# wei-zeng98/piano-a2s

Hardware: AMD Instinct MI355X
Metric: training clips/sec (12 s, 5-bar) (higher is better)
Workload: dtype f32

## Files before the change

### include/a2s.h

```cpp
#ifndef A2S_H
#define A2S_H
#include <stddef.h>
#include <stdint.h>
#ifdef __cplusplus
extern "C" {
#endif

#define A2S_OK 0
#define A2S_ERR_ARG (-1)
#define A2S_ERR_HIP (-2)
#define A2S_ERR_WORKSPACE (-3)

const char* a2s_last_error(void);
int a2s_version(void);
long long a2s_launch_count(void);

int a2s_gemm_f32(void* stream, int M, int N, int K, float alpha, const float* A, long sAm, long sAk,
                 const float* B, long sBk, long sBn, float beta, float* C, long ldc, const float* bias, int act,
                 int batch, long bsA, long bsB, long bsC, int splitk, float* workspace, size_t workspace_bytes);
int a2s_gemm_f32_affine(void* stream, int M, int N, int K, float alpha, const float* A, long sAm, long sAk, const float* B, long sBk,
                        long sBn, float beta, float* C, long ldc, const float* bias, int act, int batch, long bsA, long bsB, long bsC,
                        int splitk, float* workspace, size_t workspace_bytes, const float* a_scale, const float* a_shift, int a_period,
                        const float* b_scale, const float* b_shift, int b_period);
int a2s_gemm_f32_bnstats(void* stream, int M, int N, int K, const float* A, long sAm, long sAk, const float* B, long sBk, long sBn, float* C, long ldc,
                         const float* y, const float* mean, const float* invstd, const float* scale, const float* shift, int period, float* partial);
int a2s_gemm_f32_affine_scaled(void* stream, int M, int N, int K, float alpha, const float* A, long sAm, long sAk, const float* B, long sBk,
                               long sBn, float beta, float* C, long ldc, const float* bias, int act, int batch, long bsA, long bsB, long bsC,
                               int splitk, float* workspace, size_t workspace_bytes, const float* a_scale, const float* a_shift, int a_period,
                               const float* b_scale, const float* b_shift, int b_period, const float* a_absmax, const float* b_absmax);
int a2s_gemm_f32_bnstats_scaled(void* stream, int M, int N, int K, const float* A, long sAm, long sAk, const float* B, long sBk, long sBn, float* C, long ldc,
                                const float* y, const float* mean, const float* invstd, const float* scale, const float* shift, int period, float* partial,
                                const float* a_absmax, const float* b_absmax);
int a2s_linear_dgrad_bnstats(void* stream, int M, int N, int K, const float* dz, long lda, const float* Wt, float* da, long ldc, const float* y,
                             const float* mean, const float* invstd, const float* scale, const float* shift, int period, float* partial,
                             const float* dz_absmax, const float* w_absmax, float* workspace, size_t workspace_bytes, float* da_absmax_out);
int a2s_linear_fwd(void* stream, int M, int N, int K, const float* y, long lda, const float* W, float* z, long ldc, const float* scale, const float* shift,
                   int period, const float* y_absmax, const float* w_absmax, float* workspace, size_t workspace_bytes);
int a2s_linear_fwd_eligible(int M, int N, int K, int period);
int a2s_linear_wgrad(void* stream, int M, int N, int K, const float* dz, long ldz, const float* y, long lda, float* G, long ldg, const float* scale,
                     const float* shift, int period, const float* dz_absmax, const float* y_absmax, float* workspace, size_t workspace_bytes);
size_t a2s_linear_wgrad_ws_bytes(int M, int K);
int a2s_linear_wgrad_eligible(int M, int N, int K, int period);
size_t a2s_linear_dgrad_ws_bytes(int N, int K);
int a2s_linear_dgrad_blocks(int M);
int a2s_linear_dgrad_eligible(int M, int N, int K, int period);
int a2s_absmax(void* stream, const float* x, long n, float* out);
int a2s_gemm_bnstats_blocks(int M, int period);
size_t a2s_gemm_workspace_bytes(int M, int N, int batch, int splitk);
int a2s_gemm_pick_splitk(int M, int N, int K, int batch);
void a2s_gemm_debug_tile(int cfg);
int a2s_debug_set(const char* key, int value);
int a2s_debug_get(const char* key);
int a2s_env_check(void);
int a2s_persist_abort_latch(void* device_word);

int a2s_conv3x3(void* stream, const float* x, const float* w, float* y, const float* in_scale, const float* in_shift,
                float* stat_partial, int B, int T, int F, int Cin, int Cout, int flip, float* workspace);
int a2s_conv3x3_ranged(void* stream, const float* x, const float* w, float* y, const float* in_scale, const float* in_shift, const float* in_absmax,
                       float* stat_partial, float* out_absmax, int B, int T, int F, int Cin, int Cout, float* workspace);
int a2s_conv3x3_stat_blocks(int B, int T, int F, int Cin);
int a2s_conv3x3_dgrad_bnstats(void* stream, const float* dy, const float* w, float* g, const float* yl, const float* yl_mean, const float* yl_invstd,
                              const float* yl_scale, const float* yl_shift, float* stat_partial, int B, int T, int F, int Cin, int Cout,
                              float* workspace);
int a2s_bn_bwd_from_partial(void* stream, const float* g, const float* x, const float* mean, const float* invstd, const float* scale, const float* shift,
                            float* dgamma, float* dbeta, float* dx , const float* partial, int nblocks, float* c12, long rows, int C, int F);
int a2s_conv3x3_dgrad_bnstats_scaled(void* stream, const float* dy, const float* w, float* g, const float* yl, const float* yl_mean, const float* yl_invstd,
                                     const float* yl_scale, const float* yl_shift, float* stat_partial, int B, int T, int F, int Cin, int Cout,
                                     float* workspace, const float* dy_absmax);
int a2s_conv3x3_dgrad_bnstats_ranged(void* stream, const float* dy, const float* w, float* g, const float* yl, const float* yl_mean, const float* yl_invstd,
                                     const float* yl_scale, const float* yl_shift, float* stat_partial, int B, int T, int F, int Cin, int Cout,
                                     float* workspace, const float* dy_absmax, float* g_absmax_out);
int a2s_bn_bwd_from_partial_amax(void* stream, const float* g, const float* x, const float* mean, const float* invstd, const float* scale, const float* shift,
                                 float* dgamma, float* dbeta, float* dx, const float* partial, int nblocks, float* c12, long rows, int C, int F,
                                 float* dx_absmax);
size_t a2s_conv3x3_workspace_floats(int Cin);
int a2s_bn_finalize(void* stream, const float* partial, int nblocks, int C, double count, const float* gamma,
                    const float* beta, float* running_mean, float* running_var, long long* num_batches_tracked,
                    float* mean, float* invstd, float* scale, float* shift, float eps, float momentum, int training);
int a2s_bn_relu_apply(void* stream, const float* x, float* y, const float* scale, const float* shift, long n, int C, int F);
int a2s_col_stats(void* stream, const float* x, float* partial, long rows, int C, int rows_per_block);
int a2s_bn1d_relu_dropout(void* stream, const float* x, float* y, const float* scale, const float* shift,
                          const uint8_t* keep_mask, float inv_keep, long n, int C);

int a2s_gru_gates_fwd(void* stream, const float* gi, long ldgi, const float* gh, long ldgh, const float* hprev, long ldhp,
                      float* hout, long ldho, float* hout2, long ldho2, float* save, int R, int H);
int a2s_gru_seq_fwd(void* stream, const float* gi_all, long gi_bstride, long gi_tstride, const float* w_hh,
                    const float* b_hh, float* out, long out_bstride, long out_tstride, float* hbuf, float* gh,
                    float* save, float* hn, int B, int T, int H, int reverse, float* workspace, size_t workspace_bytes);

int a2s_attn_step_fwd(void* stream, const float* keys, const float* enc, const float* q, long ldq, const float* v,
                      float* ctx, long ldctx, float* ctx2, long ldctx2, float* attw, int B, int T, int H,
                      const int* n_done, int n_rows_total, float* workspace);
int a2s_attn_step_fwd_rows(void* stream, const float* keys, const float* enc, const float* q, long ldq, const float* v, float* ctx,
                           long ldctx, float* ctx2, long ldctx2, float* attw, int R, int T, int H, float* workspace, int n_clips,
                           const int* clip_order, const int* clip_rank, const int* row_until, int n_active, int step);
size_t a2s_attn_workspace_floats(int B, int T, int H);
size_t a2s_attn_workspace_floats_fused(int n_clips, int T, int H, int groups);

int a2s_log_softmax_rows(void* stream, const float* x, long ldx, float* y, long ldy, int* argmax_out, int R, int V);
int a2s_embed_rows(void* stream, const float* table, const long long* ids64, const int* ids32, long id_stride,
                   int const_id, float* out, long ldo, int col0, int R, int E, const uint8_t* keep_mask, float inv_keep);

typedef struct a2s_note_dec_args {
    const float* attn_w; const float* attn_b; const float* attn_v;
    const float* w_ih; const float* w_hh; const float* b_ih; const float* b_hh;
    const float* out_w; const float* out_b; const float* emb;
    const float* keys; const float* enc;
    float* h; float* x; float* q; float* gates; float* attw; float* o;
    float* gh; float* gi; float* logits;
    float* probs; long probs_bstride;
    const long long* gt; long gt_bstride;
    const uint8_t* tf_flags;
    const uint8_t* drop; float inv_keep;
    int* argmax_out; long am_bstride;
    int* eos_seen; long long* lengths; int* n_done;
    int* steps_exec;
    float* attn_ws;
    float* gemm_ws; size_t gemm_ws_bytes;
    int* t_base;
    const int* clip_order;
    const int* clip_rank;
    const int* row_until;
    const int* n_active;
    int n_clips;
    const int* m_active;
// ... 22 lines not shown
    float* probs_scratch;
    int* ids_out; long long* lengths_out; float* score_out;
} a2s_beam_args;
int a2s_note_decoder_fwd_beam(void* stream, const a2s_note_dec_args* args, const a2s_beam_args* beam, int* steps_done);
int a2s_beam_step(void* stream, const a2s_beam_args* beam, const float* logits, long ldl, const float* emb, float* xnext, long ldx, float* h, int h_cols,
                  float* q, int q_cols, int* n_done, int* steps_exec, int B, int V, int E, int t, int max_steps, int eos_id);
int a2s_beam_backtrack(void* stream, const a2s_beam_args* beam, float* probs, long probs_bstride, const int* steps_exec, int B, int V, int max_steps, int eos_id);
int a2s_beam_launches(void);
typedef struct a2s_align_args {
    float* attw_step;
    int* peak; float* weight; float* centroid;
    long out_stride;
    const signed char* next_state; int n_states;
    int* row_state;
} a2s_align_args;
int a2s_attn_align_rows(void* stream, const float* attw, long ldw, int R, int T, int* peak_out, float* weight_out, float* centroid_out, long out_stride);
int a2s_note_decoder_fwd_align(void* stream, const a2s_note_dec_args* args, const a2s_align_args* align, int* steps_done);
int a2s_align_launches(void);

int a2s_render_notes(void* stream, const int* programs, int rows_per_clip, int n_samples, float* wave, long wave_bstride, int B);
int a2s_render_launches(void);
int a2s_note_decoder_fwd_pair(void* stream_upper, void* stream_lower, const a2s_note_dec_args* upper, const a2s_note_dec_args* lower,
                              const int* pair_order, const int* pair_rank, const int* pair_n_active, int* steps_done_upper, int* steps_done_lower);
size_t a2s_note_step_workspace_floats(int H, int E);
size_t a2s_note_decoder_persist_ws_bytes(int n_clips, int R, int steps);
size_t a2s_note_decoder_bwd_persist_ws_bytes(int n_clips);

int a2s_staff_emb_fwd(void* stream, const float* note_emb, const float* const* gru_w, const long long* ids64,
                      const int* ids32, long id_bstride, const long long* lengths, long len_stride, float* out,
                      long ldo, int col0, float* hsave, int R, int maxlen, int E, int S);


int a2s_log_softmax_bwd_rows(void* stream, const float* g, const float* y, long outer_stride, int inner, float* dx,
                             int R, int V, int n_outer, int time_major);
int a2s_gru_gates_bwd(void* stream, const float* dh_a, long lda, const float* dh_b, long ldb, const float* save,
                      const float* hprev, long ldhp, float* dgi, long ldgi, float* dgh, long ldgh, float* dgh2, long ldgh2,
                      float* dhprev, long lddp, int R, int H);
int a2s_attn_step_bwd(void* stream, const float* keys, const float* enc, const float* q, long ldq, const float* v,
                      const float* attw, const float* ctx, long ldctx, const float* dctx_a, long ldda, const float* dctx_b,
                      long lddb, float* dctx_out, long lddo, float* dq, long lddq, float* ds_out, int B, int T, int H, float* workspace);
int a2s_attn_step_bwd_rows(void* stream, const float* keys, const float* enc, const float* q, long ldq, const float* v, const float* attw,
                           const float* ctx, long ldctx, const float* dctx_a, long ldda, const float* dctx_b, long lddb, float* dctx_out,
                           long lddo, float* dq, long lddq, float* ds_out, int R, int T, int H, float* workspace, int n_clips,
                           const int* clip_order, const int* clip_rank, const int* row_until, int n_active, int step);
int a2s_attn_dk_accum(void* stream, const float* keys, const float* q_all, const float* ds_all, const float* v, float* dK,
                      float* dv_partial, int B, int T, int S, int H, const int* row_until, int groups);
int a2s_attn_dk_blocks(int B, int T);
int a2s_attn_denc_accum(void* stream, const float* attw_all, const float* dctx_all, float* dEnc, int B, int T, int S, int H2,
                        const int* row_until, int groups);
int a2s_col_sum(void* stream, const float* x, long ld, float* out, long rows, int C, float alpha, float beta, float* workspace, size_t workspace_floats);
int a2s_embed_scatter_add(void* stream, float* table_grad, const long long* ids64, const int* ids32, long id_stride,
                          int const_id, const float* g, long ldg, int col0, int R, int E, const uint8_t* keep_mask, float inv_keep);
int a2s_ew_act_bwd(void* stream, const float* g, const float* y, float* dx, long n, int act);

typedef struct a2s_note_dec_bwd_args {
    const float* attn_w; const float* attn_v; const float* w_ih; const float* w_hh;
    const float* keys; const float* enc;
    const float* h; const float* x; const float* q; const float* gates; const float* attw;
    const float* do_all;
    float* dgi_all; float* dgh_all; float* dq_all; float* ds_all; float* dctx_all; float* dx;
    float* dh;
    float* attn_ws;
    float* gemm_ws; size_t gemm_ws_bytes;
    const int* clip_order;
    const int* clip_rank;
    const int* row_until;
    const int* n_active;
    int n_clips;
    const int* m_active;
    const int* row_list;
    const int* n_rows_active;
    int R, T, H, E, steps;
    float* step_ws; size_t step_ws_floats;
    float* persist_ws; size_t persist_ws_bytes;
    const float* w_ih_full;
} a2s_note_dec_bwd_args;
int a2s_note_decoder_bwd(void* stream, const a2s_note_dec_bwd_args* args);
int a2s_note_decoder_bwd_pair(void* stream_upper, void* stream_lower, const a2s_note_dec_bwd_args* upper, const a2s_note_dec_bwd_args* lower,
                              const int* pair_order, const int* pair_rank, const int* pair_n_active);

int a2s_gru_seq_bwd(void* stream, const float* dout, long do_bstride, long do_tstride, const float* out, long out_bstride,
                    long out_tstride, const float* gates, const float* w_hh, const float* dhn, float* dgi_all, float* dgh_shift,
                    float* dgh_first, float* dhbuf, float* dgh_tmp, int B, int T, int H, int reverse, float* workspace, size_t workspace_bytes);
int a2s_staff_emb_bwd(void* stream, const float* note_emb, const float* const* gru_w, float* const* grads, float* note_emb_grad,
                      const long long* ids64, const int* ids32, long id_bstride, const long long* lengths, long len_stride,
                      const float* dout, long lddo, int col0, const float* hsave, int R, int maxlen, int E, int S);

int a2s_bn_bwd(void* stream, const float* g, const float* x, const float* mean, const float* invstd, const float* scale,
               const float* shift, const uint8_t* keep_mask, float inv_keep, float* dgamma, float* dbeta, float* dx,
               float* partial, float* c12, long rows, int C, int F);
int a2s_bn_bwd_amax(void* stream, const float* g, const float* x, const float* mean, const float* invstd, const float* scale,
                    const float* shift, const uint8_t* keep_mask, float inv_keep, float* dgamma, float* dbeta, float* dx,
                    float* partial, float* c12, long rows, int C, int F, float* dx_absmax);
size_t a2s_bn_bwd_partial_floats(long rows, int C, int F);
int a2s_bn_bwd_stats(void* stream, const float* g, const float* x, const float* mean, const float* invstd, const float* scale,
                     const float* shift, const uint8_t* keep_mask, float inv_keep, float* partial, float* sums, long rows, int C, int F);
int a2s_bn_bwd_apply(void* stream, const float* g, const float* x, const float* mean, const float* invstd, const float* scale,
                     const float* shift, const uint8_t* keep_mask, float inv_keep, const float* sums_local, const float* sums_global,
                     double count_global, float* dgamma, float* dbeta, float* dx, float* c12, long rows, int C, int F);
int a2s_bn_bwd_sums_from_partial(void* stream, const float* partial, int nblocks, int C, float* sums);
int a2s_bn_bwd_c12_from_sums(void* stream, const float* sums_local, const float* sums_global, double count_global, float* dgamma, float* dbeta,
                             float* c12, int C);
int a2s_conv3x3_wgrad(void* stream, const float* dy, const float* x, const float* in_scale, const float* in_shift, float* dW,
                      float* workspace, size_t workspace_bytes, int B, int T, int F, int Cin, int Cout);
int a2s_conv3x3_wgrad_scaled(void* stream, const float* dy, const float* x, const float* in_scale, const float* in_shift, float* dW,
                             float* workspace, size_t workspace_bytes, int B, int T, int F, int Cin, int Cout, const float* dy_absmax);
int a2s_conv3x3_wgrad_ranged(void* stream, const float* dy, const float* x, const float* in_scale, const float* in_shift, float* dW, float* workspace,
                             size_t workspace_bytes, int B, int T, int F, int Cin, int Cout, const float* dy_absmax, const float* act_absmax);
int a2s_act_bound(void* stream, const float* scale, const float* shift, const float* absmax, int C, float* out);
size_t a2s_conv3x3_wgrad_workspace_bytes(int Cin, int Cout);
int a2s_conv3x3_wgrad_bn(void* stream, const float* g, const float* y, const float* mean, const float* invstd, const float* scale, const float* shift,
                         const float* c12, float* dy_out, const float* x, const float* in_scale, const float* in_shift, float* dW, float* workspace,
                         size_t workspace_bytes, int B, int T, int F, int Cin, int Cout);
int a2s_conv3x3_wgrad_bn_ranged(void* stream, const float* g, const float* y, const float* mean, const float* invstd, const float* scale, const float* shift,
                                const float* c12, const float* g_absmax, int g_absmax_n, const float* y_absmax, float* dy_out, float* dy_absmax_out, const float* x,
                                const float* in_scale, const float* in_shift, float* dW, float* workspace, size_t workspace_bytes, int B, int T, int F,
                                int Cin, int Cout, const float* act_absmax);
int a2s_conv3x3_wgrad_bn_ranged_eligible(int F, int Cin, int Cout);

int a2s_nll_loss(void* stream, const float* logp, const long long* target, long rows, int V, long long ignore_index,
                 float* loss_out, float* dlogp, float gscale, double* partial, int nblocks);
int a2s_nll_grad(void* stream, float* dlogp, const long long* target, const float* loss_out, float gscale, long rows, int V,
                 long long ignore_index);
int a2s_clip_adadelta(void* stream, float* params, float* grads, float* square_avg, float* acc_delta, long n, const float* loss,
                      float max_norm, float lr, float rho, float eps, float* ctl, double* partial, int nblocks, int zero_grad);

int a2s_vqt_logmag(void* stream, const float* C, float* out, float* partial, int B, long rows, int bins, float top_db);
int a2s_vqt_logmag_octaves(void* stream, const float* C, float* out, float* partial, int B, long rows, int bins, int bins_per_octave, float top_db);
int a2s_vqt_decimate(void* stream, const float* ypad, long padded_len, const float* taps, int ntaps, float* out, long n_out, int B);

int a2s_edit_distance(void* stream, const int* ref, const long long* ref_off, const int* hyp, const long long* hyp_off, const int* order,
                      int n_pairs, int max_ref_len, int max_hyp_len, int* dist);
int a2s_edit_distance_max_len(void);

#ifdef __cplusplus
}
#endif
#endif
```

### piano_a2s_amd/csrc/a2s_api.hip

```cpp
#define A2S_SWITCHES_IMPL
#include "a2s_internal.h"

thread_local char a2s_err_msg[512] = {0};
long long a2s_launch_counter = 0;

#define ST ((hipStream_t)stream)

extern "C" {

const char* a2s_last_error(void) { return a2s_err_msg; }
int a2s_version(void) { return 1; }
long long a2s_launch_count(void) { return __atomic_load_n(&a2s_launch_counter, __ATOMIC_RELAXED); }

int a2s_gemm_f32(void* stream, int M, int N, int K, float alpha, const float* A, long sAm, long sAk, const float* B, long sBk,
                 long sBn, float beta, float* C, long ldc, const float* bias, int act, int batch, long bsA, long bsB, long bsC,
                 int splitk, float* workspace, size_t workspace_bytes) {
    return a2s_gemm_impl(ST, M, N, K, alpha, A, sAm, sAk, B, sBk, sBn, beta, C, ldc, bias, act, batch, bsA, bsB, bsC, splitk,
                         workspace, workspace_bytes);
}
int a2s_gemm_f32_affine(void* stream, int M, int N, int K, float alpha, const float* A, long sAm, long sAk, const float* B, long sBk,
                        long sBn, float beta, float* C, long ldc, const float* bias, int act, int batch, long bsA, long bsB, long bsC,
                        int splitk, float* workspace, size_t workspace_bytes, const float* a_scale, const float* a_shift, int a_period,
                        const float* b_scale, const float* b_shift, int b_period) {
    return a2s_gemm_affine_impl(ST, M, N, K, alpha, A, sAm, sAk, B, sBk, sBn, beta, C, ldc, bias, act, batch, bsA, bsB, bsC, splitk,
                                workspace, workspace_bytes, a_scale, a_shift, a_period, b_scale, b_shift, b_period,
                                nullptr, nullptr, nullptr, nullptr, nullptr, nullptr, 0, 0, nullptr, nullptr);
}
int a2s_gemm_f32_affine_scaled(void* stream, int M, int N, int K, float alpha, const float* A, long sAm, long sAk, const float* B, long sBk,
                               long sBn, float beta, float* C, long ldc, const float* bias, int act, int batch, long bsA, long bsB, long bsC,
                               int splitk, float* workspace, size_t workspace_bytes, const float* a_scale, const float* a_shift, int a_period,
                               const float* b_scale, const float* b_shift, int b_period, const float* a_absmax, const float* b_absmax) {
    return a2s_gemm_affine_impl(ST, M, N, K, alpha, A, sAm, sAk, B, sBk, sBn, beta, C, ldc, bias, act, batch, bsA, bsB, bsC, splitk,
                                workspace, workspace_bytes, a_scale, a_shift, a_period, b_scale, b_shift, b_period,
                                nullptr, nullptr, nullptr, nullptr, nullptr, nullptr, 0, 1, a_absmax, b_absmax);
}
int a2s_gemm_f32_bnstats_scaled(void* stream, int M, int N, int K, const float* A, long sAm, long sAk, const float* B, long sBk, long sBn, float* C, long ldc,
                                const float* y, const float* mean, const float* invstd, const float* scale, const float* shift, int period, float* partial,
                                const float* a_absmax, const float* b_absmax) {
    return a2s_gemm_affine_impl(ST, M, N, K, 1.f, A, sAm, sAk, B, sBk, sBn, 0.f, C, ldc, nullptr, 0, 1, 0, 0, 0, 1, nullptr, 0,
                                nullptr, nullptr, 0, nullptr, nullptr, 0, y, mean, invstd, scale, shift, partial, period, 1, a_absmax, b_absmax);
}
int a2s_absmax(void* stream, const float* x, long n, float* out) { return a2s_absmax_impl(ST, x, n, out); }
int a2s_linear_dgrad_bnstats(void* stream, int M, int N, int K, const float* dz, long lda, const float* Wt, float* da, long ldc, const float* y,
                             const float* mean, const float* invstd, const float* scale, const float* shift, int period, float* partial,
                             const float* dz_absmax, const float* w_absmax, float* workspace, size_t workspace_bytes, float* da_absmax_out) {
    return a2s_linear_dgrad_bnstats_impl(ST, M, N, K, dz, lda, Wt, 1, K, da, ldc, y, mean, invstd, scale, shift, period, partial, dz_absmax, w_absmax,
                                         workspace, workspace_bytes, da_absmax_out);
}
size_t a2s_linear_dgrad_ws_bytes(int N, int K) { return a2s_linear_dgrad_ws_bytes_impl(N, K); }
int a2s_linear_fwd(void* stream, int M, int N, int K, const float* y, long lda, const float* W, float* z, long ldc, const float* scale, const float* shift,
                   int period, const float* y_absmax, const float* w_absmax, float* workspace, size_t workspace_bytes) {
    return a2s_linear_fwd_impl(ST, M, N, K, y, lda, W, z, ldc, scale, shift, period, y_absmax, w_absmax, workspace, workspace_bytes);
}
int a2s_linear_wgrad(void* stream, int M, int N, int K, const float* dz, long ldz, const float* y, long lda, float* G, long ldg, const float* scale,
                     const float* shift, int period, const float* dz_absmax, const float* y_absmax, float* workspace, size_t workspace_bytes) {
    return a2s_linear_wgrad_impl(ST, M, N, K, dz, ldz, y, lda, G, ldg, scale, shift, period, dz_absmax, y_absmax, workspace, workspace_bytes);
}
size_t a2s_linear_wgrad_ws_bytes(int M, int K) { return a2s_linear_wgrad_ws_bytes_impl(M, K); }
int a2s_linear_wgrad_eligible(int M, int N, int K, int period) { return a2s_linear_wgrad_ok(M, N, K, 256, 4, 4, period, nullptr, nullptr, nullptr) ? 1 : 0; }
int a2s_linear_fwd_eligible(int M, int N, int K, int period) { return a2s_linear_fwd_ok(M, N, K, 4, 4, period, nullptr, nullptr, nullptr) ? 1 : 0; }
int a2s_linear_dgrad_blocks(int M) { return a2s_linear_dgrad_blocks_impl(M); }
int a2s_linear_dgrad_eligible(int M, int N, int K, int period) {
    return a2s_linear_dgrad_ok(M, N, K, 4, 1, K, 4, period, nullptr, nullptr, nullptr, nullptr) ? 1 : 0;
}
int a2s_gemm_f32_bnstats(void* stream, int M, int N, int K, const float* A, long sAm, long sAk, const float* B, long sBk, long sBn, float* C, long ldc,
                         const float* y, const float* mean, const float* invstd, const float* scale, const float* shift, int period, float* partial) {
    return a2s_gemm_affine_impl(ST, M, N, K, 1.f, A, sAm, sAk, B, sBk, sBn, 0.f, C, ldc, nullptr, 0, 1, 0, 0, 0, 1, nullptr, 0,
                                nullptr, nullptr, 0, nullptr, nullptr, 0, y, mean, invstd, scale, shift, partial, period, 0, nullptr, nullptr);
}
int a2s_gemm_bnstats_blocks(int M, int period) { return a2s_cdiv(M, 128) * a2s_gemm_bnstats_slots(period); }
size_t a2s_gemm_workspace_bytes(int M, int N, int batch, int splitk) { return a2s_gemm_workspace_bytes_impl(M, N, batch, splitk); }
int a2s_gemm_pick_splitk(int M, int N, int K, int batch) { return a2s_gemm_pick_splitk_impl(M, N, K, batch); }
void a2s_gemm_debug_tile(int cfg) { a2s_gemm_debug_tile_impl(cfg); }
size_t a2s_note_step_workspace_floats(int H, int E) { return a2s_note_step_workspace_floats_impl(H, E); }
int a2s_debug_set(const char* key, int value) {
    if (!key) return A2S_ERR_ARG;
    const int id = a2s_switch_find(key);
    if (id >= 0) { a2s_switch_store(id, value); return A2S_OK; }
    if (!strcmp(key, "attn_deferred_fast")) { a2s_attn_deferred_fast = value ? 1 : 0; return A2S_OK; }
    if (!strcmp(key, "gemm_tile")) { a2s_gemm_debug_tile_impl(value); return A2S_OK; }
    snprintf(a2s_err_msg, sizeof(a2s_err_msg), "a2s_debug_set: unknown key %s", key);
    return A2S_ERR_ARG;
}
int a2s_env_check(void) {
    if (const char* e = a2s_switch_env_error()) A2S_FAIL(A2S_ERR_ARG, "%s: expected a decimal number >= 0", e);
    return A2S_OK;
}

int a2s_persist_abort_latch(void* device_word) { a2s_persist_latch_set(device_word); return A2S_OK; }

int a2s_debug_get(const char* key) {
    if (!key) return -1;
    const int id = a2s_switch_find(key);
    if (id == A2S_SW_attn_pair_fused_rows) return a2s_attn_pair_fused_rows();
    if (id >= 0) return a2s_sw((a2s_switch)id);
    if (!strcmp(key, "attn_pair_launches")) return (int)a2s_attn_pair_launches();
    if (!strcmp(key, "attn_pair_bwd_launches")) return (int)a2s_attn_pair_bwd_launches();
    if (!strcmp(key, "attn_deferred_fast")) return a2s_attn_deferred_fast;
    if (!strcmp(key, "attn_dk_ahead_launches")) return (int)a2s_attn_dk_ahead_launches();
    if (!strcmp(key, "attn_denc_launches")) return (int)a2s_attn_denc_launches();
    if (!strcmp(key, "dec_mid_launches")) return a2s_dec_mid_launches();
    if (!strcmp(key, "dec_persist_launches")) return a2s_dec_persist_launches();
    if (!strcmp(key, "edit_distance_launches")) return (int)a2s_edit_distance_launches();
    if (!strcmp(key, "conv_rows16_c20_launches")) return (int)a2s_conv_rows16_c20_launches();
    if (!strcmp(key, "device_cus")) return a2s_device_geometry().cus;
    if (!strcmp(key, "device_xccs")) return a2s_device_geometry().xccs;
    return -1;
}

int a2s_conv3x3(void* stream, const float* x, const float* w, float* y, const float* in_scale, const float* in_shift,
                float* stat_partial, int B, int T, int F, int Cin, int Cout, int flip, float* workspace) {
    return a2s_conv3x3_impl(ST, x, w, y, in_scale, in_shift, stat_partial, B, T, F, Cin, Cout, flip, workspace, nullptr, nullptr, nullptr, nullptr, nullptr, nullptr,
                            nullptr, nullptr);
}
int a2s_conv3x3_ranged(void* stream, const float* x, const float* w, float* y, const float* in_scale, const float* in_shift, const float* in_absmax,
                       float* stat_partial, float* out_absmax, int B, int T, int F, int Cin, int Cout, float* workspace) {
    return a2s_conv3x3_impl(ST, x, w, y, in_scale, in_shift, stat_partial, B, T, F, Cin, Cout, 0, workspace, nullptr, nullptr, nullptr, nullptr, nullptr, nullptr,
                            in_absmax, out_absmax);
}
int a2s_conv3x3_dgrad_bnstats(void* stream, const float* dy, const float* w, float* g, const float* yl, const float* yl_mean, const float* yl_invstd,
                              const float* yl_scale, const float* yl_shift, float* stat_partial, int B, int T, int F, int Cin, int Cout,
                              float* workspace) {
    if (!yl) { snprintf(a2s_err_msg, sizeof(a2s_err_msg), "conv3x3_dgrad_bnstats: yl is required"); return A2S_ERR_ARG; }
    return a2s_conv3x3_impl(ST, dy, w, g, nullptr, nullptr, stat_partial, B, T, F, Cin, Cout, 1, workspace, yl, yl_mean, yl_invstd, yl_scale, yl_shift, nullptr, nullptr, nullptr);
}
int a2s_conv3x3_dgrad_bnstats_scaled(void* stream, const float* dy, const float* w, float* g, const float* yl, const float* yl_mean, const float* yl_invstd,
                                     const float* yl_scale, const float* yl_shift, float* stat_partial, int B, int T, int F, int Cin, int Cout,
                                     float* workspace, const float* dy_absmax) {
    if (!yl) { snprintf(a2s_err_msg, sizeof(a2s_err_msg), "conv3x3_dgrad_bnstats_scaled: yl is required"); return A2S_ERR_ARG; }
    return a2s_conv3x3_impl(ST, dy, w, g, nullptr, nullptr, stat_partial, B, T, F, Cin, Cout, 1, workspace, yl, yl_mean, yl_invstd, yl_scale, yl_shift, dy_absmax, nullptr, nullptr);
}
int a2s_conv3x3_dgrad_bnstats_ranged(void* stream, const float* dy, const float* w, float* g, const float* yl, const float* yl_mean, const float* yl_invstd,
                                     const float* yl_scale, const float* yl_shift, float* stat_partial, int B, int T, int F, int Cin, int Cout,
                                     float* workspace, const float* dy_absmax, float* g_absmax_out) {
    if (!yl) { snprintf(a2s_err_msg, sizeof(a2s_err_msg), "conv3x3_dgrad_bnstats_ranged: yl is required"); return A2S_ERR_ARG; }
    return a2s_conv3x3_impl(ST, dy, w, g, nullptr, nullptr, stat_partial, B, T, F, Cin, Cout, 1, workspace, yl, yl_mean, yl_invstd, yl_scale, yl_shift, dy_absmax, nullptr, g_absmax_out);
}
int a2s_bn_bwd_from_partial(void* stream, const float* g, const float* x, const float* mean, const float* invstd, const float* scale, const float* shift,
                            float* dgamma, float* dbeta, float* dx, const float* partial, int nblocks, float* c12, long rows, int C, int F) {
    return a2s_bn_bwd_from_partial_impl(ST, g, x, mean, invstd, scale, shift, dgamma, dbeta, dx, partial, nblocks, c12, rows, C, F, nullptr);
}
int a2s_bn_bwd_from_partial_amax(void* stream, const float* g, const float* x, const float* mean, const float* invstd, const float* scale, const float* shift,
                                 float* dgamma, float* dbeta, float* dx, const float* partial, int nblocks, float* c12, long rows, int C, int F,
                                 float* dx_absmax) {
    return a2s_bn_bwd_from_partial_impl(ST, g, x, mean, invstd, scale, shift, dgamma, dbeta, dx, partial, nblocks, c12, rows, C, F, dx_absmax);
}
size_t a2s_conv3x3_workspace_floats(int Cin) { return a2s_conv3x3_workspace_floats_impl(Cin); }
int a2s_conv3x3_stat_blocks(int B, int T, int F, int Cin) { return a2s_conv3x3_stat_blocks_impl(B, T, F, Cin); }
int a2s_bn_finalize(void* stream, const float* partial, int nblocks, int C, double count, const float* gamma, const float* beta,
                    float* running_mean, float* running_var, long long* nbt, float* mean, float* invstd, float* scale,
                    float* shift, float eps, float momentum, int training) {
    return a2s_bn_finalize_impl(ST, partial, nblocks, C, count, gamma, beta, running_mean, running_var, nbt, mean, invstd, scale,
                                shift, eps, momentum, training);
}
int a2s_bn_relu_apply(void* stream, const float* x, float* y, const float* scale, const float* shift, long n, int C, int F) {
    return a2s_bn_relu_apply_impl(ST, x, y, scale, shift, n, C, F);
}
int a2s_col_stats(void* stream, const float* x, float* partial, long rows, int C, int rows_per_block) {
    return a2s_col_stats_impl(ST, x, partial, rows, C, rows_per_block);
}
int a2s_bn1d_relu_dropout(void* stream, const float* x, float* y, const float* scale, const float* shift, const uint8_t* keep_mask,
                          float inv_keep, long n, int C) {
    return a2s_bn1d_relu_dropout_impl(ST, x, y, scale, shift, keep_mask, inv_keep, n, C);
}
int a2s_gru_gates_fwd(void* stream, const float* gi, long ldgi, const float* gh, long ldgh, const float* hprev, long ldhp,
                      float* hout, long ldho, float* hout2, long ldho2, float* save, int R, int H) {
    return a2s_gru_gates_fwd_impl(ST, gi, ldgi, gh, ldgh, hprev, ldhp, hout, ldho, hout2, ldho2, save, R, H);
}
int a2s_gru_seq_fwd(void* stream, const float* gi_all, long gi_bstride, long gi_tstride, const float* w_hh, const float* b_hh,
                    float* out, long out_bstride, long out_tstride, float* hbuf, float* gh, float* save, float* hn, int B, int T,
                    int H, int reverse, float* workspace, size_t workspace_bytes) {
    return a2s_gru_seq_fwd_impl(ST, gi_all, gi_bstride, gi_tstride, w_hh, b_hh, out, out_bstride, out_tstride, hbuf, gh, save, hn,
                                B, T, H, reverse, workspace, workspace_bytes);
}
int a2s_attn_step_fwd(void* stream, const float* keys, const float* enc, const float* q, long ldq, const float* v, float* ctx,
                      long ldctx, float* ctx2, long ldctx2, float* attw, int B, int T, int H, const int* n_done, int n_rows_total, float* workspace) {
    return a2s_attn_step_fwd_impl(ST, keys, enc, q, ldq, v, ctx, ldctx, ctx2, ldctx2, attw, B, T, H, n_done, n_rows_total, workspace, nullptr);
}
int a2s_attn_step_fwd_rows(void* stream, const float* keys, const float* enc, const float* q, long ldq, const float* v, float* ctx,
                           long ldctx, float* ctx2, long ldctx2, float* attw, int R, int T, int H, float* workspace, int n_clips,
                           const int* clip_order, const int* clip_rank, const int* row_until, int n_active, int step) {
// ... 39 lines not shown
    if (!beam) { snprintf(a2s_err_msg, sizeof(a2s_err_msg), "beam_backtrack: null args"); return A2S_ERR_ARG; }
    const a2s_beam_args& g = *beam;
    const BeamBackArgs a = {g.score, g.token_hist, g.parent_hist, g.probs_scratch, probs, probs_bstride, g.ids_out, (long)max_steps, g.lengths_out, g.score_out,
                            steps_exec, g.alpha, B, g.K, V, max_steps, eos_id, g.pad_id};
    return a2s_beam_backtrack_impl(ST, a);
}
int a2s_beam_launches(void) { return a2s_beam_launches_impl(); }
int a2s_attn_align_rows(void* stream, const float* attw, long ldw, int R, int T, int* peak_out, float* weight_out, float* centroid_out, long out_stride) {
    return a2s_attn_align_rows_impl(ST, attw, ldw, R, T, peak_out, weight_out, centroid_out, out_stride);
}
int a2s_note_decoder_fwd_align(void* stream, const a2s_note_dec_args* args, const a2s_align_args* align, int* steps_done) {
    if (!args || !align) { snprintf(a2s_err_msg, sizeof(a2s_err_msg), "note_decoder_fwd_align: null args"); return A2S_ERR_ARG; }
    return a2s_note_decoder_fwd_align_impl(ST, *args, *align, steps_done);
}
int a2s_align_launches(void) { return a2s_align_launches_impl(); }
int a2s_render_notes(void* stream, const int* programs, int rows_per_clip, int n_samples, float* wave, long wave_bstride, int B) {
    return a2s_render_notes_impl(ST, programs, rows_per_clip, n_samples, wave, wave_bstride, B);
}
int a2s_render_launches(void) { return a2s_render_launches_impl(); }
int a2s_note_decoder_fwd_pair(void* stream_upper, void* stream_lower, const a2s_note_dec_args* upper, const a2s_note_dec_args* lower,
                              const int* pair_order, const int* pair_rank, const int* pair_n_active, int* steps_done_upper, int* steps_done_lower) {
    if (!upper || !lower) { snprintf(a2s_err_msg, sizeof(a2s_err_msg), "note_decoder_fwd_pair: null args"); return A2S_ERR_ARG; }
    return a2s_note_decoder_fwd_pair_impl((hipStream_t)stream_upper, (hipStream_t)stream_lower, *upper, *lower, pair_order, pair_rank, pair_n_active,
                                          steps_done_upper, steps_done_lower);
}
int a2s_staff_emb_fwd(void* stream, const float* note_emb, const float* const* gru_w, const long long* ids64, const int* ids32,
                      long id_bstride, const long long* lengths, long len_stride, float* out, long ldo, int col0, float* hsave,
                      int R, int maxlen, int E, int S) {
    if (!gru_w) { snprintf(a2s_err_msg, sizeof(a2s_err_msg), "staff_emb_fwd: null weight table"); return A2S_ERR_ARG; }
    return a2s_staff_emb_fwd_impl(ST, note_emb, gru_w, ids64, ids32, id_bstride, lengths, len_stride, out, ldo, col0, hsave, R,
                                  maxlen, E, S);
}

int a2s_log_softmax_bwd_rows(void* stream, const float* g, const float* y, long outer_stride, int inner, float* dx, int R, int V,
                             int n_outer, int time_major) {
    return a2s_log_softmax_bwd_rows_impl(ST, g, y, outer_stride, inner, dx, R, V, n_outer, time_major);
}
int a2s_gru_gates_bwd(void* stream, const float* dh_a, long lda, const float* dh_b, long ldb, const float* save, const float* hprev,
                      long ldhp, float* dgi, long ldgi, float* dgh, long ldgh, float* dgh2, long ldgh2, float* dhprev, long lddp, int R, int H) {
    return a2s_gru_gates_bwd_impl(ST, dh_a, lda, dh_b, ldb, save, hprev, ldhp, dgi, ldgi, dgh, ldgh, dgh2, ldgh2, dhprev, lddp, R, H);
}
int a2s_attn_step_bwd(void* stream, const float* keys, const float* enc, const float* q, long ldq, const float* v, const float* attw,
                      const float* ctx, long ldctx, const float* dctx_a, long ldda, const float* dctx_b, long lddb, float* dctx_out,
                      long lddo, float* dq, long lddq, float* ds_out, int B, int T, int H, float* workspace) {
    return a2s_attn_step_bwd_impl(ST, keys, enc, q, ldq, v, attw, ctx, ldctx, dctx_a, ldda, dctx_b, lddb, dctx_out, lddo, dq, lddq, ds_out, B, T, H, workspace, nullptr);
}
int a2s_attn_step_bwd_rows(void* stream, const float* keys, const float* enc, const float* q, long ldq, const float* v, const float* attw,
                           const float* ctx, long ldctx, const float* dctx_a, long ldda, const float* dctx_b, long lddb, float* dctx_out,
                           long lddo, float* dq, long lddq, float* ds_out, int R, int T, int H, float* workspace, int n_clips,
                           const int* clip_order, const int* clip_rank, const int* row_until, int n_active, int step) {
    a2s_attn_rows rows = {clip_order, clip_rank, row_until, n_clips, n_active, step};
    return a2s_attn_step_bwd_impl(ST, keys, enc, q, ldq, v, attw, ctx, ldctx, dctx_a, ldda, dctx_b, lddb, dctx_out, lddo, dq, lddq, ds_out, R, T, H, workspace, &rows);
}
int a2s_attn_dk_accum(void* stream, const float* keys, const float* q_all, const float* ds_all, const float* v, float* dK,
                      float* dv_partial, int B, int T, int S, int H, const int* row_until, int groups) {
    return a2s_attn_dk_accum_impl(ST, keys, q_all, ds_all, v, dK, dv_partial, B, T, S, H, row_until, groups);
}
int a2s_attn_dk_blocks(int B, int T) { return B * ((T + 15) / 16); }
int a2s_attn_denc_accum(void* stream, const float* attw_all, const float* dctx_all, float* dEnc, int B, int T, int S, int H2,
                        const int* row_until, int groups) {
    return a2s_attn_denc_accum_impl(ST, attw_all, dctx_all, dEnc, B, T, S, H2, row_until, groups);
}
int a2s_col_sum(void* stream, const float* x, long ld, float* out, long rows, int C, float alpha, float beta, float* workspace, size_t workspace_floats) {
    return a2s_col_sum_impl(ST, x, ld, out, rows, C, alpha, beta, workspace, workspace_floats);
}
int a2s_embed_scatter_add(void* stream, float* table_grad, const long long* ids64, const int* ids32, long id_stride, int const_id,
                          const float* g, long ldg, int col0, int R, int E, const uint8_t* keep_mask, float inv_keep) {
    return a2s_embed_scatter_add_impl(ST, table_grad, ids64, ids32, id_stride, const_id, g, ldg, col0, R, E, keep_mask, inv_keep);
}
int a2s_ew_act_bwd(void* stream, const float* g, const float* y, float* dx, long n, int act) { return a2s_ew_act_bwd_impl(ST, g, y, dx, n, act); }
int a2s_note_decoder_bwd(void* stream, const a2s_note_dec_bwd_args* args) {
    if (!args) { snprintf(a2s_err_msg, sizeof(a2s_err_msg), "note_decoder_bwd: null args"); return A2S_ERR_ARG; }
    return a2s_note_decoder_bwd_impl(ST, *args);
}
int a2s_note_decoder_bwd_pair(void* stream_upper, void* stream_lower, const a2s_note_dec_bwd_args* upper, const a2s_note_dec_bwd_args* lower,
                              const int* pair_order, const int* pair_rank, const int* pair_n_active) {
    if (!upper || !lower) { snprintf(a2s_err_msg, sizeof(a2s_err_msg), "note_decoder_bwd_pair: null args"); return A2S_ERR_ARG; }
    return a2s_note_decoder_bwd_pair_impl((hipStream_t)stream_upper, (hipStream_t)stream_lower, *upper, *lower, pair_order, pair_rank, pair_n_active);
}
int a2s_gru_seq_bwd(void* stream, const float* dout, long do_bstride, long do_tstride, const float* out, long out_bstride, long out_tstride,
                    const float* gates, const float* w_hh, const float* dhn, float* dgi_all, float* dgh_shift, float* dgh_first,
                    float* dhbuf, float* dgh_tmp, int B, int T, int H, int reverse, float* workspace, size_t workspace_bytes) {
    return a2s_gru_seq_bwd_impl(ST, dout, do_bstride, do_tstride, out, out_bstride, out_tstride, gates, w_hh, dhn, dgi_all, dgh_shift,
                                dgh_first, dhbuf, dgh_tmp, B, T, H, reverse, workspace, workspace_bytes);
}
int a2s_staff_emb_bwd(void* stream, const float* note_emb, const float* const* gru_w, float* const* grads, float* note_emb_grad,
                      const long long* ids64, const int* ids32, long id_bstride, const long long* lengths, long len_stride,
                      const float* dout, long lddo, int col0, const float* hsave, int R, int maxlen, int E, int S) {
    if (!gru_w) { snprintf(a2s_err_msg, sizeof(a2s_err_msg), "staff_emb_bwd: null weight table"); return A2S_ERR_ARG; }
    return a2s_staff_emb_bwd_impl(ST, note_emb, gru_w, grads, note_emb_grad, ids64, ids32, id_bstride, lengths, len_stride, dout, lddo,
                                  col0, hsave, R, maxlen, E, S);
}

int a2s_bn_bwd(void* stream, const float* g, const float* x, const float* mean, const float* invstd, const float* scale, const float* shift,
               const uint8_t* keep_mask, float inv_keep, float* dgamma, float* dbeta, float* dx, float* partial, float* c12, long rows, int C, int F) {
    return a2s_bn_bwd_impl(ST, g, x, mean, invstd, scale, shift, keep_mask, inv_keep, dgamma, dbeta, dx, partial, c12, rows, C, F, nullptr);
}
int a2s_bn_bwd_amax(void* stream, const float* g, const float* x, const float* mean, const float* invstd, const float* scale, const float* shift,
                    const uint8_t* keep_mask, float inv_keep, float* dgamma, float* dbeta, float* dx, float* partial, float* c12, long rows, int C, int F,
                    float* dx_absmax) {
    return a2s_bn_bwd_impl(ST, g, x, mean, invstd, scale, shift, keep_mask, inv_keep, dgamma, dbeta, dx, partial, c12, rows, C, F, dx_absmax);
}
size_t a2s_bn_bwd_partial_floats(long rows, int C, int F) { return a2s_bn_bwd_partial_floats_impl(rows, C, F); }
int a2s_conv3x3_wgrad(void* stream, const float* dy, const float* x, const float* in_scale, const float* in_shift, float* dW, float* workspace,
                      size_t workspace_bytes, int B, int T, int F, int Cin, int Cout) {
    return a2s_conv3x3_wgrad_impl(ST, dy, x, in_scale, in_shift, dW, workspace, workspace_bytes, B, T, F, Cin, Cout, nullptr, nullptr, nullptr, nullptr,
                                  nullptr, nullptr, nullptr, nullptr, nullptr);
}
int a2s_conv3x3_wgrad_ranged(void* stream, const float* dy, const float* x, const float* in_scale, const float* in_shift, float* dW, float* workspace,
                             size_t workspace_bytes, int B, int T, int F, int Cin, int Cout, const float* dy_absmax, const float* act_absmax) {
    return a2s_conv3x3_wgrad_impl(ST, dy, x, in_scale, in_shift, dW, workspace, workspace_bytes, B, T, F, Cin, Cout, nullptr, nullptr, nullptr, nullptr,
                                  nullptr, nullptr, nullptr, dy_absmax, act_absmax);
}
int a2s_act_bound(void* stream, const float* scale, const float* shift, const float* absmax, int C, float* out) {
    return a2s_act_bound_impl(ST, scale, shift, absmax, C, out);
}
int a2s_conv3x3_wgrad_scaled(void* stream, const float* dy, const float* x, const float* in_scale, const float* in_shift, float* dW, float* workspace,
                             size_t workspace_bytes, int B, int T, int F, int Cin, int Cout, const float* dy_absmax) {
    return a2s_conv3x3_wgrad_impl(ST, dy, x, in_scale, in_shift, dW, workspace, workspace_bytes, B, T, F, Cin, Cout, nullptr, nullptr, nullptr, nullptr,
                                  nullptr, nullptr, nullptr, dy_absmax, nullptr);
}
int a2s_conv3x3_wgrad_bn(void* stream, const float* g, const float* y, const float* mean, const float* invstd, const float* scale, const float* shift,
                         const float* c12, float* dy_out, const float* x, const float* in_scale, const float* in_shift, float* dW, float* workspace,
                         size_t workspace_bytes, int B, int T, int F, int Cin, int Cout) {
    if (!y) { snprintf(a2s_err_msg, sizeof(a2s_err_msg), "conv3x3_wgrad_bn: y is required"); return A2S_ERR_ARG; }
    return a2s_conv3x3_wgrad_impl(ST, g, x, in_scale, in_shift, dW, workspace, workspace_bytes, B, T, F, Cin, Cout, y, mean, invstd, scale, shift, c12, dy_out, nullptr, nullptr);
}
size_t a2s_conv3x3_wgrad_workspace_bytes(int Cin, int Cout) { return a2s_conv3x3_wgrad_workspace_bytes_impl(Cin, Cout); }
int a2s_conv3x3_wgrad_bn_ranged_eligible(int F, int Cin, int Cout) { return (a2s_wgrad_rows_eligible(F, Cin, Cout) && !(Cin == 40 && Cout == 20)) ? 1 : 0; }
int a2s_conv3x3_wgrad_bn_ranged(void* stream, const float* g, const float* y, const float* mean, const float* invstd, const float* scale, const float* shift,
                                const float* c12, const float* g_absmax, int g_absmax_n, const float* y_absmax, float* dy_out, float* dy_absmax_out, const float* x,
                                const float* in_scale, const float* in_shift, float* dW, float* workspace, size_t workspace_bytes, int B, int T, int F,
                                int Cin, int Cout, const float* act_absmax) {
    if (!a2s_conv3x3_wgrad_bn_ranged_eligible(F, Cin, Cout)) { snprintf(a2s_err_msg, sizeof(a2s_err_msg), "conv3x3_wgrad_bn_ranged: shape not eligible"); return A2S_ERR_ARG; }
    return a2s_conv3x3_wgrad_rows_bn_impl(ST, g, y, mean, invstd, scale, shift, c12, g_absmax, g_absmax_n, y_absmax, dy_out, dy_absmax_out, x, in_scale, in_shift, dW,
                                          workspace, workspace_bytes, B, T, F, Cin, Cout, act_absmax);
}

int a2s_nll_grad(void* stream, float* dlogp, const long long* target, const float* loss_out, float gscale, long rows, int V, long long ignore_index) {
    return a2s_nll_grad_impl(ST, dlogp, target, loss_out, gscale, rows, V, ignore_index);
}
int a2s_nll_loss(void* stream, const float* logp, const long long* target, long rows, int V, long long ignore_index, float* loss_out,
                 float* dlogp, float gscale, double* partial, int nblocks) {
    return a2s_nll_loss_impl(ST, logp, target, rows, V, ignore_index, loss_out, dlogp, gscale, partial, nblocks);
}
int a2s_clip_adadelta(void* stream, float* params, float* grads, float* square_avg, float* acc_delta, long n, const float* loss, float max_norm,
                      float lr, float rho, float eps, float* ctl, double* partial, int nblocks, int zero_grad) {
    return a2s_clip_adadelta_impl(ST, params, grads, square_avg, acc_delta, n, loss, max_norm, lr, rho, eps, ctl, partial, nblocks, zero_grad);
}

int a2s_vqt_logmag(void* stream, const float* C, float* out, float* partial, int B, long rows, int bins, float top_db) {
    return a2s_vqt_logmag_impl(ST, C, out, partial, B, rows, bins, top_db);
}

int a2s_edit_distance(void* stream, const int* ref, const long long* ref_off, const int* hyp, const long long* hyp_off, const int* order,
                      int n_pairs, int max_ref_len, int max_hyp_len, int* dist) {
    return a2s_edit_distance_impl(ST, ref, ref_off, hyp, hyp_off, order, n_pairs, max_ref_len, max_hyp_len, dist);
}
int a2s_edit_distance_max_len(void) { return a2s_edit_distance_max_len_impl(); }

int a2s_bn_bwd_stats(void* stream, const float* g, const float* x, const float* mean, const float* invstd, const float* scale, const float* shift,
                     const uint8_t* keep_mask, float inv_keep, float* partial, float* sums, long rows, int C, int F) {
    return a2s_bn_bwd_stats_impl(ST, g, x, mean, invstd, scale, shift, keep_mask, inv_keep, partial, sums, rows, C, F);
}
int a2s_bn_bwd_apply(void* stream, const float* g, const float* x, const float* mean, const float* invstd, const float* scale, const float* shift,
                     const uint8_t* keep_mask, float inv_keep, const float* sums_local, const float* sums_global, double count_global,
                     float* dgamma, float* dbeta, float* dx, float* c12, long rows, int C, int F) {
// ... 19 lines not shown
```

### piano_a2s_amd/csrc/a2s_bwd.hip

```cpp
#include "a2s_internal.h"

__global__ __launch_bounds__(256) void log_softmax_bwd_rows(const float* __restrict__ g, const float* __restrict__ y,
                                                            long outer_stride, int inner, float* __restrict__ dx,
                                                            int R, int V, int n_outer, int time_major) {
    const int row = blockIdx.x * 4 + (threadIdx.x >> 6), lane = threadIdx.x & 63;
    if (row >= R) return;
    const int ob = row / inner, in = row % inner;
    const float* gr = g + (long)ob * outer_stride + (long)in * V;
    const float* yr = y + (long)ob * outer_stride + (long)in * V;
    float s = 0.f;
    for (int j = lane; j < V; j += 64) s += gr[j];
    s = wave_sum(s);
    const long orow = time_major ? ((long)in * n_outer + ob) : row;
    for (int j = lane; j < V; j += 64) dx[orow * V + j] = gr[j] - expf(yr[j]) * s;
}

int a2s_log_softmax_bwd_rows_impl(hipStream_t st, const float* g, const float* y, long outer_stride, int inner, float* dx,
                                  int R, int V, int n_outer, int time_major) {
    hipLaunchKernelGGL(log_softmax_bwd_rows, dim3(a2s_cdiv(R, 4)), dim3(256), 0, st, g, y, outer_stride, inner, dx, R, V, n_outer, time_major);
    A2S_CHECK_LAUNCH("log_softmax_bwd_rows");
    return A2S_OK;
}

__global__ void gru_gates_bwd(const float* __restrict__ dh_a, long lda, const float* __restrict__ dh_b, long ldb,
// ... 473 lines not shown
    for (int s = a.steps - 1; s >= 0 && !any_fused; --s) any_fused = note_bwd_step_fused(a, s);
    const bool mid = a2s_note_step_mid_bwd_ok(a);
    bool any_mid = false;
    if (mid) for (int s = a.steps - 1; s >= 0 && !any_mid; --s) any_mid = !note_bwd_step_fused(a, s);
    if (any_fused || any_mid) { int rc = a2s_note_step_fused_bwd_prepare(st, a); if (rc) return rc; }
    *mid_out = mid;
    return A2S_OK;
}
static int note_bwd_finish(hipStream_t st, const a2s_note_dec_bwd_args& a, int cur) {
    if (cur != 0) {
        const hipError_t e = hipMemcpyAsync(a.dh, a.dh + (long)a.R * 2 * a.H, sizeof(float) * a.R * 2 * a.H, hipMemcpyDeviceToDevice, st);
        if (e != hipSuccess) A2S_FAIL(A2S_ERR_HIP, "note_decoder_bwd copy: %s", hipGetErrorString(e));
    }
    return A2S_OK;
}

int a2s_note_decoder_bwd_impl(hipStream_t st, const a2s_note_dec_bwd_args& a) {
    if (a2s_note_decoder_bwd_persist_ok(a)) return a2s_note_decoder_bwd_persist(st, a);
    bool mid = false;
    int rc = note_bwd_prepare(st, a, &mid);
    if (rc) return rc;
    int cur = 0;
    for (int s = a.steps - 1; s >= 0; --s) {
        rc = note_bwd_step(st, a, s, cur, mid, 0, nullptr);
        if (rc) return rc;
    }
    return note_bwd_finish(st, a, cur);
}

int a2s_note_decoder_bwd_pair_impl(hipStream_t su, hipStream_t sl, const a2s_note_dec_bwd_args& au, const a2s_note_dec_bwd_args& al, const int* pair_order,
                                   const int* pair_rank, const int* pair_n_active) {
    const a2s_note_dec_bwd_args* as[2] = {&au, &al};
    hipStream_t sts[2] = {su, sl};
    const bool can_pair = a2s_sw(A2S_SW_attn_pair) && su != sl && pair_order && pair_rank && pair_n_active && au.n_active && al.n_active && au.n_clips > 0 &&
                          au.n_clips == al.n_clips && au.R == al.R && au.T == al.T && au.H == 256 && al.H == 256 && au.enc == al.enc && au.attn_ws && al.attn_ws &&
                          !a2s_note_decoder_bwd_persist_ok(au) && !a2s_note_decoder_bwd_persist_ok(al) && a2s_note_step_mid_bwd_ok(au) && a2s_note_step_mid_bwd_ok(al);
    if (!can_pair) {
        const int rc = a2s_note_decoder_bwd_impl(su, au);
        return rc ? rc : a2s_note_decoder_bwd_impl(sl, al);
    }
    static thread_local hipEvent_t ev[2] = {nullptr, nullptr};
    for (int k = 0; k < 2; ++k)
        if (!ev[k]) { const hipError_t e = hipEventCreateWithFlags(&ev[k], hipEventDisableTiming); if (e != hipSuccess) A2S_FAIL(A2S_ERR_HIP, "note_decoder_bwd_pair: hipEventCreate: %s", hipGetErrorString(e)); }
    bool mid[2] = {false, false};
    int cur[2] = {0, 0};
    const PairRowsLimit limit(a2s_attn_pair_fused_rows());
    for (int k = 0; k < 2; ++k) { const int rc = note_bwd_prepare(sts[k], *as[k], &mid[k]); if (rc) return rc; }
    const int nmax = au.steps > al.steps ? au.steps : al.steps;
    for (int s = nmax - 1; s >= 0; --s) {
        bool in[2], fused[2] = {false, false};
        for (int k = 0; k < 2; ++k) { in[k] = s < as[k]->steps; if (in[k]) fused[k] = note_bwd_step_fused(*as[k], s); }
        AttnPairBwdStep p = {pair_order, pair_rank, au.n_clips, pair_n_active[s], s, 1, au.T};
        const bool joint = in[0] && in[1] && mid[0] && mid[1] && !fused[0] && !fused[1] && p.n_active > 0 && au.n_active[s] > 0 && al.n_active[s] > 0;
        if (!joint) {
            for (int k = 0; k < 2; ++k)
                if (in[k]) { const int rc = note_bwd_step(sts[k], *as[k], s, cur[k], mid[k], 0, nullptr); if (rc) return rc; }
            continue;
        }
        for (int k = 0; k < 2; ++k) { const int rc = note_bwd_step(sts[k], *as[k], s, cur[k], mid[k], 1, nullptr); if (rc) return rc; }
        hipError_t e = hipEventRecord(ev[1], sl);
        if (e == hipSuccess) e = hipStreamWaitEvent(su, ev[1], 0);
        if (e != hipSuccess) A2S_FAIL(A2S_ERR_HIP, "note_decoder_bwd_pair: event: %s", hipGetErrorString(e));
        const int rc = attn_pair_bwd_sweep(su, au, al, s, p);
        if (rc) return rc;
        e = hipEventRecord(ev[0], su);
        if (e == hipSuccess) e = hipStreamWaitEvent(sl, ev[0], 0);
        if (e != hipSuccess) A2S_FAIL(A2S_ERR_HIP, "note_decoder_bwd_pair: event: %s", hipGetErrorString(e));
        for (int k = 0; k < 2; ++k) { const int rc2 = note_bwd_step(sts[k], *as[k], s, cur[k], mid[k], 2, &p); if (rc2) return rc2; }
    }
    for (int k = 0; k < 2; ++k) { const int rc = note_bwd_finish(sts[k], *as[k], cur[k]); if (rc) return rc; }
    return A2S_OK;
}


__global__ void transpose_f32(const float* __restrict__ in, float* __restrict__ out, int rows, int cols) {
    const int idx = blockIdx.x * blockDim.x + threadIdx.x;
    if (idx >= rows * cols) return;
    const int c = idx / rows, r = idx % rows;
    out[idx] = in[(long)r * cols + c];
}

int a2s_gru_seq_bwd_impl(hipStream_t st, const float* dout, long do_bstride, long do_tstride, const float* out, long out_bstride,
                         long out_tstride, const float* gates, const float* w_hh, const float* dhn, float* dgi_all, float* dgh_shift,
                         float* dgh_first, float* dhbuf, float* dgh_tmp, int B, int T, int H, int reverse, float* ws, size_t ws_bytes) {
    A2S_REQUIRE(dout && out && gates && w_hh && dgi_all && dgh_shift && dgh_first && dhbuf && dgh_tmp, "gru_seq_bwd: null tensor");
    hipError_t e;
    if (dhn) e = hipMemcpyAsync(dhbuf, dhn, sizeof(float) * B * H, hipMemcpyDeviceToDevice, st);
    else e = hipMemsetAsync(dhbuf, 0, sizeof(float) * B * H, st);
    if (e != hipSuccess) A2S_FAIL(A2S_ERR_HIP, "gru_seq_bwd init: %s", hipGetErrorString(e));
    e = hipMemsetAsync(dgh_shift, 0, sizeof(float) * (size_t)B * T * 3 * H, st);
    if (e != hipSuccess) A2S_FAIL(A2S_ERR_HIP, "gru_seq_bwd memset: %s", hipGetErrorString(e));
    const bool fused = a2s_sw(A2S_SW_gru_fused) && H % 32 == 0 && ws && ws_bytes >= sizeof(float) * 3 * H * H && ((uintptr_t)ws % 16 == 0);
    if (fused) {
        hipLaunchKernelGGL(transpose_f32, dim3(a2s_cdiv(3 * H * H, 256)), dim3(256), 0, st, w_hh, ws, 3 * H, H);
        A2S_CHECK_LAUNCH("transpose_f32");
    }
    if (fused && a2s_gru_seq_bwd_persist_ok(B, T, H, ws, ws_bytes, sizeof(float) * 3 * (size_t)H * H))
        return a2s_gru_seq_bwd_persist_impl(st, dout, do_bstride, do_tstride, out, out_bstride, out_tstride, gates, ws, dhn, dgi_all, dgh_shift, dgh_first, B, T, H,
                                            reverse, ws, sizeof(float) * 3 * (size_t)H * H, ws_bytes);
    if (fused && ws_bytes >= sizeof(float) * (3 * (size_t)H * H + 3 * (size_t)B * H) && (3 * H * H) % 4 == 0) {
        float* tmp[2] = {dgh_tmp, ws + 3 * (size_t)H * H};
        auto tix = [&](int s) { return reverse ? T - 1 - s : s; };
        int cur = 0, p = 0;
        {
            const int s = T - 1, t = tix(s), tp = reverse ? t + 1 : t - 1;
            float* dgh = (s == 0) ? dgh_first : tmp[p];
            int rc = a2s_gru_gates_bwd_impl(st, dhbuf, H, dout + (long)t * do_tstride, do_bstride, gates + (long)t * B * 4 * H,
                                            s == 0 ? nullptr : out + (long)tp * out_tstride, out_bstride,
                                            dgi_all + (long)t * 3 * H, (long)T * 3 * H, dgh, 3 * H,
                                            s == 0 ? nullptr : dgh_shift + (long)tp * 3 * H, (long)T * 3 * H, dhbuf + (long)B * H, H, B, H);
            if (rc) return rc;
            cur = 1;
        }
        for (int s = T - 1; s >= 1; --s) {
            const int sp = s - 1, t = tix(sp), tp = reverse ? t + 1 : t - 1;
            float* dgh_out = (sp == 0) ? dgh_first : tmp[p ^ 1];
            int rc = a2s_gru_bptt_step_impl(st, tmp[p], ws, dhbuf + (long)cur * B * H, dout + (long)t * do_tstride, do_bstride,
                                            gates + (long)t * B * 4 * H, sp == 0 ? nullptr : out + (long)tp * out_tstride, out_bstride,
                                            dgi_all + (long)t * 3 * H, (long)T * 3 * H, dgh_out,
                                            sp == 0 ? nullptr : dgh_shift + (long)tp * 3 * H, (long)T * 3 * H,
                                            dhbuf + (long)(cur ^ 1) * B * H, B, H);
            if (rc) return rc;
            cur ^= 1; p ^= 1;
        }
        return A2S_OK;
    }
    int cur = 0;
    for (int s = T - 1; s >= 0; --s) {
        const int t = reverse ? T - 1 - s : s;
        const int tp = reverse ? t + 1 : t - 1;
        float* dh_in = dhbuf + (long)cur * B * H;
        float* dh_out = dhbuf + (long)(cur ^ 1) * B * H;
        float* dgh = (s == 0) ? dgh_first : dgh_tmp;
        int rc = a2s_gru_gates_bwd_impl(st, dh_in, H, dout + (long)t * do_tstride, do_bstride, gates + (long)t * B * 4 * H,
                                        s == 0 ? nullptr : out + (long)tp * out_tstride, out_bstride,
                                        dgi_all + (long)t * 3 * H, (long)T * 3 * H, dgh, 3 * H,
                                        s == 0 ? nullptr : dgh_shift + (long)tp * 3 * H, (long)T * 3 * H, dh_out, H, B, H);
        if (rc) return rc;
        if (s > 0) {
            if (fused) rc = a2s_skinny_gemm_acc_impl(st, dgh, 3 * H, ws, 3 * H, dh_out, H, B, H, 3 * H);
            else rc = a2s_gemm_impl(st, B, H, 3 * H, 1.f, dgh, 3 * H, 1, w_hh, H, 1, 1.f, dh_out, H, nullptr, 0, 1, 0, 0, 0, 0, ws, ws_bytes);
            if (rc) return rc;
        }
        cur ^= 1;
    }
    return A2S_OK;
}

__global__ __launch_bounds__(128) void staff_emb_bwd(const float* __restrict__ note_emb, const float* __restrict__ w_ih_f,
                                                     const float* __restrict__ w_hh_f, const float* __restrict__ b_ih_f,
                                                     const float* __restrict__ b_hh_f, const float* __restrict__ w_ih_r,
                                                     const float* __restrict__ w_hh_r, const float* __restrict__ b_ih_r,
                                                     const float* __restrict__ b_hh_r, float* const* __restrict__ grads ,
                                                     float* __restrict__ note_emb_grad, const long long* __restrict__ ids64,
                                                     const int* __restrict__ ids32, long id_bstride, const long long* __restrict__ lengths,
                                                     long len_stride, const float* __restrict__ dout, long lddo, int col0,
                                                     const float* __restrict__ hsave, int maxlen, int E, int S) {
    extern __shared__ float sm[];
    const int b = blockIdx.x, dir = blockIdx.y, tid = threadIdx.x, nt = blockDim.x;
    const float* w_ih = dir ? w_ih_r : w_ih_f; const float* w_hh = dir ? w_hh_r : w_hh_f;
    const float* b_ih = dir ? b_ih_r : b_ih_f; const float* b_hh = dir ? b_hh_r : b_hh_f;
    float* Wi = sm;
    float* Wh = Wi + 3 * S * E;
    float* gWi = Wh + 3 * S * S;
    float* gWh = gWi + 3 * S * E;
    float* gbi = gWh + 3 * S * S;
    float* gbh = gbi + 3 * S;
    float* bi = gbh + 3 * S; float* bh = bi + 3 * S;
    float* xe = bh + 3 * S;
    float* hp = xe + E;
    float* g = hp + S;
    float* dgi = g + 6 * S;
    float* dgh = dgi + 3 * S;
    float* dh = dgh + 3 * S;
    for (int i = tid; i < 3 * S * E; i += nt) { Wi[i] = w_ih[i]; gWi[i] = 0.f; }
    for (int i = tid; i < 3 * S * S; i += nt) { Wh[i] = w_hh[i]; gWh[i] = 0.f; }
    for (int i = tid; i < 3 * S; i += nt) { bi[i] = b_ih[i]; bh[i] = b_hh[i]; gbi[i] = 0.f; gbh[i] = 0.f; }
    for (int i = tid; i < S; i += nt) dh[i] = dout[(long)b * lddo + col0 + dir * S + i];
    int len = (int)lengths[(long)b * len_stride];
    len = max(0, min(len, maxlen));
    int* lid = reinterpret_cast<int*>(dh + S);
    for (int i = tid; i < len; i += nt) {
// ... 815 lines not shown
```

### piano_a2s_amd/csrc/a2s_internal.h

```cpp
#pragma once
#include "a2s_common.h"
#include "../../include/a2s.h"
#include "a2s_switches.h"

static inline int a2s_attn_pair_fused_rows(void) {
    const int cap = a2s_sw(A2S_SW_dec_fused_max_rows), v = a2s_sw(A2S_SW_attn_pair_fused_rows);
    return v < cap ? v : cap;
}
static inline unsigned a2s_persist_dbg(void) {
    return (a2s_sw(A2S_SW_persist_force_agent) ? PERSIST_DBG_FORCE_AGENT : 0u) | (a2s_sw(A2S_SW_persist_inject_abort) ? PERSIST_DBG_INJECT_ABORT : 0u);
}

int a2s_absmax_impl(hipStream_t st, const float* x, long n, float* out);
size_t a2s_gemm_workspace_bytes_impl(int M, int N, int batch, int splitk);
int a2s_gemm_pick_splitk_impl(int M, int N, int K, int batch);
int a2s_gemm_bnstats_slots(int period);
void a2s_gemm_debug_tile_impl(int cfg);
int a2s_gemm_affine_impl(hipStream_t st, int M, int N, int K, float alpha, const float* A, long sAm, long sAk,
    const float* B, long sBk, long sBn, float beta, float* C, long ldc, const float* bias, int act,
    int batch, long bsA, long bsB, long bsC, int splitk, float* ws, size_t ws_bytes,
    const float* a_scale, const float* a_shift, int a_period, const float* b_scale, const float* b_shift, int b_period,
    const float* ep_y, const float* ep_mean, const float* ep_invstd, const float* ep_scale, const float* ep_shift,
    float* ep_partial, int ep_period, int two_term, const float* a_absmax, const float* b_absmax);
int a2s_gemm_impl(hipStream_t st, int M, int N, int K, float alpha, const float* A, long sAm, long sAk,
    const float* B, long sBk, long sBn, float beta, float* C, long ldc, const float* bias, int act,
    int batch, long bsA, long bsB, long bsC, int splitk, float* ws, size_t ws_bytes);

size_t a2s_linear_dgrad_ws_bytes_impl(int N, int K);
int a2s_linear_dgrad_blocks_impl(int M);
bool a2s_linear_dgrad_ok(int M, int N, int K, long lda, long sBk, long sBn, long ldc, int period, const void* A, const void* B, const void* C, const void* y);
int a2s_linear_dgrad_bnstats_impl(hipStream_t st, int M, int N, int K, const float* A, long lda, const float* Wt, long sBk, long sBn, float* C, long ldc,
    const float* ep_y, const float* mean, const float* invstd, const float* scale, const float* shift, int period,
    float* partial, const float* a_absmax, const float* b_absmax, float* ws, size_t ws_bytes, float* c_absmax_out);
bool a2s_linear_fwd_ok(int M, int N, int K, long lda, long ldc, int period, const void* A, const void* W, const void* C);
int a2s_linear_fwd_impl(hipStream_t st, int M, int N, int K, const float* A, long lda, const float* W, float* C, long ldc, const float* a_scale,
    const float* a_shift, int period, const float* a_absmax, const float* w_absmax, float* ws, size_t ws_bytes);
size_t a2s_linear_wgrad_ws_bytes_impl(int M, int K);
bool a2s_linear_wgrad_ok(int M, int N, int K, long ldz, long lda, long ldg, int period, const void* dz, const void* A, const void* G);
int a2s_linear_wgrad_impl(hipStream_t st, int M, int N, int K, const float* dz, long ldz, const float* A, long lda, float* G, long ldg, const float* a_scale,
    const float* a_shift, int period, const float* dz_absmax, const float* a_absmax, float* ws, size_t ws_bytes);

int a2s_act_bound_impl(hipStream_t st, const float* scale, const float* shift, const float* absmax, int C, float* out);
size_t a2s_conv3x3_workspace_floats_impl(int Cin);
int a2s_conv3x3_impl(hipStream_t st, const float* x, const float* w, float* y, const float* in_scale,
    const float* in_shift, float* stat_partial, int B, int T, int F, int Cin, int Cout, int flip, float* ws,
    const float* yl, const float* yl_mean, const float* yl_invstd, const float* yl_scale, const float* yl_shift,
    const float* x_absmax, const float* in_absmax, float* out_absmax);
int a2s_conv3x3_stat_blocks_impl(int B, int T, int F, int Cin);
int a2s_bn_finalize_impl(hipStream_t st, const float* partial, int nblocks, int C, double count, const float* gamma,
    const float* beta, float* running_mean, float* running_var, long long* nbt, float* mean,
    float* invstd, float* scale, float* shift, float eps, float momentum, int training);
int a2s_bn_relu_apply_impl(hipStream_t st, const float* x, float* y, const float* scale, const float* shift, long n, int C, int F);
int a2s_col_stats_impl(hipStream_t st, const float* x, float* partial, long rows, int C, int rows_per_block);
int a2s_bn1d_relu_dropout_impl(hipStream_t st, const float* x, float* y, const float* scale, const float* shift,
    const uint8_t* mask, float inv_keep, long n, int C);
size_t a2s_conv3x3_wgrad_workspace_bytes_impl(int Cin, int Cout);
int a2s_conv3x3_wgrad_impl(hipStream_t st, const float* dy, const float* x, const float* in_scale, const float* in_shift, float* dW,
    float* ws, size_t ws_bytes, int B, int T, int F, int Cin, int Cout, const float* bn_y, const float* bn_mean,
    const float* bn_invstd, const float* bn_scale, const float* bn_shift, const float* bn_c12, float* dy_out,
    const float* dy_absmax, const float* act_absmax);
int a2s_bn_bwd_impl(hipStream_t st, const float* g, const float* x, const float* mean, const float* invstd, const float* scale,
    const float* shift, const uint8_t* mask, float inv_keep, float* dgamma, float* dbeta, float* dx, float* partial,
    float* c12, long rows, int C, int F, float* dx_absmax);
int a2s_bn_bwd_from_partial_impl(hipStream_t st, const float* g, const float* x, const float* mean, const float* invstd, const float* scale,
    const float* shift, float* dgamma, float* dbeta, float* dx, const float* partial, int nblocks, float* c12,
    long rows, int C, int F, float* dx_absmax);
int a2s_bn_bwd_stats_impl(hipStream_t st, const float* g, const float* x, const float* mean, const float* invstd, const float* scale,
    const float* shift, const uint8_t* mask, float inv_keep, float* partial, float* sums, long rows, int C, int F);
int a2s_bn_bwd_apply_impl(hipStream_t st, const float* g, const float* x, const float* mean, const float* invstd, const float* scale,
    const float* shift, const uint8_t* mask, float inv_keep, const float* sums_local, const float* sums_global,
    double count_global, float* dgamma, float* dbeta, float* dx, float* c12, long rows, int C, int F);
int a2s_bn_bwd_sums_from_partial_impl(hipStream_t st, const float* partial, int nblocks, int C, float* sums);
int a2s_bn_bwd_c12_from_sums_impl(hipStream_t st, const float* sums_local, const float* sums_global, double count_global, float* dgamma, float* dbeta,
    float* c12, int C);
size_t a2s_bn_bwd_partial_floats_impl(long rows, int C, int F);

int a2s_channel_absmax_impl(hipStream_t st, const float* x, long rows, int C, int F, float* out);
bool a2s_conv_rows_eligible(int F, int Cin);
int a2s_conv_rows_blocks(int B, int T, int F);
size_t a2s_conv_rows_workspace_floats(int Cin);
long a2s_conv_rows16_c20_launches(void);
int a2s_conv3x3_rows_impl(hipStream_t st, const float* x, const float* w, float* y, const float* in_scale, const float* in_shift,
    const float* in_absmax, float* stat_partial, float* out_absmax, int B, int T, int F, int Cin, int Cout, int flip,
    float* ws, const float* yl, const float* yl_mean, const float* yl_invstd, const float* yl_scale, const float* yl_shift,
    const float* x_absmax);

bool a2s_wgrad_rows_eligible(int F, int Cin, int Cout);
int a2s_conv3x3_wgrad_rows_bn_impl(hipStream_t st, const float* g, const float* y, const float* mean, const float* invstd, const float* scale,
    const float* shift, const float* c12, const float* g_absmax, int g_absmax_n, const float* y_absmax, float* dz_out,
    float* dz_absmax_out, const float* x, const float* in_scale, const float* in_shift, float* dW, float* ws, size_t ws_bytes,
    int B, int T, int F, int Cin, int Cout, const float* act_absmax);
int a2s_conv3x3_wgrad_rows_impl(hipStream_t st, const float* dy, const float* x, const float* in_scale, const float* in_shift, float* dW, float* ws,
    size_t ws_bytes, int B, int T, int F, int Cin, int Cout, const float* dy_absmax, const float* act_absmax);

struct StepFinArgs {
    const float* logits; long ldl;
    float* probs; long probs_bstride;
    const long long* gt; long gt_bstride;
    const float* emb;
    float* xnext; long ldx;
    const uint8_t* drop; float inv_keep;
    int* argmax_out; long am_bstride;
    int* eos_seen; long long* lengths; int* n_done; int* steps_exec;
    const int* t_base;
    const int* row_until;
    int n_clips;
    int R, V, E, t, teacher_force, eos_id, max_t;
};
struct a2s_grammar_ref { const signed char* next; int n_states; int* row_state; };
int a2s_gru_gates_fwd_impl(hipStream_t st, const float* gi, long ldgi, const float* gh, long ldgh, const float* hprev,
    long ldhp, float* hout, long ldho, float* hout2, long ldho2, float* save, int R, int H);
int a2s_gru_bptt_step_impl(hipStream_t st, const float* dgh, const float* w_hh_t, const float* dhz_in, const float* dout, long ld_dout,
    const float* save, const float* hprev, long ld_hprev, float* dgi, long ld_dgi, float* dgh_out, float* dgh2,
    long ld_dgh2, float* dhz_out, int R, int H);
int a2s_skinny_gemm_acc_impl(hipStream_t st, const float* A, long lda, const float* Bt, long ldb, float* Cm, long ldc, int R, int N, int K);
int a2s_gru_seq_fwd_impl(hipStream_t st, const float* gi_all, long gi_bstride, long gi_tstride, const float* w_hh,
    const float* b_hh, float* out, long out_bstride, long out_tstride, float* hbuf, float* gh,
    float* save, float* hn, int B, int T, int H, int reverse, float* ws, size_t ws_bytes);
int a2s_attn_step_fwd_impl(hipStream_t st, const float* Kmat, const float* enc, const float* q, long ldq, const float* v,
    float* ctx, long ldctx, float* ctx2, long ldctx2, float* attw, int B, int T, int H,
    const int* n_done, int n_rows_total, float* ws, const a2s_attn_rows* rows = nullptr, a2s_attn_deferred* defer = nullptr);
int a2s_log_softmax_rows_impl(hipStream_t st, const float* x, long ldx, float* y, long ldy, int* argmax_out, int R, int V);
int a2s_embed_rows_impl(hipStream_t st, const float* table, const long long* ids64, const int* ids32, long id_stride,
    int const_id, float* out, long ldo, int col0, int R, int E, const uint8_t* drop, float inv_keep);
int a2s_note_decoder_fwd_impl(hipStream_t st, const a2s_note_dec_args& a, int* steps_done);
int a2s_note_decoder_fwd_grammar_impl(hipStream_t st, const a2s_note_dec_args& a, const a2s_grammar_ref& g, int* steps_done);
int a2s_note_decoder_fwd_pair_impl(hipStream_t su, hipStream_t sl, const a2s_note_dec_args& au, const a2s_note_dec_args& al, const int* pair_order,
    const int* pair_rank, const int* pair_n_active, int* done_u, int* done_l);
int a2s_staff_emb_fwd_impl(hipStream_t st, const float* note_emb, const float* const* w ,
    const long long* ids64, const int* ids32, long id_bstride, const long long* lengths,
    long len_stride, float* out, long ldo, int col0, float* hsave, int R, int maxlen, int E, int S);
size_t a2s_attn_workspace_floats_impl(int B, int T, int H, int groups);
size_t a2s_attn_bulk_lds(size_t shm, int n_active, int backward);
long a2s_attn_pair_launches(void);

int a2s_log_softmax_bwd_rows_impl(hipStream_t st, const float* g, const float* y, long outer_stride, int inner, float* dx,
    int R, int V, int n_outer, int time_major);
int a2s_gru_gates_bwd_impl(hipStream_t st, const float* dh_a, long lda, const float* dh_b, long ldb, const float* save,
    const float* hprev, long ldhp, float* dgi, long ldgi, float* dgh, long ldgh, float* dgh2, long ldgh2,
    float* dhprev, long lddp, int R, int H);
int a2s_attn_step_bwd_impl(hipStream_t st, const float* Kmat, const float* enc, const float* q, long ldq, const float* v,
    const float* attw, const float* ctx, long ldctx, const float* dctx_a, long ldda, const float* dctx_b,
    long lddb, float* dctx_out, long lddo, float* dq, long lddq, float* ds_out, int B, int T, int H, float* ws,
    const a2s_attn_rows* rows = nullptr);
int a2s_attn_dk_accum_impl(hipStream_t st, const float* Kmat, const float* q_all, const float* ds_all, const float* v,
    float* dK, float* dv_partial, int B, int T, int S, int H, const int* row_until, int groups);
int a2s_attn_denc_accum_impl(hipStream_t st, const float* attw_all, const float* dctx_all, float* dEnc, int B, int T, int S, int H2,
    const int* row_until, int groups);
long a2s_attn_dk_ahead_launches(void);
long a2s_attn_denc_launches(void);
int a2s_col_sum_impl(hipStream_t st, const float* x, long ld, float* out, long rows, int C, float alpha, float beta, float* ws, size_t ws_floats);
int a2s_embed_scatter_add_impl(hipStream_t st, float* table_grad, const long long* ids64, const int* ids32, long id_stride,
    int const_id, const float* g, long ldg, int col0, int R, int E, const uint8_t* drop, float inv_keep);
int a2s_ew_act_bwd_impl(hipStream_t st, const float* g, const float* y, float* dx, long n, int act);
int a2s_note_decoder_bwd_impl(hipStream_t st, const a2s_note_dec_bwd_args& a);
int a2s_note_decoder_bwd_pair_impl(hipStream_t su, hipStream_t sl, const a2s_note_dec_bwd_args& au, const a2s_note_dec_bwd_args& al, const int* pair_order,
    const int* pair_rank, const int* pair_n_active);
int a2s_gru_seq_bwd_impl(hipStream_t st, const float* dout, long do_bstride, long do_tstride, const float* out, long out_bstride,
    long out_tstride, const float* gates, const float* w_hh, const float* dhn, float* dgi_all, float* dgh_shift,
    float* dgh_first, float* dhbuf, float* dgh_tmp, int B, int T, int H, int reverse, float* ws, size_t ws_bytes);
int a2s_staff_emb_bwd_impl(hipStream_t st, const float* note_emb, const float* const* w, float* const* grads_dev, float* note_emb_grad,
    const long long* ids64, const int* ids32, long id_bstride, const long long* lengths, long len_stride,
    const float* dout, long lddo, int col0, const float* hsave, int R, int maxlen, int E, int S);
long a2s_attn_pair_bwd_launches(void);

size_t a2s_note_step_fused_head_floats(void);
size_t a2s_note_step_workspace_floats_impl(int H, int E);
int a2s_dec_mid_launches(void);
bool a2s_dec_step_fusable(int R, int H, int E, int V, const void* const* ptrs, int nptrs, const float* ws, size_t ws_floats, bool greedy = false);
int a2s_note_step_fused_fwd(hipStream_t st, const a2s_note_dec_args& a, int si, int so, int sv, int sv_next, int t, const int* t_base, int tf, bool last,
    int nrows, const int* rowmap, const a2s_attn_deferred* defer = nullptr);
int a2s_note_step_fused_bwd_prepare(hipStream_t st, const a2s_note_dec_bwd_args& a);
int a2s_note_step_fused_bwd(hipStream_t st, const a2s_note_dec_bwd_args& a, int s, const float* dh_in, float* dh_out, const a2s_attn_rows* rows,
    int nrows, const int* rowmap);
bool a2s_note_step_mid_ok(int H, int E, const void* const* ptrs, int nptrs);
int a2s_note_step_mid_gru(hipStream_t st, const a2s_note_dec_args& a, int si, int so, int sv, int sv_next, int nrows, const int* rowmap);
bool a2s_note_step_mid_bwd_ok(const a2s_note_dec_bwd_args& a);
int a2s_note_step_mid_bwd(hipStream_t st, const a2s_note_dec_bwd_args& a, int s, float* dh_out, int nrows, const int* rowmap);
int a2s_note_step_mid_bwd_query(hipStream_t st, const a2s_note_dec_bwd_args& a, int s, float* dh_out, int nrows, const int* rowmap);

bool a2s_grammar_ref_ok(const a2s_grammar_ref& g, int R, int V);
int a2s_grammar_argmax_rows_impl(hipStream_t st, const float* x, long ldx, float* y, long ldy, const signed char* next, int n_states, int* row_state,
    int* choice_out, int R, int V);
int a2s_grammar_step_finalize_impl(hipStream_t st, const StepFinArgs& a, const a2s_grammar_ref& g);
int a2s_grammar_launches_impl(void);

int a2s_attn_align_rows_impl(hipStream_t st, const float* attw, long ldw, int R, int T, int* peak_out, float* weight_out, float* centroid_out,
    long out_stride, const int* n_done = nullptr, int n_rows_total = 0);
int a2s_align_launches_impl(void);
int a2s_note_decoder_fwd_align_impl(hipStream_t st, const a2s_note_dec_args& a, const a2s_align_args& g, int* steps_done);

int a2s_render_notes_impl(hipStream_t st, const int* programs, int rows_per_clip, int n_samples, float* wave, long wave_bstride, int B);
int a2s_render_launches_impl(void);

struct BeamStepArgs {
    const float* logits; long ldl;
    const float* emb;
    float* xnext; long ldx;
    float* h; int h_cols;
    float* q; int q_cols;
    const signed char* next; int n_states; int* row_state;
    float* score; int* finished; int* done_count;
    int* token_hist; int* parent_hist; float* score_hist;
    float* probs_scratch;
    int* n_done; int* steps_exec;
    int B, K, V, E, t, max_t, eos_id, pad_id;
};
struct BeamBackArgs {
    const float* score; const int* token_hist; const int* parent_hist; const float* probs_scratch;
    float* probs; long probs_bstride;
    int* ids_out; long ids_bstride; long long* lengths_out; float* score_out;
    const int* steps_exec;
    float alpha;
    int B, K, V, max_t, eos_id, pad_id;
};
bool a2s_beam_args_ok(const a2s_beam_args& g, int R, int n_clips, int V);
int a2s_beam_init_impl(hipStream_t st, const a2s_beam_args& g, int* n_done, int B, int steps);
int a2s_beam_step_finalize_impl(hipStream_t st, const BeamStepArgs& a);
int a2s_beam_backtrack_impl(hipStream_t st, const BeamBackArgs& a);
int a2s_beam_launches_impl(void);
int a2s_note_decoder_fwd_beam_impl(hipStream_t st, const a2s_note_dec_args& a, const a2s_beam_args& g, int* steps_done);

unsigned* a2s_persist_latch_ptr(void);
void a2s_persist_latch_set(void* p);
a2s_device_geom a2s_device_geometry(void);
bool a2s_gru_seq_fwd_persist_ok(const float* w_hh, const float* gi, int B, int T, int H, float* ws, size_t ws_bytes);
int a2s_gru_seq_fwd_persist_impl(hipStream_t st, const float* gi_all, long gi_bstride, long gi_tstride, const float* w_hh, const float* b_hh, float* out,
    long out_bstride, long out_tstride, float* save, float* hn, int B, int T, int H, int reverse, float* ws, size_t ws_bytes);
bool a2s_gru_seq_bwd_persist_ok(int B, int T, int H, float* ws, size_t ws_bytes, size_t ws_used);
int a2s_gru_seq_bwd_persist_impl(hipStream_t st, const float* dout, long do_bstride, long do_tstride, const float* out, long out_bstride, long out_tstride,
    const float* gates, const float* w_hh_t, const float* dhn, float* dgi_all, float* dgh_shift, float* dgh_first, int B, int T,
    int H, int reverse, float* ws, size_t ws_off, size_t ws_bytes);

int a2s_dec_persist_launches(void);
bool a2s_note_decoder_fwd_persist_ok(const a2s_note_dec_args& a);
int a2s_note_decoder_fwd_persist(hipStream_t st, const a2s_note_dec_args& a, int* steps_done);
bool a2s_note_decoder_bwd_persist_ok(const a2s_note_dec_bwd_args& a);
int a2s_note_decoder_bwd_persist(hipStream_t st, const a2s_note_dec_bwd_args& a);

int a2s_nll_loss_impl(hipStream_t st, const float* logp, const long long* target, long rows, int V, long long ignore_index,
    float* loss_out , float* dlogp , float gscale, double* partial, int nblocks);
int a2s_nll_grad_impl(hipStream_t st, float* dlogp, const long long* target, const float* loss_out, float gscale, long rows, int V, long long ignore_index);
int a2s_clip_adadelta_impl(hipStream_t st, float* params, float* grads, float* square_avg, float* acc_delta, long n, const float* loss,
    float max_norm, float lr, float rho, float eps, float* ctl , double* partial, int nblocks, int zero_grad);

int a2s_edit_distance_max_len_impl(void);
long a2s_edit_distance_launches(void);
int a2s_edit_distance_impl(hipStream_t st, const int* ref, const long long* ref_off, const int* hyp, const long long* hyp_off, const int* order,
    int n_pairs, int max_ref_len, int max_hyp_len, int* dist);

int a2s_vqt_logmag_impl(hipStream_t st, const float* C, float* out, float* partial, int B, long rows, int bins, float top_db);
int a2s_vqt_decimate_impl(hipStream_t st, const float* ypad, long plen, const float* taps, int ntaps, float* out, long n_out, int B);
int a2s_vqt_logmag_octaves_impl(hipStream_t st, const float* C, float* out, float* partial, int B, long rows, int bins, int bpo, float top_db);
```

### piano_a2s_amd/csrc/a2s_linear.hip

```cpp
#include "a2s_internal.h"

#define LIN_BM 128
#define LIN_K 256
#define LIN_RS 288
#define LIN_NTH 512
#define LIN_LDS (2 * 2 * LIN_BM * LIN_RS)

typedef unsigned lu32x4 __attribute__((ext_vector_type(4)));

struct LinDgradArgs {
    const float* A; long lda;
    const unsigned char* planes;
    float* C; long ldc;
    const float* ep_y;
    const float* mean; const float* invstd; const float* scale; const float* shift;
    float* partial;
    const float* a_absmax; const float* b_absmax;
    int M, N, period, channels;
    float* c_absmax_out;
};

__global__ __launch_bounds__(256) void lin_pack_planes_k(const float* __restrict__ W, long ld, int N, int K, const float* __restrict__ absmax,
                                                         unsigned char* __restrict__ out) {
    const long id = (long)blockIdx.x * 256 + threadIdx.x;
// ... 262 lines not shown
    load_b(0, bf[0]);
    auto load_af = [&](const unsigned char* st, int h, int qt, lu32x4 (&af)[2][2]) {
#pragma unroll
        for (int sp = 0; sp < 2; ++sp)
#pragma unroll
            for (int q = 0; q < 2; ++q) af[sp][q] = *reinterpret_cast<const lu32x4*>(st + (sp * LIN_BM + (qt * 2 + q) * 16 + lr) * LF_RS + h * 64 + lk * 16);
    };
    auto multiply = [&](int qt, const lu32x4 (&af)[2][2], const lu32x4 (&b)[4][2]) {
#define LR_PRODUCT(SA, SB)                                                                                                        \
        _Pragma("unroll") for (int nt = 0; nt < 4; ++nt)                                                                          \
            _Pragma("unroll") for (int q = 0; q < 2; ++q)                                                                         \
                acc[qt * 2 + q][nt] = __builtin_amdgcn_mfma_f32_16x16x32_f16(__builtin_bit_cast(f16x8, b[nt][SB]),                \
                                                                             __builtin_bit_cast(f16x8, af[SA][q]), acc[qt * 2 + q][nt], 0, 0, 0);
        LR_PRODUCT(1, 0) LR_PRODUCT(0, 1) LR_PRODUCT(0, 0)
#undef LR_PRODUCT
    };
#pragma unroll 1
    for (int blk = 0; blk < nblk; ++blk) {
        __syncthreads();
        const unsigned char* st = lds + (blk % LF_NS) * LF_STAGE;
        lu32x4 fa[2][2], fb[2][2];
        load_af(st, 0, 0, fa);
        load_b(2 * blk + 1, bf[1]);
        __builtin_amdgcn_sched_barrier(0);
        load_af(st, 0, 1, fb); multiply(0, fa, bf[0]);
        __builtin_amdgcn_sched_barrier(0);
        load_af(st, 0, 2, fa); multiply(1, fb, bf[0]);
        __builtin_amdgcn_sched_barrier(0);
        load_af(st, 0, 3, fb); multiply(2, fa, bf[0]);
        __builtin_amdgcn_sched_barrier(0);
        load_af(st, 1, 0, fa); multiply(3, fb, bf[0]);
        __builtin_amdgcn_sched_barrier(0);
        load_b(2 * blk + 2, bf[0]);
        load_af(st, 1, 1, fb); multiply(0, fa, bf[1]);
        __builtin_amdgcn_sched_barrier(0);
        load_af(st, 1, 2, fa); multiply(1, fb, bf[1]);
        __builtin_amdgcn_sched_barrier(0);
        load_af(st, 1, 3, fb); multiply(2, fa, bf[1]);
        __builtin_amdgcn_sched_barrier(0);
        multiply(3, fb, bf[1]);
        __builtin_amdgcn_sched_barrier(0);
    }
#pragma unroll
    for (int mt = 0; mt < 8; ++mt) {
        const int m = m0 + mt * 16 + lr;
        if (m >= a.M) continue;
#pragma unroll
        for (int nt = 0; nt < 4; ++nt) {
            f32x4 v = acc[mt][nt];
#pragma unroll
            for (int r = 0; r < 4; ++r) v[r] *= unscale;
            *reinterpret_cast<f32x4*>(a.C + (long)m * a.ldc + wave * 64 + nt * 16 + lk * 4) = v;
        }
    }
}

bool a2s_linear_fwd_ok(int M, int N, int K, long lda, long ldc, int period, const void* A, const void* W, const void* C) {
    return N == 256 && M >= 1 && K >= 128 && K % 64 == 0 && (period == 0 || (period % 32 == 0 && K % period == 0)) && lda % 4 == 0 && ldc % 4 == 0 &&
           (((uintptr_t)A | (uintptr_t)W | (uintptr_t)C) % 16 == 0);
}

int a2s_linear_fwd_impl(hipStream_t st, int M, int N, int K, const float* A, long lda, const float* W, float* C, long ldc, const float* a_scale,
                        const float* a_shift, int period, const float* a_absmax, const float* w_absmax, float* ws, size_t ws_bytes) {
    A2S_REQUIRE(A && W && C && w_absmax && ws && ((a_scale == nullptr) == (a_shift == nullptr)), "linear_fwd: null argument");
    A2S_REQUIRE(a2s_linear_fwd_ok(M, N, K, lda, ldc, a_scale ? period : 0, A, W, C),
                "linear_fwd: needs N = 256, K %% 64 == 0, period %% 32 == 0 and 16-byte aligned rows");
    A2S_REQUIRE(((uintptr_t)ws % 16 == 0) && ws_bytes >= (size_t)N * K * 4, "linear_fwd: workspace too small (%zu bytes needed)", (size_t)N * K * 4);
    unsigned char* planes = reinterpret_cast<unsigned char*>(ws);
    hipLaunchKernelGGL(lin_pack_planes_k, dim3((unsigned)(((long)N * (K / 8) + 255) / 256)), dim3(256), 0, st, W, (long)K, N, K, w_absmax, planes);
    A2S_CHECK_LAUNCH("lin_pack_planes_k");
    LinFwdArgs a{A, lda, planes, C, ldc, a_scale, a_shift, a_absmax, w_absmax, M, K, a_scale ? period : K};
    hipLaunchKernelGGL(lin_fwd_roles, dim3((M + LIN_BM - 1) / LIN_BM), dim3(LIN_NTH), 0, st, a);
    A2S_CHECK_LAUNCH("lin_fwd");
    return A2S_OK;
}

struct LinWgradArgs {
    const float* A; long lda;
    const unsigned char* planes;
    float* partial;
    const float* a_scale; const float* a_shift;
    const float* a_absmax; const float* d_absmax;
    int M, K, period, nblk, blk_per_split;
};

__global__ __launch_bounds__(256) void lin_pack_dz_planes(const float* __restrict__ dz, long ld, int M, int nsteps, const float* __restrict__ absmax,
                                                          unsigned char* __restrict__ out) {
    const long id = (long)blockIdx.x * 256 + threadIdx.x;
    const int n = (int)(id & 255), lk = (int)((id >> 8) & 3), s = (int)(id >> 10);
    if (s >= nsteps) return;
    float ps = ldexpf(1.f, pow2_scale_exp(*absmax, 12));
    if ((s >> 3) & 1) ps = -ps;
    float x[8];
#pragma unroll
    for (int j = 0; j < 8; ++j) {
        const int m = s * 32 + lk * 8 + j;
        x[j] = m < M ? __builtin_amdgcn_fmed3f(dz[(long)m * ld + n] * ps, -65000.f, 65000.f) : 0.f;
    }
    lu32x4 hi, lo;
#pragma unroll
    for (int i = 0; i < 4; ++i) { unsigned h, l; split2_pair_f16(x[2 * i], x[2 * i + 1], h, l); hi[i] = h; lo[i] = l; }
    unsigned char* o = out + ((((long)s * 16 + (n >> 4)) * 2) * 64 + (lk * 16 + (n & 15))) * 16;
    *reinterpret_cast<lu32x4*>(o) = hi;
    *reinterpret_cast<lu32x4*>(o + 64 * 16) = lo;
}

__global__ __launch_bounds__(LIN_NTH) void lin_wgrad_roles(LinWgradArgs a) {
    __shared__ __attribute__((aligned(16))) unsigned char lds[LF_NS * LF_STAGE];
    const int tid = threadIdx.x, lane = tid & 63, lr = lane & 15, lk = lane >> 4;
    const int wave = __builtin_amdgcn_readfirstlane(tid >> 6);
    const int k0 = blockIdx.x * LIN_BM;
    const int b_lo = blockIdx.y * a.blk_per_split, b_hi = min(a.nblk, b_lo + a.blk_per_split);
    const int ka = a.a_absmax ? pow2_scale_exp(*a.a_absmax, 12) : 0, kd = pow2_scale_exp(*a.d_absmax, 12);
    const float psa = ldexpf(1.f, ka), unscale = ldexpf(1.f, -(ka + kd));
    const bool affine = a.a_scale != nullptr;
    if (wave >= 4) {
        const int st_ = tid - 256;
        const int rq = st_ & 15, cq0 = st_ >> 4;
        float sc[2], sh[2];
#pragma unroll
        for (int u = 0; u < 2; ++u) {
            const int ch = affine ? (k0 + 4 * (cq0 + 16 * u)) / a.period : 0;
            sc[u] = affine ? a.a_scale[ch] * psa : psa; sh[u] = affine ? a.a_shift[ch] * psa : 0.f;
        }
        const float floor_ = affine ? 0.f : -INFINITY;
        f32x4 ar[2][8];
        auto issue_a = [&](int blk, f32x4 (&r)[8]) {
#pragma unroll
            for (int u = 0; u < 2; ++u)
#pragma unroll
                for (int j = 0; j < 4; ++j) {
                    const int m = blk * 64 + 4 * rq + j;
                    r[4 * u + j] = (f32x4){0.f, 0.f, 0.f, 0.f};
                    if (m < a.M && blk < b_hi) r[4 * u + j] = __builtin_nontemporal_load(reinterpret_cast<const f32x4*>(a.A + (long)m * a.lda + k0 + 4 * (cq0 + 16 * u)));
                }
        };
        auto commit_a = [&](int blk, const f32x4 (&r)[8]) {
            if (blk >= b_hi) return;
            unsigned char* st = lds + (blk % LF_NS) * LF_STAGE;
#pragma unroll
            for (int u = 0; u < 2; ++u)
#pragma unroll
                for (int c = 0; c < 4; ++c) {
                    float x[4];
#pragma unroll
                    for (int j = 0; j < 4; ++j) x[j] = __builtin_amdgcn_fmed3f(fmaxf(fmaf(r[4 * u + j][c], sc[u], sh[u]), floor_), -65000.f, 65000.f);
                    uint2 hi, lo;
                    split2_pair_f16(x[0], x[1], hi.x, lo.x);
                    split2_pair_f16(x[2], x[3], hi.y, lo.y);
                    *reinterpret_cast<uint2*>(st + (0 * LIN_BM + 4 * (cq0 + 16 * u) + c) * LF_RS + rq * 8) = hi;
                    *reinterpret_cast<uint2*>(st + (1 * LIN_BM + 4 * (cq0 + 16 * u) + c) * LF_RS + rq * 8) = lo;
                }
        };
        if (b_lo < b_hi) {
            issue_a(b_lo, ar[0]);
            commit_a(b_lo, ar[0]);
            issue_a(b_lo + 1, ar[1]); issue_a(b_lo + 2, ar[0]);
        }
#pragma unroll 1
        for (int b = b_lo; b < b_hi; b += 2) {
            __syncthreads();
            commit_a(b + 1, ar[1]); issue_a(b + 3, ar[1]);
            if (b + 1 < b_hi) {
                __syncthreads();
                commit_a(b + 2, ar[0]); issue_a(b + 4, ar[0]);
            }
        }
        return;
    }
    lu32x4 df[2][4][2];
    auto load_d = [&](int step, lu32x4 (&dst)[4][2]) {
        if (step >= 2 * b_hi) return;
#pragma unroll
        for (int nt = 0; nt < 4; ++nt)
#pragma unroll
            for (int sp = 0; sp < 2; ++sp)
                dst[nt][sp] = *reinterpret_cast<const lu32x4*>(a.planes + ((((long)step) * 16 + wave * 4 + nt) * 2 + sp) * 1024 + (unsigned)lane * 16u);
    };
    f32x4 acc[8][4];
#pragma unroll
    for (int kt = 0; kt < 8; ++kt)
#pragma unroll
        for (int nt = 0; nt < 4; ++nt) acc[kt][nt] = (f32x4){0.f, 0.f, 0.f, 0.f};
    bool neg = false;
    auto flip = [&]() {
#pragma unroll
        for (int kt = 0; kt < 8; ++kt)
#pragma unroll
            for (int nt = 0; nt < 4; ++nt)
#pragma unroll
                for (int r = 0; r < 4; ++r) acc[kt][nt][r] = -acc[kt][nt][r];
    };
    auto load_bf = [&](const unsigned char* st, int h, int qt, lu32x4 (&f)[2][2]) {
#pragma unroll
        for (int sp = 0; sp < 2; ++sp)
#pragma unroll
            for (int q = 0; q < 2; ++q) f[sp][q] = *reinterpret_cast<const lu32x4*>(st + (sp * LIN_BM + (qt * 2 + q) * 16 + lr) * LF_RS + h * 64 + lk * 16);
    };
    auto multiply = [&](int qt, const lu32x4 (&f)[2][2], const lu32x4 (&d)[4][2]) {
#define LW_PRODUCT(SX, SD)                                                                                                        \
        _Pragma("unroll") for (int nt = 0; nt < 4; ++nt)                                                                          \
            _Pragma("unroll") for (int q = 0; q < 2; ++q)                                                                         \
                acc[qt * 2 + q][nt] = __builtin_amdgcn_mfma_f32_16x16x32_f16(__builtin_bit_cast(f16x8, f[SX][q]),                 \
                                                                             __builtin_bit_cast(f16x8, d[nt][SD]), acc[qt * 2 + q][nt], 0, 0, 0);
        LW_PRODUCT(1, 0) LW_PRODUCT(0, 1) LW_PRODUCT(0, 0)
#undef LW_PRODUCT
    };
    load_d(2 * b_lo, df[0]);
#pragma unroll 1
    for (int blk = b_lo; blk < b_hi; ++blk) {
        const bool want = ((2 * blk) >> 3) & 1;
        if (want != neg) { flip(); neg = want; }
        __syncthreads();
        const unsigned char* st = lds + (blk % LF_NS) * LF_STAGE;
        lu32x4 fa[2][2], fb[2][2];
        load_bf(st, 0, 0, fa);
        load_d(2 * blk + 1, df[1]);
        __builtin_amdgcn_sched_barrier(0);
        load_bf(st, 0, 1, fb); multiply(0, fa, df[0]);
        __builtin_amdgcn_sched_barrier(0);
        load_bf(st, 0, 2, fa); multiply(1, fb, df[0]);
        __builtin_amdgcn_sched_barrier(0);
        load_bf(st, 0, 3, fb); multiply(2, fa, df[0]);
        __builtin_amdgcn_sched_barrier(0);
        load_bf(st, 1, 0, fa); multiply(3, fb, df[0]);
        __builtin_amdgcn_sched_barrier(0);
        load_d(2 * blk + 2, df[0]);
        load_bf(st, 1, 1, fb); multiply(0, fa, df[1]);
        __builtin_amdgcn_sched_barrier(0);
        load_bf(st, 1, 2, fa); multiply(1, fb, df[1]);
        __builtin_amdgcn_sched_barrier(0);
        load_bf(st, 1, 3, fb); multiply(2, fa, df[1]);
        __builtin_amdgcn_sched_barrier(0);
        multiply(3, fb, df[1]);
        __builtin_amdgcn_sched_barrier(0);
    }
    if (neg) flip();
    float* slab = a.partial + (long)blockIdx.y * 256 * a.K;
#pragma unroll
    for (int kt = 0; kt < 8; ++kt)
#pragma unroll
        for (int nt = 0; nt < 4; ++nt) {
            f32x4 v = acc[kt][nt];
#pragma unroll
            for (int r = 0; r < 4; ++r) v[r] *= unscale;
            *reinterpret_cast<f32x4*>(slab + (long)(wave * 64 + nt * 16 + lr) * a.K + k0 + kt * 16 + lk * 4) = v;
        }
}

__global__ __launch_bounds__(256) void lin_wgrad_reduce(const float* __restrict__ partial, int splits, long n, float* __restrict__ G, long ldg, int K) {
    const long i = ((long)blockIdx.x * 256 + threadIdx.x) * 4;
    if (i >= n) return;
    f32x4 s = *reinterpret_cast<const f32x4*>(partial + i);
    for (int p = 1; p < splits; ++p) {
        const f32x4 v = *reinterpret_cast<const f32x4*>(partial + (long)p * n + i);
#pragma unroll
        for (int r = 0; r < 4; ++r) s[r] += v[r];
    }
    float* g = G + (i / K) * ldg + (i % K);
    const f32x4 o = *reinterpret_cast<const f32x4*>(g);
#pragma unroll
    for (int r = 0; r < 4; ++r) s[r] += o[r];
    *reinterpret_cast<f32x4*>(g) = s;
}

static int lin_wgrad_splits(int M, int K) {
    const int ncol = K / LIN_BM, nblk = (M + 63) / 64;
    int s = (768 + ncol - 1) / ncol;
    if (s > 16) s = 16;
    if (s > nblk) s = nblk;
    return s < 1 ? 1 : s;
}
size_t a2s_linear_wgrad_ws_bytes_impl(int M, int K) {
    if (M < 1 || K < LIN_BM || K % LIN_BM) return 0;
    const size_t nsteps = 2 * (size_t)((M + 63) / 64);
    return nsteps * 16 * 2 * 1024 + (size_t)lin_wgrad_splits(M, K) * 256 * K * sizeof(float);
}
bool a2s_linear_wgrad_ok(int M, int N, int K, long ldz, long lda, long ldg, int period, const void* dz, const void* A, const void* G) {
    return N == 256 && M >= 64 && K >= LIN_BM && K % LIN_BM == 0 && (period == 0 || (period % 4 == 0 && K % period == 0)) && lda % 4 == 0 && ldg % 4 == 0 && ldz >= 256 &&
           (((uintptr_t)dz | (uintptr_t)A | (uintptr_t)G) % 16 == 0);
}
int a2s_linear_wgrad_impl(hipStream_t st, int M, int N, int K, const float* dz, long ldz, const float* A, long lda, float* G, long ldg, const float* a_scale,
                          const float* a_shift, int period, const float* dz_absmax, const float* a_absmax, float* ws, size_t ws_bytes) {
    A2S_REQUIRE(dz && A && G && dz_absmax && ws && ((a_scale == nullptr) == (a_shift == nullptr)), "linear_wgrad: null argument");
    A2S_REQUIRE(a2s_linear_wgrad_ok(M, N, K, ldz, lda, ldg, a_scale ? period : 0, dz, A, G), "linear_wgrad: needs N = 256, K %% 128 == 0, period %% 4 == 0, 16-byte aligned rows");
    A2S_REQUIRE(((uintptr_t)ws % 16 == 0) && ws_bytes >= a2s_linear_wgrad_ws_bytes_impl(M, K), "linear_wgrad: workspace too small (%zu bytes needed)",
                a2s_linear_wgrad_ws_bytes_impl(M, K));
    const int nblk = (M + 63) / 64, nsteps = 2 * nblk, splits = lin_wgrad_splits(M, K);
    unsigned char* planes = reinterpret_cast<unsigned char*>(ws);
    float* partial = reinterpret_cast<float*>(planes + (size_t)nsteps * 16 * 2 * 1024);
    hipLaunchKernelGGL(lin_pack_dz_planes, dim3((unsigned)(((long)nsteps * 1024 + 255) / 256)), dim3(256), 0, st, dz, ldz, M, nsteps, dz_absmax, planes);
    A2S_CHECK_LAUNCH("lin_pack_dz_planes");
    LinWgradArgs a{A, lda, planes, partial, a_scale, a_shift, a_absmax, dz_absmax, M, K, a_scale ? period : K, nblk, (nblk + splits - 1) / splits};
    hipLaunchKernelGGL(lin_wgrad_roles, dim3(K / LIN_BM, splits), dim3(LIN_NTH), 0, st, a);
    A2S_CHECK_LAUNCH("lin_wgrad");
    const long n = 256L * K;
    hipLaunchKernelGGL(lin_wgrad_reduce, dim3((unsigned)((n / 4 + 255) / 256)), dim3(256), 0, st, partial, splits, n, G, ldg, K);
    A2S_CHECK_LAUNCH("lin_wgrad_reduce");
    return A2S_OK;
}
```

### piano_a2s_amd/csrc/a2s_persist.hip

```cpp
#include "a2s_internal.h"

typedef unsigned long long u64;
typedef __attribute__((address_space(1))) u64 gu64;
typedef __attribute__((address_space(1))) unsigned gu32;
#define RLX_AGENT __ATOMIC_RELAXED, __HIP_MEMORY_SCOPE_AGENT
#define SPIN_LIMIT (1u << 21)

__device__ __forceinline__ u64 granule_load(const u64* g) {
    return __hip_atomic_load((gu64*)(const_cast<u64*>(g)), RLX_AGENT);
}
__device__ __forceinline__ bool aborted(unsigned* flag) {
    return __hip_atomic_load((gu32*)(flag), RLX_AGENT) != 0;
}
__device__ __forceinline__ void raise_abort(unsigned* flag, unsigned code) {
    __hip_atomic_store((gu32*)(flag), code, RLX_AGENT);
}

typedef unsigned u32x4_t __attribute__((ext_vector_type(4)));
__device__ __forceinline__ void granule_put(u64* g, unsigned tag, float v, bool same_xcd) {
    const u64 x = ((u64)tag << 32) | (u64)__float_as_uint(v);
    if (same_xcd) __hip_atomic_store((gu64*)(g), x, __ATOMIC_RELAXED, __HIP_MEMORY_SCOPE_WORKGROUP);
    else __hip_atomic_store((gu64*)(g), x, RLX_AGENT);
}
__device__ __forceinline__ long granule_index(int r, int k) { return ((long)((k >> 4) * 64 + ((k & 15) >> 2) * 16 + r) << 2) + (k & 3); }
// ... 124 lines not shown
            }
            __syncthreads();
            if (wave == 0) {
#pragma unroll
                for (int g = 0; g < 3; ++g)
#pragma unroll
                    for (int w = 0; w < 3; ++w) {
                        const f32x4 o = part[(w * 3 + g) * 64 + lane];
#pragma unroll
                        for (int r = 0; r < 4; ++r) acc[g][r] += o[r];
                    }
            }
            __syncthreads();
        }
        if (wave == 0) {
            u64* gout = a.hx + (long)(s & 1) * par + by * TILE;
#pragma unroll
            for (int r = 0; r < 4; ++r) {
                const int row = row0 + lk * 4 + r;
                const float ghn = acc[2][r] + bn;
                const float rg = fast_sigmoid(gir[r] + acc[0][r] + br);
                const float zg = fast_sigmoid(giz[r] + acc[1][r] + bz);
                const float ng = fast_tanh(gin[r] + rg * ghn);
                const float hnew = (1.f - zg) * ng + zg * hp[r];
                hp[r] = hnew;
                if (s + 1 < a.T) granule_put(gout + granule_index(lk * 4 + r, j), (unsigned)(s + 1), hnew, same_xcd);
                if (row < R) {
                    a.out[(long)row * a.out_bstride + (long)t * a.out_tstride + j] = hnew;
                    if (a.save) {
                        float* sv = a.save + ((long)t * R + row) * 4 * H;
                        sv[j] = rg; sv[H + j] = zg; sv[2 * H + j] = ng; sv[3 * H + j] = ghn;
                    }
                }
            }
        }
    }
    if (wave == 0) {
        const bool bad = dead || aborted(a.abort_flag);
#pragma unroll
        for (int r = 0; r < 4; ++r) {
            const int row = row0 + lk * 4 + r;
            if (row < R) a.hn[(long)row * H + j] = bad ? __builtin_nanf("") : hp[r];
        }
        if (bad && lane == 0 && a.latch) atomicOr(a.latch, 1u);
    }
}

struct GruPersistBwd {
    const float* dout; long do_bstride, do_tstride;
    const float* out; long out_bstride, out_tstride;
    const float* gates;
    const float* w_hh_t;
    const float* dhn;
    float* dgi_all; float* dgh_shift; float* dgh_first;
    u64* gx;
    unsigned* abort_flag;
    unsigned* xcc;
    int B, T, reverse, nrb;
    unsigned* latch; unsigned dbg;
};

template <int H>
__global__ __launch_bounds__(256, 2) void gru_seq_bwd_persist(GruPersistBwd a) {
    constexpr int KS = 3 * H / 64;
    __shared__ f32x4 part[3 * 64];
    int bx, by;
    persist_block(H / 16, a.nrb, bx, by);
    const int j0 = bx * 16, row0 = by * 16;
    const int tid = threadIdx.x, lane = tid & 63, wave = tid >> 6;
    const int li = lane & 15, lk = lane >> 4;
    const int j = j0 + li, R = a.B, T = a.T;
    if ((a.dbg & PERSIST_DBG_INJECT_ABORT) && blockIdx.x == 0 && tid == 0) raise_abort(a.abort_flag, 99u);
    const bool same_xcd = wave == 0 && row_block_on_one_xcd(a.xcc + by * 16, bx, H / 16, lane, a.abort_flag) && !(a.dbg & PERSIST_DBG_FORCE_AGENT);
    if (tid == 0 && same_xcd) atomicAdd(a.abort_flag + 1, 1u);
    f32x4 bw[KS];
#pragma unroll
    for (int c = 0; c < KS; ++c) bw[c] = *reinterpret_cast<const f32x4*>(a.w_hh_t + (long)(j0 + li) * 3 * H + 16 * (wave + 4 * c) + 4 * lk);
    constexpr long TILE = 16L * 3 * H;
    const long par = (long)a.nrb * TILE;
    float carry[4];
#pragma unroll
    for (int r = 0; r < 4; ++r) carry[r] = (wave == 0 && a.dhn) ? a.dhn[(long)min(row0 + lk * 4 + r, R - 1) * H + j] : 0.f;
    bool dead = false;
    for (int s = T - 1; s >= 0; --s) {
        const int t = a.reverse ? T - 1 - s : s;
        const int tp = a.reverse ? t + 1 : t - 1;
        float dov[4], rg[4], zg[4], ng[4], ghn[4], hp[4];
        if (wave == 0) {
#pragma unroll
            for (int r = 0; r < 4; ++r) {
                const int row = min(row0 + lk * 4 + r, R - 1);
                dov[r] = a.dout[(long)row * a.do_bstride + (long)t * a.do_tstride + j];
                const float* sv = a.gates + ((long)t * R + row) * 4 * H;
                rg[r] = sv[j]; zg[r] = sv[H + j]; ng[r] = sv[2 * H + j]; ghn[r] = sv[3 * H + j];
                hp[r] = s > 0 ? a.out[(long)row * a.out_bstride + (long)tp * a.out_tstride + j] : 0.f;
            }
        }
        f32x4 acc = {0.f, 0.f, 0.f, 0.f};
        if (s < T - 1) {
            const __amdgpu_buffer_rsrc_t rs = tile_rsrc(a.gx + (long)((s + 1) & 1) * par + by * TILE, (unsigned)(TILE * 8));
            const unsigned tag = (unsigned)(T - 1 - s);
            if (!dead && !wait_tile<KS>(rs, wave, lane, tag, a.abort_flag, 2u)) dead = true;
            f32x4 acc2 = {0.f, 0.f, 0.f, 0.f};
            constexpr int NG = KS / 3;
#define A2S_BPTT_GROUP(G)                                                                                                   \
            if (!dead) {                                                                                                    \
                float av[NG][4];                                                                                            \
                if (!gather_tile<G * NG, NG>(rs, wave, lane, tag, av, a.abort_flag, 2u)) dead = true;                       \
                else {                                                                                                      \
                    _Pragma("unroll") for (int c = 0; c < NG; ++c) {                                                        \
                        acc = __builtin_amdgcn_mfma_f32_16x16x4f32(av[c][0], bw[G * NG + c][0], acc, 0, 0, 0);              \
                        acc2 = __builtin_amdgcn_mfma_f32_16x16x4f32(av[c][1], bw[G * NG + c][1], acc2, 0, 0, 0);            \
                        acc = __builtin_amdgcn_mfma_f32_16x16x4f32(av[c][2], bw[G * NG + c][2], acc, 0, 0, 0);              \
                        acc2 = __builtin_amdgcn_mfma_f32_16x16x4f32(av[c][3], bw[G * NG + c][3], acc2, 0, 0, 0);            \
                    }                                                                                                       \
                }                                                                                                           \
            }
            A2S_BPTT_GROUP(0)
            A2S_BPTT_GROUP(1)
            A2S_BPTT_GROUP(2)
#undef A2S_BPTT_GROUP
#pragma unroll
            for (int r = 0; r < 4; ++r) acc[r] += acc2[r];
            if (wave > 0) part[(wave - 1) * 64 + lane] = acc;
            __syncthreads();
            if (wave == 0) {
#pragma unroll
                for (int r = 0; r < 4; ++r) acc[r] += part[lane][r] + part[64 + lane][r] + part[128 + lane][r];
            }
            __syncthreads();
        }
        if (wave == 0) {
            u64* gout = a.gx + (long)(s & 1) * par + by * TILE;
            const unsigned tag = (unsigned)(T - s);
#pragma unroll
            for (int r = 0; r < 4; ++r) {
                const int row = row0 + lk * 4 + r;
                const float dh = carry[r] + acc[r] + dov[r];
                const float dn = dh * (1.f - zg[r]) * (1.f - ng[r] * ng[r]);
                const float dz = dh * (hp[r] - ng[r]) * zg[r] * (1.f - zg[r]);
                const float dr = dn * ghn[r] * rg[r] * (1.f - rg[r]);
                const float dnr = dn * rg[r];
                carry[r] = dh * zg[r];
                if (s > 0) {
                    const int rr = lk * 4 + r;
                    granule_put(gout + granule_index(rr, j), tag, dr, same_xcd);
                    granule_put(gout + granule_index(rr, H + j), tag, dz, same_xcd);
                    granule_put(gout + granule_index(rr, 2 * H + j), tag, dnr, same_xcd);
                }
                if (row < R) {
                    float* gi = a.dgi_all + ((long)row * T + t) * 3 * H;
                    gi[j] = dr; gi[H + j] = dz; gi[2 * H + j] = dn;
                    if (s > 0) { float* g2 = a.dgh_shift + ((long)row * T + tp) * 3 * H; g2[j] = dr; g2[H + j] = dz; g2[2 * H + j] = dnr; }
                    else { float* g1 = a.dgh_first + (long)row * 3 * H; g1[j] = dr; g1[H + j] = dz; g1[2 * H + j] = dnr; }
                }
            }
        }
    }
    if (wave == 0 && (dead || aborted(a.abort_flag))) {
#pragma unroll
        for (int r = 0; r < 4; ++r) {
            const int row = row0 + lk * 4 + r;
            if (row < R) a.dgh_first[(long)row * 3 * H + j] = __builtin_nanf("");
        }
        if (lane == 0 && a.latch) atomicOr(a.latch, 2u);
    }
}

static size_t a2s_gru_persist_ws_bytes(int B, int H, int bwd) {
    if (H != 256 || B < 1) return 0;
    const size_t rb = (size_t)(B + 15) / 16;
    return 256 + ((rb * 16 * sizeof(unsigned) + 255) & ~(size_t)255) + sizeof(u64) * 2 * rb * 16 * (size_t)(bwd ? 3 * H : H);
}
static unsigned* g_abort_latch = nullptr;
unsigned* a2s_persist_latch_ptr(void) { return g_abort_latch; }
void a2s_persist_latch_set(void* p) { g_abort_latch = reinterpret_cast<unsigned*>(p); }
a2s_device_geom a2s_device_geometry(void) {
    static a2s_device_geom cache[16];
    static bool have[16];
    int dev = 0;
    if (hipGetDevice(&dev) != hipSuccess || dev < 0 || dev >= 16) return a2s_device_geom{0, 0};
    if (!have[dev]) {
        int cus = 0, xccs = 0;
        if (hipDeviceGetAttribute(&cus, hipDeviceAttributeMultiprocessorCount, dev) != hipSuccess) cus = 0;
        if (hipDeviceGetAttribute(&xccs, hipDeviceAttributeNumberOfXccs, dev) != hipSuccess) xccs = 0;
        (void)hipGetLastError();
        cache[dev] = a2s_device_geom{cus, xccs};
        have[dev] = true;
    }
    return cache[dev];
}
template <typename K>
static int persist_blocks_per_cu(K kernel) {
    int n = 0;
    if (hipOccupancyMaxActiveBlocksPerMultiprocessor(&n, kernel, 256, 0) != hipSuccess) { (void)hipGetLastError(); n = 0; }
    return n;
}
static bool persist_fits(int B, int H, bool bwd) {
    static int occ[2] = {-1, -1};
    if (occ[bwd] < 0) occ[bwd] = bwd ? persist_blocks_per_cu(gru_seq_bwd_persist<256>) : persist_blocks_per_cu(gru_seq_fwd_persist<256>);
    const a2s_device_geom g = a2s_device_geometry();
    return (a2s_sw(A2S_SW_gru_persist_alone) ? 1L : 2L) * (H / 16) * ((B + 15) / 16) <= (long)g.cus * occ[bwd];
}

bool a2s_gru_seq_fwd_persist_ok(const float* w_hh, const float* gi, int B, int T, int H, float* ws, size_t ws_bytes) {
    return a2s_sw(A2S_SW_gru_persist) && H == 256 && T >= 2 && persist_fits(B, H, false) && ws && ((uintptr_t)ws % 256 == 0) && ws_bytes >= a2s_gru_persist_ws_bytes(B, H, 0) &&
           ((uintptr_t)w_hh % 16 == 0) && gi;
}
int a2s_gru_seq_fwd_persist_impl(hipStream_t st, const float* gi_all, long gi_bstride, long gi_tstride, const float* w_hh, const float* b_hh, float* out,
                                 long out_bstride, long out_tstride, float* save, float* hn, int B, int T, int H, int reverse, float* ws, size_t ws_bytes) {
    const size_t need = a2s_gru_persist_ws_bytes(B, H, 0);
    A2S_REQUIRE(need && ws_bytes >= need, "gru_seq_fwd_persist: workspace too small");
    hipError_t e = hipMemsetAsync(ws, 0, need, st);
    if (e != hipSuccess) A2S_FAIL(A2S_ERR_HIP, "gru_seq_fwd_persist memset: %s", hipGetErrorString(e));
    const int nrb = a2s_cdiv(B, 16);
    char* base = reinterpret_cast<char*>(ws);
    const size_t xcc_bytes = ((size_t)nrb * 16 * sizeof(unsigned) + 255) & ~(size_t)255;
    GruPersistFwd a{gi_all, gi_bstride, gi_tstride, w_hh, b_hh, out, out_bstride, out_tstride, save, hn,
                    reinterpret_cast<u64*>(base + 256 + xcc_bytes), reinterpret_cast<unsigned*>(base), reinterpret_cast<unsigned*>(base + 256), B, T, reverse, nrb,
                    g_abort_latch, a2s_persist_dbg()};
    hipLaunchKernelGGL(gru_seq_fwd_persist<256>, dim3((H / 16) * nrb), dim3(256), 0, st, a);
    A2S_CHECK_LAUNCH("gru_seq_fwd_persist");
    return A2S_OK;
}

bool a2s_gru_seq_bwd_persist_ok(int B, int T, int H, float* ws, size_t ws_bytes, size_t ws_used) {
    return a2s_sw(A2S_SW_gru_persist) && H == 256 && T >= 2 && persist_fits(B, H, true) && ws && ((uintptr_t)ws % 256 == 0) && ws_used % 256 == 0 &&
           ws_bytes >= ws_used + a2s_gru_persist_ws_bytes(B, H, 1);
}
int a2s_gru_seq_bwd_persist_impl(hipStream_t st, const float* dout, long do_bstride, long do_tstride, const float* out, long out_bstride, long out_tstride,
                                 const float* gates, const float* w_hh_t, const float* dhn, float* dgi_all, float* dgh_shift, float* dgh_first, int B, int T,
                                 int H, int reverse, float* ws, size_t ws_off, size_t ws_bytes) {
    const size_t need = a2s_gru_persist_ws_bytes(B, H, 1);
    A2S_REQUIRE(need && ws_bytes >= ws_off + need, "gru_seq_bwd_persist: workspace too small");
    char* base = reinterpret_cast<char*>(ws) + ws_off;
    hipError_t e = hipMemsetAsync(base, 0, need, st);
    if (e != hipSuccess) A2S_FAIL(A2S_ERR_HIP, "gru_seq_bwd_persist memset: %s", hipGetErrorString(e));
    const int nrb = a2s_cdiv(B, 16);
    const size_t xcc_bytes = ((size_t)nrb * 16 * sizeof(unsigned) + 255) & ~(size_t)255;
    GruPersistBwd a{dout, do_bstride, do_tstride, out, out_bstride, out_tstride, gates, w_hh_t, dhn, dgi_all, dgh_shift, dgh_first,
                    reinterpret_cast<u64*>(base + 256 + xcc_bytes), reinterpret_cast<unsigned*>(base), reinterpret_cast<unsigned*>(base + 256), B, T, reverse, nrb,
                    g_abort_latch, a2s_persist_dbg()};
    hipLaunchKernelGGL(gru_seq_bwd_persist<256>, dim3((H / 16) * nrb), dim3(256), 0, st, a);
    A2S_CHECK_LAUNCH("gru_seq_bwd_persist");
    return A2S_OK;
}
```

### piano_a2s_amd/engine_bwd.py

```python
import ctypes as C
import os
import threading

import torch

from . import hip
from .spec import SOS, VOCAB_SIZE

NULL = C.c_void_p(0)


def _os_env(name, default):
    return os.environ.get(name, default)


def _ptr(t, off=0):
    return C.c_void_p(t.data_ptr() + 4 * off)


_COLSUM_WS = {}


def _colsum(x, ld, out, rows, ncol, x_off=0, out_off=0, beta=1.0):
    ws = None
# ... 344 lines not shown
            ldxb = tokw + H2
            dgi, dgh = torch.empty((Bg, 3 * H2), device=dev), torch.empty((Bg, 3 * H2), device=dev)
            dhp = torch.empty((Bg, H2), device=dev)
            hip.check(L.a2s_gru_gates_bwd(hip.stream(), hip._p(d_hnew), C.c_long(H2), NULL, C.c_long(0), hip._p(b["gates"]), hip._p(b["hprev"]), C.c_long(H2),
                                          hip._p(dgi), C.c_long(3 * H2), hip._p(dgh), C.c_long(3 * H2), NULL, C.c_long(0), hip._p(dhp), C.c_long(H2), Bg, H2),
                      "gates bwd bar")
            d_xbar = torch.empty((Bg, ldxb), device=dev)
            _linear_bwd(b["xbar"], S["decoder.gru.weight_ih_l0"], dgi, Gg, "decoder.gru.weight_ih_l0", "decoder.gru.bias_ih_l0", dx=d_xbar)
            _linear_bwd(b["hprev"], S["decoder.gru.weight_hh_l0"], dgh, Gg, "decoder.gru.weight_hh_l0", "decoder.gru.bias_hh_l0", dx=dhp, dx_beta=1.0)
            dq, ds = torch.empty((Bg, H), device=dev), torch.empty((1, Bg, T), device=dev)
            dctx = torch.empty((1, Bg, H2), device=dev)
            from .engine import bar_attn_workspace
            bar_ws = bar_attn_workspace(dev, gidx, Bg, T, H)
            if bar_ws is not None:
                ctx_c, dctx_c = b["xbar"][:, tokw:].contiguous(), d_xbar[:, tokw:].contiguous()
                hip.check(L.a2s_attn_step_bwd(hip.stream(), hip._p(keys_g["decoder"]), hip._p(enc_g), hip._p(b["qb"]), C.c_long(H), hip._p(S["decoder.attn.v.weight"]),
                                              hip._p(b["attw"]), hip._p(ctx_c), C.c_long(H2), hip._p(dctx_c), C.c_long(H2), _ptr(d_headin, H2),
                                              C.c_long(4 * H), hip._p(dctx), C.c_long(H2), hip._p(dq), C.c_long(H), hip._p(ds), Bg, T, H, hip._p(bar_ws)), "attn bwd bar")
            else:
                hip.check(L.a2s_attn_step_bwd(hip.stream(), hip._p(keys_g["decoder"]), hip._p(enc_g), hip._p(b["qb"]), C.c_long(H), hip._p(S["decoder.attn.v.weight"]),
                                              hip._p(b["attw"]), _ptr(b["xbar"], tokw), C.c_long(ldxb), _ptr(d_xbar, tokw), C.c_long(ldxb), _ptr(d_headin, H2),
                                              C.c_long(4 * H), hip._p(dctx), C.c_long(H2), hip._p(dq), C.c_long(H), hip._p(ds), Bg, T, H, NULL), "attn bwd bar")
            Wa = S["decoder.attn.attn.weight"]
            hip.gemm(dq, H, 1, Wa, 4 * H, 1, dhp, H2, Bg, H2, H, beta=1.0)
            hip.gemm(dq, 1, H, b["hprev"], H2, 1, Gg["decoder.attn.attn.weight"], 4 * H, H, H2, Bg, beta=1.0)
            _colsum(dq, H, Gg["decoder.attn.attn.bias"], Bg, H)
            bar_attn.append((b["qb"].view(1, Bg, H), ds, b["attw"].view(1, Bg, T), dctx))
            d_hid_carry = dhp
            d_token = d_xbar[:, :tokw].contiguous()
            if b["keep"] is not None:
                d_token = d_token * b["keep"] / 0.9
            d_token_next = d_token
        qs, dss, aws, dcs = [torch.cat(t, 0) for t in zip(*bar_attn)]
        _attn_deferred(eng, S, Gg, "decoder.attn", keys_g["decoder"], enc_g, qs, dss, aws, dcs, dK_g["decoder"], dEnc_g, Bg, T, H, len(bar_attn))
        d_sos = d_token_next.clone()
        d_sos[:, :2 * Sz] += d_sos[:, 2 * Sz:4 * Sz]
        _staff_token_bwd(eng, S, Gg, gs["sos_rec"][0], d_sos)
        for table, cid, col, width in (("decoder.time_sig_emb.weight", cfg["num_time_sig"], 4 * Sz, te), ("decoder.key_emb.weight", cfg["num_keys"], 4 * Sz + te, ke)):
            hip.check(L.a2s_embed_scatter_add(hip.stream(), hip._p(Gg[table]), NULL, NULL, C.c_long(0), cid, hip._p(d_token_next), C.c_long(tokw), col, Bg, width,
                                              NULL, hip.f32(1.0)), "scatter sos ts/key")
        d_hidden[b0:b1].copy_(d_hid_carry)
        for ev in deferred_done:
            torch.cuda.current_stream().wait_event(ev)
        return None


    def finish(self, grad_ready=None):
        eng, S, G, dev = self.eng, self.S, self.G, self.dev
        B, T, F = self.B, self.T, self.F
        names, offs, total, flat = self.names, self.offs, self.total, self.flat
        dEnc, dK = self.dEnc, self.dK
        sv = eng.saved
        assert sv["training"], "backward needs a forward run with training=True (batch statistics / saved activations)"
        L = hip.lib()
        H = eng.cfg["hidden_size"]
        H2 = 2 * H
        enc = sv["enc_out"]
        G["__staff_emb_ptrs__"] = self.group_ptrs[0]
        late_join = None
        if self.late:
            dec_lo = next(off for k, off in zip(names, offs) if k.startswith("decoder."))
            assert all(k.startswith("decoder.") for k, off in zip(names, offs) if off >= dec_lo), "the decoder's parameters must be the tail of the flat layout"
            wg = _weight_grad_stream(dev)
            wg.wait_stream(torch.cuda.current_stream())
            with torch.cuda.stream(wg):
                for fn, ev, tensors in self.late:
                    wg.wait_event(ev)
                    for t in tensors:
                        if t is not None:
                            t.record_stream(wg)
                    fn()
            late_join = dec_lo
            self.late = []
        else:
            for gf in self.group_flat[1:]:
                flat.add_(gf)
        d_hid_carry = self.d_hidden
        if self.concurrent:
            dEnc.add_(self.dEnc_staff[0]).add_(self.dEnc_staff[1])
        enc2d = enc.view(B * T, H2)
        enc_amax = hip.absmax(enc) if self.two_term else None
        for p, dKp in dK.items():
            Wn = p + ".attn.attn.weight"
            sk = L.a2s_gemm_pick_splitk(H, H2, B * T, 1)
            dk_amax = hip.absmax(dKp) if self.two_term else None
            hip.gemm(dKp, 1, H, enc2d, H2, 1, G[Wn], 4 * H, H, H2, B * T, beta=1.0, splitk=sk, c_off=H2,
                     two_term=(dk_amax, enc_amax) if self.two_term else None)
            hip.gemm(dKp, H, 1, S[Wn], 4 * H, 1, dEnc, H2, B * T, H2, H, beta=1.0, b_off=H2,
                     two_term=(dk_amax, hip.absmax(S[Wn])) if self.two_term else None)
        if late_join is not None:
            wg = _weight_grad_stream(dev)
            wg.wait_stream(torch.cuda.current_stream())
            with torch.cuda.stream(wg):
                for gf in self.group_flat[1:]:
                    flat[late_join:].add_(gf[late_join:])
                if Backward.check_fold:
                    for gi, gf in enumerate(self.group_flat[1:], 1):
                        assert not bool(gf[:late_join].any()), f"clip group {gi}: non-decoder gradients in the group buffer would be lost by the late fold"
        defer = True
        d_conv = _encoder_bwd(eng, S, G, sv["enc"], dEnc, d_hid_carry, B, T, wait_weight_grads=not defer)
        n_conv = next(off for k, off in zip(names, offs) if not k.startswith("convstack."))
        if grad_ready is not None:
            if defer:
                with torch.cuda.stream(_weight_grad_stream(dev)):
                    grad_ready(self.flat_full, n_conv, total + 1)
            else:
                grad_ready(self.flat_full, n_conv, total + 1)
        if getattr(eng, "conv_unperm", None) is not None:
            d_conv = d_conv.reshape(B, T, -1).index_select(0, eng.conv_unperm)
        _convstack_bwd(eng, S, G, sv["conv"], d_conv, B, T, F)
        if defer:
            torch.cuda.current_stream().wait_stream(_weight_grad_stream(dev))
        if grad_ready is not None:
            grad_ready(flat, 0, n_conv)
        G[None] = flat
        G["__loss_gate__"] = self.flat_full[total:]
        eng._keep_alive = self.keep_alive
        return G




def backward(eng, S, grad_outputs, grad_ready=None, loss_total=None):
    from .engine import group_views, run_clip_groups
    sv = eng.saved
    assert sv["training"], "backward needs a forward run with training=True (batch statistics / saved activations)"
    dev = sv["enc_out"].device
    clip_groups = sv.get("clip_groups") or [(0, sv["shape"][0])]
    ctx = Backward(eng, S, sv["shape"], dev, clip_groups, sv.get("concurrent"), sv.get("bar_major"))
    dts, dkey, dup, dlo = [g.contiguous() for g in grad_outputs]

    def group(gidx):
        b0, b1 = clip_groups[gidx]
        if ctx.bar_major:
            dup_g, dlo_g = group_views(dup, clip_groups, gidx), group_views(dlo, clip_groups, gidx)
        else:
            dup_g, dlo_g = dup[b0:b1], dlo[b0:b1]
        ctx.decoder_group(gidx, sv["groups"][gidx], dts[b0:b1], dkey[b0:b1], dup_g, dlo_g)

    run_clip_groups(dev, [lambda gi=gi: group(gi) for gi in range(len(clip_groups))])
    if loss_total is not None:
        ctx.flat_full[ctx.total:].copy_(loss_total.reshape(1))
    return ctx.finish(grad_ready)


_WG_STREAMS = {}
_DEFERRED_STREAMS = {}


def _deferred_streams(dev, group=0):
    idx = torch.device(dev).index if torch.device(dev).index is not None else torch.cuda.current_device()
    key = (idx, group)
    if key not in _DEFERRED_STREAMS:
        _DEFERRED_STREAMS[key] = (torch.cuda.Stream(device=idx), torch.cuda.Stream(device=idx))
    return _DEFERRED_STREAMS[key]



def _weight_grad_stream(dev):
    from .engine import group_stream
    return group_stream(dev, 1)


def _encoder_bwd(eng, S, G, es, dEnc, d_hidden, B, T, wait_weight_grads=True):
    L = hip.lib()
    H = eng.cfg["hidden_size"]
    dev = dEnc.device
    W = S["encoder.fc.weight"]
    dpre = torch.empty_like(d_hidden)
    hip.check(L.a2s_ew_act_bwd(hip.stream(), hip._p(d_hidden), hip._p(es["hidden"]), hip._p(dpre), C.c_long(dpre.numel()), 2), "tanh bwd")
    dhn = []
    for l in (0, 1):
        for half, hfin in enumerate((es["finals"][2 * l], es["finals"][2 * l + 1])):
            d = torch.empty((B, H), device=dev)
            hip.gemm(dpre, 2 * H, 1, W, 2 * H, 1, d, H, B, H, H, a_off=l * H, b_off=half * H)
            hip.gemm(dpre, 1, 2 * H, hfin, H, 1, G["encoder.fc.weight"], 2 * H, H, H, B, beta=1.0, a_off=l * H, c_off=half * H)
            dhn.append(d)
        _colsum(dpre, 2 * H, G["encoder.fc.bias"], B, H, x_off=l * H)
    gws = [hip.gemm_workspace(B, dev), hip.gemm_workspace(B, dev)]
    two_term = True
    in_amax = hip.absmax(es["layers"][0]["in"]) if two_term else None
    dout = dEnc
    for layer in (1, 0):
        ls = es["layers"][layer]
        inp = ls["in"]
        I = inp.shape[1]
        out = ls["out"]
        dX = torch.empty((B * T, I), device=dev)
        from .engine import encoder_streams, fork_on_streams
        streams = encoder_streams(dev, B)

        def direction(d, sfx):
            dgi = torch.empty((B, T, 3 * H), device=dev)
            dghs = torch.empty((B, T, 3 * H), device=dev)
            dgh_first, dhbuf, dgh_tmp = torch.empty((B, 3 * H), device=dev), torch.empty((2, B, H), device=dev), torch.empty((B, 3 * H), device=dev)
            hip.check(L.a2s_gru_seq_bwd(hip.stream(), _ptr(dout, d * H), C.c_long(T * 2 * H), C.c_long(2 * H), _ptr(out, d * H), C.c_long(T * 2 * H),
                                        C.c_long(2 * H), hip._p(ls["dirs"][d]["gates"]), hip._p(S[f"encoder.gru.weight_hh_{sfx}"]), hip._p(dhn[2 * layer + d]),
                                        hip._p(dgi), hip._p(dghs), hip._p(dgh_first), hip._p(dhbuf), hip._p(dgh_tmp), B, T, H, d, hip._p(gws[d]),
                                        C.c_size_t(gws[d].numel() * 4)), "a2s_gru_seq_bwd")
            return (dgi, dghs, dgh_first, dhbuf, dgh_tmp)

        res = fork_on_streams(dev, streams, [lambda d=d, sfx=sfx: direction(d, sfx) for d, sfx in enumerate((f"l{layer}", f"l{layer}_reverse"))])()
        dgi_amax = []
        for d, sfx in enumerate((f"l{layer}", f"l{layer}_reverse")):
            dgi2 = res[d][0].view(B * T, 3 * H)
            Wih = S[f"encoder.gru.weight_ih_{sfx}"]
            tt = (hip.absmax(dgi2), hip.absmax(Wih)) if two_term else None
            dgi_amax.append(tt[0] if tt else None)
            if L.a2s_debug_get(b"gemm_bf16x3") > 0:
                hip.gemm(dgi2, 3 * H, 1, Wih.t().contiguous(), 1, 3 * H, dX, I, B * T, I, 3 * H, beta=0.0 if d == 0 else 1.0, two_term=tt)
            else:
                hip.gemm(dgi2, 3 * H, 1, Wih, I, 1, dX, I, B * T, I, 3 * H, beta=0.0 if d == 0 else 1.0, two_term=tt)
        wg = _weight_grad_stream(dev)
        ev = torch.cuda.Event()
        ev.record()
        wg.wait_event(ev)
        for d, sfx in enumerate((f"l{layer}", f"l{layer}_reverse")):
            dgi, dghs, dgh_first = res[d][:3]
            for t in (dgi, dghs, dgh_first, dgi_amax[d], in_amax):
                if t is not None:
                    t.record_stream(wg)
            with torch.cuda.stream(wg):
                dgi2, dghs2 = dgi.view(B * T, 3 * H), dghs.view(B * T, 3 * H)
                _linear_bwd(inp, S[f"encoder.gru.weight_ih_{sfx}"], dgi2, G, f"encoder.gru.weight_ih_{sfx}", f"encoder.gru.bias_ih_{sfx}",
                            dy_amax=dgi_amax[d], x_bound=(in_amax if layer == 0 else hip.one(dev)) if two_term else None)
                sk = L.a2s_gemm_pick_splitk(3 * H, H, B * T, 1)
                hip.gemm(dghs2, 1, 3 * H, out, 2 * H, 1, G[f"encoder.gru.weight_hh_{sfx}"], H, 3 * H, H, B * T, beta=1.0, splitk=sk, b_off=d * H,
                         two_term=(hip.absmax(dghs2), hip.one(dev)) if two_term else None)
                _colsum(dghs2, 3 * H, G[f"encoder.gru.bias_hh_{sfx}"], B * T, 3 * H)
                _colsum(dgh_first, 3 * H, G[f"encoder.gru.bias_hh_{sfx}"], B, 3 * H)
        dout = dX.view(B, T, I)
    if wait_weight_grads:
        torch.cuda.current_stream().wait_stream(_weight_grad_stream(dev))
    return dout


_FUSE_BN_APPLY = False
_FUSE_BN_APPLY_L1 = True
_DGRAD_BNSTATS = True
_SYNC_FUSED = True
_LIN_WGRAD_AT = "before"
_FUSE_BN_ROWS = os.environ.get("A2S_FUSE_BN_ROWS", "1") != "0"


def _linear_dgrad_generic(L, dev, rows, F, Cf, dz, Wout, da, y4, bn4, dz_amax, w_amax):
    nblk = L.a2s_gemm_bnstats_blocks(rows, F)
    part = torch.empty((nblk, 40, 2), dtype=torch.float32, device=dev)
    if L.a2s_debug_get(b"gemm_bf16x3") > 0:
        Wt = Wout.t().contiguous()
        wb, s_bk, s_bn = Wt, 1, Cf
    else:
        wb, s_bk, s_bn = Wout, 40 * F, 1
    hip.check(L.a2s_gemm_f32_bnstats_scaled(hip.stream(), rows, 40 * F, Cf, hip._p(dz), C.c_long(Cf), C.c_long(1), hip._p(wb), C.c_long(s_bk), C.c_long(s_bn),
                                            hip._p(da), C.c_long(40 * F), hip._p(y4), hip._p(bn4[0]), hip._p(bn4[1]), hip._p(bn4[2]), hip._p(bn4[3]), F,
                                            hip._p(part), hip._p(dz_amax), hip._p(w_amax)), "a2s_gemm_f32_bnstats_scaled")
    return part, nblk


def _convstack_bwd(eng, S, G, cs, d_out, B, T, F):
    L = hip.lib()
    dev = d_out.device
    Cf = eng.cfg["conv_feature_size"]
    rows = B * T

    def bn_bwd(g, x, bn, name, mask, n_rows, C_, F_, stats_only=False, partial=None, amax=None):
        mean, invstd, scale, shift = bn
        if partial is not None and eng.sync_bn and stats_only:
            import torch.distributed as dist
            local = torch.empty(2 * C_, dtype=torch.float32, device=dev)
            hip.check(L.a2s_bn_bwd_sums_from_partial(hip.stream(), hip._p(partial[0]), partial[1], C_, hip._p(local)), "a2s_bn_bwd_sums_from_partial")
            glob = local.clone()
            dist.all_reduce(glob)
            c12 = torch.empty(2 * C_, dtype=torch.float32, device=dev)
            hip.check(L.a2s_bn_bwd_c12_from_sums(hip.stream(), hip._p(local), hip._p(glob), C.c_double(eng.bn_counts[name]), hip._p(G[name + ".weight"]),
                                                 hip._p(G[name + ".bias"]), hip._p(c12), C_), "a2s_bn_bwd_c12_from_sums")
            return c12
        if partial is not None and not eng.sync_bn:
            c12 = torch.empty(2 * C_, dtype=torch.float32, device=dev)
            hip.check(L.a2s_bn_bwd_from_partial_amax(hip.stream(), hip._p(g), hip._p(x), hip._p(mean), hip._p(invstd), hip._p(scale), hip._p(shift),
                                                     hip._p(G[name + ".weight"]), hip._p(G[name + ".bias"]), NULL if stats_only else hip._p(g),
                                                     hip._p(partial[0]), partial[1], hip._p(c12), C.c_long(n_rows), C_, F_, hip._p(amax)),
                      "a2s_bn_bwd_from_partial")
            return c12 if stats_only else g
        part = torch.empty(L.a2s_bn_bwd_partial_floats(C.c_long(n_rows), C_, F_), dtype=torch.float32, device=dev)
        c12 = torch.empty(2 * C_, dtype=torch.float32, device=dev)
        if eng.sync_bn:
            import torch.distributed as dist
            local = torch.empty(2 * C_, dtype=torch.float32, device=dev)
            hip.check(L.a2s_bn_bwd_stats(hip.stream(), hip._p(g), hip._p(x), hip._p(mean), hip._p(invstd), hip._p(scale), hip._p(shift), hip._p(mask),
                                         hip.f32(1.0 / 0.8), hip._p(part), hip._p(local), C.c_long(n_rows), C_, F_), "a2s_bn_bwd_stats")
            glob = local.clone()
            dist.all_reduce(glob)
            hip.check(L.a2s_bn_bwd_apply(hip.stream(), hip._p(g), hip._p(x), hip._p(mean), hip._p(invstd), hip._p(scale), hip._p(shift), hip._p(mask),
                                         hip.f32(1.0 / 0.8), hip._p(local), hip._p(glob), C.c_double(eng.bn_counts[name]), hip._p(G[name + ".weight"]),
                                         hip._p(G[name + ".bias"]), hip._p(g), hip._p(c12), C.c_long(n_rows), C_, F_), "a2s_bn_bwd_apply")
            return g
        hip.check(L.a2s_bn_bwd_amax(hip.stream(), hip._p(g), hip._p(x), hip._p(mean), hip._p(invstd), hip._p(scale), hip._p(shift), hip._p(mask), hip.f32(1.0 / 0.8),
                                    hip._p(G[name + ".weight"]), hip._p(G[name + ".bias"]), NULL if stats_only else hip._p(g), hip._p(part), hip._p(c12),
                                    C.c_long(n_rows), C_, F_, hip._p(amax)), "a2s_bn_bwd")
        return c12 if stats_only else g

    g = d_out.reshape(rows, Cf).contiguous()
    dz_amax = torch.zeros(1, dtype=torch.float32, device=dev)
    dz = bn_bwd(g, cs["z"], cs["out_bn"], "convstack.out_bn", cs["drop"], rows, Cf, 1, amax=dz_amax)
    if eng.sync_bn:
        hip.absmax(dz, dz_amax)
    w_amax = cs.get("w_out_amax")
    a4 = cs["a4"]
    g_partial = None
    g_amax = None
    Wout = S["convstack.out.weight"]
    if a4 is None:
# ... 99 lines not shown
```

### piano_a2s_amd/hip.py

```python
import ctypes as C
import os

import torch

from .build import LIB

LIB = os.environ.get("A2S_LIB", LIB)

_lib = None


class A2SError(RuntimeError):
    pass


class NoteDecArgs(C.Structure):
    _fields_ = [(n, C.c_void_p) for n in (
        "attn_w", "attn_b", "attn_v", "w_ih", "w_hh", "b_ih", "b_hh", "out_w", "out_b", "emb", "keys", "enc",
        "h", "x", "q", "gates", "attw", "o", "gh", "gi", "logits")] + [
        ("probs", C.c_void_p), ("probs_bstride", C.c_long),
        ("gt", C.c_void_p), ("gt_bstride", C.c_long),
        ("tf_flags", C.c_void_p),
        ("drop", C.c_void_p), ("inv_keep", C.c_float),
        ("argmax_out", C.c_void_p), ("am_bstride", C.c_long),
        ("eos_seen", C.c_void_p), ("lengths", C.c_void_p), ("n_done", C.c_void_p), ("steps_exec", C.c_void_p), ("attn_ws", C.c_void_p),
        ("gemm_ws", C.c_void_p), ("gemm_ws_bytes", C.c_size_t), ("t_base", C.c_void_p), ("clip_order", C.c_void_p), ("clip_rank", C.c_void_p),
        ("row_until", C.c_void_p), ("n_active", C.c_void_p), ("n_clips", C.c_int), ("m_active", C.c_void_p),
        ("row_list", C.c_void_p), ("n_rows_active", C.c_void_p),
        ("R", C.c_int), ("T", C.c_int), ("H", C.c_int), ("E", C.c_int), ("V", C.c_int),
        ("steps", C.c_int), ("poll", C.c_int), ("eos_id", C.c_int), ("use_graph", C.c_int),
        ("step_ws", C.c_void_p), ("step_ws_floats", C.c_size_t),
        ("tf_flags_dev", C.c_void_p), ("persist_ws", C.c_void_p), ("persist_ws_bytes", C.c_size_t)]


class BeamArgs(C.Structure):
    _fields_ = [("K", C.c_int), ("alpha", C.c_float), ("next_state", C.c_void_p), ("n_states", C.c_int), ("pad_id", C.c_int)] + [
        (n, C.c_void_p) for n in ("row_state", "score", "finished", "done_count", "token_hist", "parent_hist", "score_hist", "probs_scratch",
                                  "ids_out", "lengths_out", "score_out")]


class AlignArgs(C.Structure):
    _fields_ = [("attw_step", C.c_void_p), ("peak", C.c_void_p), ("weight", C.c_void_p), ("centroid", C.c_void_p), ("out_stride", C.c_long),
                ("next_state", C.c_void_p), ("n_states", C.c_int), ("row_state", C.c_void_p)]


class NoteDecBwdArgs(C.Structure):
    _fields_ = [(n, C.c_void_p) for n in (
        "attn_w", "attn_v", "w_ih", "w_hh", "keys", "enc", "h", "x", "q", "gates", "attw", "do_all",
        "dgi_all", "dgh_all", "dq_all", "ds_all", "dctx_all", "dx", "dh", "attn_ws", "gemm_ws")] + [
        ("gemm_ws_bytes", C.c_size_t), ("clip_order", C.c_void_p), ("clip_rank", C.c_void_p), ("row_until", C.c_void_p),
        ("n_active", C.c_void_p), ("n_clips", C.c_int), ("m_active", C.c_void_p), ("row_list", C.c_void_p), ("n_rows_active", C.c_void_p),
        ("R", C.c_int), ("T", C.c_int), ("H", C.c_int), ("E", C.c_int), ("steps", C.c_int),
        ("step_ws", C.c_void_p), ("step_ws_floats", C.c_size_t), ("persist_ws", C.c_void_p), ("persist_ws_bytes", C.c_size_t), ("w_ih_full", C.c_void_p)]


def lib():
    global _lib
    if _lib is None:
        if not os.path.exists(LIB):
            raise A2SError(f"HIP extension not built: {LIB} is missing (run `python __graft_entry__.py build`). "
                           "There is no CPU fallback for the transcription hot path.")
        arith = os.environ.get("A2S_ARITH", "f16x2")
        if arith not in ("f16x2", "bf16x3", "f32"):
            raise A2SError(f"A2S_ARITH={arith!r}: expected f16x2, bf16x3 or f32")
        L = C.CDLL(LIB)
        L.a2s_last_error.restype = C.c_char_p
        L.a2s_launch_count.restype = C.c_longlong
        for fn in ("a2s_note_step_workspace_floats", "a2s_note_decoder_persist_ws_bytes", "a2s_note_decoder_bwd_persist_ws_bytes", "a2s_linear_dgrad_ws_bytes", "a2s_linear_wgrad_ws_bytes", "a2s_gemm_workspace_bytes", "a2s_bn_bwd_partial_floats", "a2s_conv3x3_wgrad_workspace_bytes", "a2s_attn_workspace_floats", "a2s_attn_workspace_floats_fused",
                   "a2s_conv3x3_workspace_floats"):
            getattr(L, fn).restype = C.c_size_t
        if hasattr(L, "a2s_env_check") and L.a2s_env_check() != 0:
            raise A2SError(L.a2s_last_error().decode())
        if hasattr(L, "a2s_edit_distance"):
            L.a2s_edit_distance.argtypes = [C.c_void_p] * 6 + [C.c_int] * 3 + [C.c_void_p]
        if hasattr(L, "a2s_attn_denc_accum"):
            L.a2s_attn_denc_accum.argtypes = [C.c_void_p] * 4 + [C.c_int] * 4 + [C.c_void_p, C.c_int]
        if arith != "f16x2":
            for key in (b"conv_f16x2", b"wgrad_f16x2", b"gemm_f16x2"):
                L.a2s_debug_set(key, 0)
        if arith == "f32":
            for key in (b"conv_bf16x3", b"gemm_bf16x3", b"wgrad_bf16x3"):
                L.a2s_debug_set(key, 0)
        _lib = L
    return _lib


LINEAR_KERNELS = os.environ.get("A2S_LINEAR_KERNELS", "1") != "0"

_ABORT_LATCH = {}
PERSIST_ABORTS = 0


def abort_latch(device):
    idx = torch.device(device).index if torch.device(device).index is not None else torch.cuda.current_device()
    t = _ABORT_LATCH.get(idx)
    if t is None:
        t = _ABORT_LATCH[idx] = torch.zeros(1, dtype=torch.int32, device=torch.device("cuda", idx))
        _ABORT_LATCH["registered"] = None
    if _ABORT_LATCH.get("registered") != idx:
        check(lib().a2s_persist_abort_latch(C.c_void_p(t.data_ptr())), "a2s_persist_abort_latch")
        _ABORT_LATCH["registered"] = idx
    return t


_LATCH_READS = {}


def post_persist_abort_read(device):
    idx = torch.device(device).index if torch.device(device).index is not None else torch.cuda.current_device()
    e = _LATCH_READS.get(idx)
    if e is None:
        e = _LATCH_READS[idx] = [torch.zeros(1, dtype=torch.int32).pin_memory(), None]
    if e[1] is not None:
        e[1].synchronize()
        _consume_latch_read(e, device, False)
    e[0].copy_(abort_latch(device), non_blocking=True)
    ev = torch.cuda.Event()
    ev.record()
    e[1] = ev


def poll_persist_abort(device, raise_error=False):
    idx = torch.device(device).index if torch.device(device).index is not None else torch.cuda.current_device()
    e = _LATCH_READS.get(idx)
    if e is None:
        return check_persist_abort(device, raise_error)
    if e[1] is None or not e[1].query():
        return 0
    return _consume_latch_read(e, device, raise_error)


def _consume_latch_read(e, device, raise_error):
    e[1] = None
    bits = int(e[0][0])
    if not bits:
        return 0
    return _persist_abort_seen(bits, abort_latch(device), raise_error)


def check_persist_abort(device, raise_error=False):
    t = abort_latch(device)
    bits = int(t.item())
    if not bits:
        return 0
    return _persist_abort_seen(bits, t, raise_error)


def _persist_abort_seen(bits, t, raise_error):
    global PERSIST_ABORTS
    t.zero_()
    PERSIST_ABORTS += 1
    L = lib()
    L.a2s_debug_set(b"gru_persist", 0)
    L.a2s_debug_set(b"dec_persist", 0)
    os.environ["A2S_DEC_PERSIST"] = "0"
    os.environ["A2S_GRU_PERSIST"] = "0"
    msg = (f"a persistent kernel gave up a bounded wait (latch bits {bits:#x}: 1/2 encoder fwd/bwd, 4/8 note decoder fwd/bwd); its outputs were "
           "poisoned with NaN and the persistent paths are switched off for the rest of this process (launch-per-step kernels from now on)")
    if raise_error:
# ... 205 lines not shown
         bias=bias, act=act, beta=beta, a_affine=x_affine, two_term=two_term)
    return out


def conv3x3_forward(x, w, y, scale, shift, partial, cws, in_absmax=None, out_absmax=None):
    B, T, Cin, F = x.shape
    check(lib().a2s_conv3x3_ranged(stream(), _p(x), _p(w), _p(y), _p(scale), _p(shift), _p(in_absmax), _p(partial), _p(out_absmax),
                                   B, T, F, Cin, y.shape[2], _p(cws)), "a2s_conv3x3_ranged")


def conv3x3_dgrad_for_test(dy, w, yl):
    L = lib()
    B, T, Cout, F = dy.shape
    Cin = w.shape[1]
    dev = dy.device
    dx = torch.full((B, T, Cin, F), float("nan"), device=dev)
    amax = absmax(dy)
    part = torch.zeros(L.a2s_conv3x3_stat_blocks(B, T, F, Cout), Cin, 2, device=dev)
    cws = conv_workspace(Cout, dev)
    zeros, ones = torch.zeros(Cin, device=dev), torch.ones(Cin, device=dev)
    check(L.a2s_conv3x3_dgrad_bnstats_scaled(stream(), _p(dy), _p(w), _p(dx), _p(yl), _p(zeros), _p(ones), _p(ones), _p(zeros), _p(part),
                                             B, T, F, Cout, Cin, _p(cws), _p(amax)), "a2s_conv3x3_dgrad_bnstats_scaled")
    torch.cuda.synchronize()
    return dx


def act_bound(scale, shift, x_absmax):
    out = torch.empty(1, dtype=torch.float32, device=scale.device)
    check(lib().a2s_act_bound(stream(), _p(scale), _p(shift), _p(x_absmax), scale.numel(), _p(out)), "a2s_act_bound")
    return out


def conv3x3_wgrad(dy, x, scale, shift, dW, ws, dy_absmax, act_absmax):
    B, T, Cout, F = dy.shape
    Cin = x.shape[2]
    check(lib().a2s_conv3x3_wgrad_ranged(stream(), _p(dy), _p(x), _p(scale), _p(shift), _p(dW), _p(ws), C.c_size_t(ws.numel() * 4), B, T, F, Cin, Cout,
                                          _p(dy_absmax), _p(act_absmax)), "a2s_conv3x3_wgrad_ranged")


def conv3x3_wgrad_for_test(dy, x, scale, shift):
    L = lib()
    B, T, Cout, F = dy.shape
    Cin = x.shape[2]
    dev = dy.device
    dW = torch.zeros(Cout, Cin, 3, 3, device=dev)
    ws = torch.empty(L.a2s_conv3x3_wgrad_workspace_bytes(Cin, Cout) // 4, device=dev)
    bound = act_bound(scale, shift, x.abs().amax(dim=(0, 1, 3)).contiguous())
    conv3x3_wgrad(dy, x, scale, shift, dW, ws, absmax(dy), bound)
    torch.cuda.synchronize()
    return dW


def linear_forward(x2d, weight, x_affine, x_bound, w_absmax, out=None):
    M, K = x2d.shape
    N = weight.shape[0]
    L = lib()
    period = x_affine[2]
    if (LINEAR_KERNELS and x2d.is_contiguous() and weight.is_contiguous() and x_bound is not None
            and L.a2s_linear_fwd_eligible(M, N, K, period)):
        if out is None:
            out = torch.empty((M, N), dtype=torch.float32, device=x2d.device)
        nb = L.a2s_linear_dgrad_ws_bytes(N, K)
        ws = torch.empty(nb // 4, dtype=torch.float32, device=x2d.device)
        check(L.a2s_linear_fwd(stream(), M, N, K, _p(x2d), C.c_long(K), _p(weight), _p(out), C.c_long(N), _p(x_affine[0]), _p(x_affine[1]), period,
                               _p(x_bound), _p(w_absmax), _p(ws), C.c_size_t(nb)), "a2s_linear_fwd")
        return out
    return linear(x2d, weight, out=out, x_affine=x_affine, two_term=(x_bound, w_absmax))


def linear_wgrad(dz, x2d, x_affine, dz_absmax, x_bound, G):
    M, K = x2d.shape
    N = dz.shape[1]
    L = lib()
    if (not LINEAR_KERNELS or not (x2d.is_contiguous() and dz.is_contiguous() and G.is_contiguous()) or dz_absmax is None
            or x_bound is None or not L.a2s_linear_wgrad_eligible(M, N, K, x_affine[2])):
        return False
    nb = L.a2s_linear_wgrad_ws_bytes(M, K)
    ws = torch.empty(nb // 4, dtype=torch.float32, device=x2d.device)
    check(L.a2s_linear_wgrad(stream(), M, N, K, _p(dz), C.c_long(N), _p(x2d), C.c_long(K), _p(G), C.c_long(K), _p(x_affine[0]), _p(x_affine[1]), x_affine[2],
                             _p(dz_absmax), _p(x_bound), _p(ws), C.c_size_t(nb)), "a2s_linear_wgrad")
    return True


def linear_forward_for_test(x, w, aff):
    period = aff[2]
    xmax = x.view(x.shape[0], -1, period).abs().amax(dim=(0, 2)).contiguous()
    return linear_forward(x, w, aff, act_bound(aff[0], aff[1], xmax), absmax(w))
```

Before: 626.6.

## Add tall-K wgrad path with fused bias for encoder GRU weight gradients

Adds a tall-K weight-gradient kernel path, reusing the linear wgrad roles kernel with plane-split batching. It fuses the bias column-sum into the A-operand commit and supports a transposed reduce. The GRU sequence backward can now emit absmax ranges of dgi and dghs directly, so separate absmax launches are skipped. This replaces the generic linear_bwd, split-K gemm and colsum calls for weight_ih and weight_hh gradients, at the cost of a new workspace and eligibility checks.

```diff
diff --git a/include/a2s.h b/include/a2s.h
--- a/include/a2s.h
+++ b/include/a2s.h
@@ -41,6 +41,10 @@
                      const float* shift, int period, const float* dz_absmax, const float* y_absmax, float* workspace, size_t workspace_bytes);
 size_t a2s_linear_wgrad_ws_bytes(int M, int K);
 int a2s_linear_wgrad_eligible(int M, int N, int K, int period);
+int a2s_tallk_wgrad(void* stream, int M, int Np, int K, const float* P, long ldp, const float* A, long lda, float* G, long ldg, int transposed, float* bias,
+                    const float* p_absmax, const float* a_absmax, float* workspace, size_t workspace_bytes);
+size_t a2s_tallk_wgrad_ws_bytes(int M, int Np, int K);
+int a2s_tallk_wgrad_eligible(int M, int Np, int K, long ldp, long lda, long ldg, int transposed);
 size_t a2s_linear_dgrad_ws_bytes(int N, int K);
 int a2s_linear_dgrad_blocks(int M);
 int a2s_linear_dgrad_eligible(int M, int N, int K, int period);
@@ -229,6 +233,10 @@
 int a2s_gru_seq_bwd(void* stream, const float* dout, long do_bstride, long do_tstride, const float* out, long out_bstride,
                     long out_tstride, const float* gates, const float* w_hh, const float* dhn, float* dgi_all, float* dgh_shift,
                     float* dgh_first, float* dhbuf, float* dgh_tmp, int B, int T, int H, int reverse, float* workspace, size_t workspace_bytes);
+int a2s_gru_seq_bwd_ranged(void* stream, const float* dout, long do_bstride, long do_tstride, const float* out, long out_bstride,
+                           long out_tstride, const float* gates, const float* w_hh, const float* dhn, float* dgi_all, float* dgh_shift,
+                           float* dgh_first, float* dhbuf, float* dgh_tmp, int B, int T, int H, int reverse, float* workspace, size_t workspace_bytes,
+                           float* ranges_out, int* ranges_valid);
 int a2s_staff_emb_bwd(void* stream, const float* note_emb, const float* const* gru_w, float* const* grads, float* note_emb_grad,
                       const long long* ids64, const int* ids32, long id_bstride, const long long* lengths, long len_stride,
                       const float* dout, long lddo, int col0, const float* hsave, int R, int maxlen, int E, int S);
diff --git a/piano_a2s_amd/csrc/a2s_api.hip b/piano_a2s_amd/csrc/a2s_api.hip
--- a/piano_a2s_amd/csrc/a2s_api.hip
+++ b/piano_a2s_amd/csrc/a2s_api.hip
@@ -58,6 +58,14 @@
 }
 size_t a2s_linear_wgrad_ws_bytes(int M, int K) { return a2s_linear_wgrad_ws_bytes_impl(M, K); }
 int a2s_linear_wgrad_eligible(int M, int N, int K, int period) { return a2s_linear_wgrad_ok(M, N, K, 256, 4, 4, period, nullptr, nullptr, nullptr) ? 1 : 0; }
+int a2s_tallk_wgrad(void* stream, int M, int Np, int K, const float* P, long ldp, const float* A, long lda, float* G, long ldg, int transposed, float* bias,
+                    const float* p_absmax, const float* a_absmax, float* workspace, size_t workspace_bytes) {
+    return a2s_tallk_wgrad_impl(ST, M, Np, K, P, ldp, A, lda, G, ldg, transposed, bias, p_absmax, a_absmax, workspace, workspace_bytes);
+}
+size_t a2s_tallk_wgrad_ws_bytes(int M, int Np, int K) { return a2s_tallk_wgrad_ws_bytes_impl(M, Np, K); }
+int a2s_tallk_wgrad_eligible(int M, int Np, int K, long ldp, long lda, long ldg, int transposed) {
+    return a2s_tallk_wgrad_ok(M, Np, K, ldp, lda, ldg, transposed, nullptr, nullptr, nullptr, nullptr) ? 1 : 0;
+}
 int a2s_linear_fwd_eligible(int M, int N, int K, int period) { return a2s_linear_fwd_ok(M, N, K, 4, 4, period, nullptr, nullptr, nullptr) ? 1 : 0; }
 int a2s_linear_dgrad_blocks(int M) { return a2s_linear_dgrad_blocks_impl(M); }
 int a2s_linear_dgrad_eligible(int M, int N, int K, int period) {
@@ -78,6 +86,8 @@
     const int id = a2s_switch_find(key);
     if (id >= 0) { a2s_switch_store(id, value); return A2S_OK; }
     if (!strcmp(key, "attn_deferred_fast")) { a2s_attn_deferred_fast = value ? 1 : 0; return A2S_OK; }
+    if (!strcmp(key, "tallk_wgrad")) { a2s_tallk_wgrad_on = value ? 1 : 0; return A2S_OK; }
+    if (!strcmp(key, "tallk_wgrad_max_splits")) { a2s_tallk_wgrad_max_splits = value > 0 ? value : 0; return A2S_OK; }
     if (!strcmp(key, "gemm_tile")) { a2s_gemm_debug_tile_impl(value); return A2S_OK; }
     snprintf(a2s_err_msg, sizeof(a2s_err_msg), "a2s_debug_set: unknown key %s", key);
     return A2S_ERR_ARG;
@@ -97,6 +107,9 @@
     if (!strcmp(key, "attn_pair_launches")) return (int)a2s_attn_pair_launches();
     if (!strcmp(key, "attn_pair_bwd_launches")) return (int)a2s_attn_pair_bwd_launches();
     if (!strcmp(key, "attn_deferred_fast")) return a2s_attn_deferred_fast;
+    if (!strcmp(key, "tallk_wgrad")) return a2s_tallk_wgrad_on;
+    if (!strcmp(key, "tallk_wgrad_max_splits")) return a2s_tallk_wgrad_max_splits;
+    if (!strcmp(key, "tallk_wgrad_launches")) return (int)a2s_tallk_wgrad_launches();
     if (!strcmp(key, "attn_dk_ahead_launches")) return (int)a2s_attn_dk_ahead_launches();
     if (!strcmp(key, "attn_denc_launches")) return (int)a2s_attn_denc_launches();
     if (!strcmp(key, "dec_mid_launches")) return a2s_dec_mid_launches();
@@ -302,7 +315,15 @@
                     const float* gates, const float* w_hh, const float* dhn, float* dgi_all, float* dgh_shift, float* dgh_first,
                     float* dhbuf, float* dgh_tmp, int B, int T, int H, int reverse, float* workspace, size_t workspace_bytes) {
     return a2s_gru_seq_bwd_impl(ST, dout, do_bstride, do_tstride, out, out_bstride, out_tstride, gates, w_hh, dhn, dgi_all, dgh_shift,
-                                dgh_first, dhbuf, dgh_tmp, B, T, H, reverse, workspace, workspace_bytes);
+                                dgh_first, dhbuf, dgh_tmp, B, T, H, reverse, workspace, workspace_bytes, nullptr, nullptr);
+}
+int a2s_gru_seq_bwd_ranged(void* stream, const float* dout, long do_bstride, long do_tstride, const float* out, long out_bstride, long out_tstride,
+                           const float* gates, const float* w_hh, const float* dhn, float* dgi_all, float* dgh_shift, float* dgh_first,
+                           float* dhbuf, float* dgh_tmp, int B, int T, int H, int reverse, float* workspace, size_t workspace_bytes,
+                           float* ranges_out, int* ranges_valid) {
+    if (!ranges_out || !ranges_valid) { snprintf(a2s_err_msg, sizeof(a2s_err_msg), "gru_seq_bwd_ranged: null ranges_out / ranges_valid"); return A2S_ERR_ARG; }
+    return a2s_gru_seq_bwd_impl(ST, dout, do_bstride, do_tstride, out, out_bstride, out_tstride, gates, w_hh, dhn, dgi_all, dgh_shift,
+                                dgh_first, dhbuf, dgh_tmp, B, T, H, reverse, workspace, workspace_bytes, ranges_out, ranges_valid);
 }
 int a2s_staff_emb_bwd(void* stream, const float* note_emb, const float* const* gru_w, float* const* grads, float* note_emb_grad,
                       const long long* ids64, const int* ids32, long id_bstride, const long long* lengths, long len_stride,
diff --git a/piano_a2s_amd/csrc/a2s_bwd.hip b/piano_a2s_amd/csrc/a2s_bwd.hip
--- a/piano_a2s_amd/csrc/a2s_bwd.hip
+++ b/piano_a2s_amd/csrc/a2s_bwd.hip
@@ -579,8 +579,10 @@
 
 int a2s_gru_seq_bwd_impl(hipStream_t st, const float* dout, long do_bstride, long do_tstride, const float* out, long out_bstride,
                          long out_tstride, const float* gates, const float* w_hh, const float* dhn, float* dgi_all, float* dgh_shift,
-                         float* dgh_first, float* dhbuf, float* dgh_tmp, int B, int T, int H, int reverse, float* ws, size_t ws_bytes) {
+                         float* dgh_first, float* dhbuf, float* dgh_tmp, int B, int T, int H, int reverse, float* ws, size_t ws_bytes,
+                         float* ranges_out, int* ranges_valid) {
     A2S_REQUIRE(dout && out && gates && w_hh && dgi_all && dgh_shift && dgh_first && dhbuf && dgh_tmp, "gru_seq_bwd: null tensor");
+    if (ranges_valid) *ranges_valid = 0;
     hipError_t e;
     if (dhn) e = hipMemcpyAsync(dhbuf, dhn, sizeof(float) * B * H, hipMemcpyDeviceToDevice, st);
     else e = hipMemsetAsync(dhbuf, 0, sizeof(float) * B * H, st);
@@ -592,9 +594,12 @@
         hipLaunchKernelGGL(transpose_f32, dim3(a2s_cdiv(3 * H * H, 256)), dim3(256), 0, st, w_hh, ws, 3 * H, H);
         A2S_CHECK_LAUNCH("transpose_f32");
     }
-    if (fused && a2s_gru_seq_bwd_persist_ok(B, T, H, ws, ws_bytes, sizeof(float) * 3 * (size_t)H * H))
-        return a2s_gru_seq_bwd_persist_impl(st, dout, do_bstride, do_tstride, out, out_bstride, out_tstride, gates, ws, dhn, dgi_all, dgh_shift, dgh_first, B, T, H,
-                                            reverse, ws, sizeof(float) * 3 * (size_t)H * H, ws_bytes);
+    if (fused && a2s_gru_seq_bwd_persist_ok(B, T, H, ws, ws_bytes, sizeof(float) * 3 * (size_t)H * H)) {
+        const int rc = a2s_gru_seq_bwd_persist_impl(st, dout, do_bstride, do_tstride, out, out_bstride, out_tstride, gates, ws, dhn, dgi_all, dgh_shift, dgh_first,
+                                                    B, T, H, reverse, ws, sizeof(float) * 3 * (size_t)H * H, ws_bytes, ranges_out);
+        if (rc == A2S_OK && ranges_out && ranges_valid) *ranges_valid = 1;
+        return rc;
+    }
     if (fused && ws_bytes >= sizeof(float) * (3 * (size_t)H * H + 3 * (size_t)B * H) && (3 * H * H) % 4 == 0) {
         float* tmp[2] = {dgh_tmp, ws + 3 * (size_t)H * H};
         auto tix = [&](int s) { return reverse ? T - 1 - s : s; };
diff --git a/piano_a2s_amd/csrc/a2s_internal.h b/piano_a2s_amd/csrc/a2s_internal.h
--- a/piano_a2s_amd/csrc/a2s_internal.h
+++ b/piano_a2s_amd/csrc/a2s_internal.h
@@ -39,6 +39,13 @@
 bool a2s_linear_wgrad_ok(int M, int N, int K, long ldz, long lda, long ldg, int period, const void* dz, const void* A, const void* G);
 int a2s_linear_wgrad_impl(hipStream_t st, int M, int N, int K, const float* dz, long ldz, const float* A, long lda, float* G, long ldg, const float* a_scale,
     const float* a_shift, int period, const float* dz_absmax, const float* a_absmax, float* ws, size_t ws_bytes);
+extern int a2s_tallk_wgrad_on;
+extern int a2s_tallk_wgrad_max_splits;
+long a2s_tallk_wgrad_launches(void);
+size_t a2s_tallk_wgrad_ws_bytes_impl(int M, int Np, int K);
+bool a2s_tallk_wgrad_ok(int M, int Np, int K, long ldp, long lda, long ldg, int transposed, const void* P, const void* A, const void* G, const void* bias);
+int a2s_tallk_wgrad_impl(hipStream_t st, int M, int Np, int K, const float* P, long ldp, const float* A, long lda, float* G, long ldg, int transposed,
+    float* bias, const float* p_absmax, const float* a_absmax, float* ws, size_t ws_bytes);
 
 int a2s_act_bound_impl(hipStream_t st, const float* scale, const float* shift, const float* absmax, int C, float* out);
 size_t a2s_conv3x3_workspace_floats_impl(int Cin);
@@ -158,7 +165,8 @@
     const int* pair_rank, const int* pair_n_active);
 int a2s_gru_seq_bwd_impl(hipStream_t st, const float* dout, long do_bstride, long do_tstride, const float* out, long out_bstride,
     long out_tstride, const float* gates, const float* w_hh, const float* dhn, float* dgi_all, float* dgh_shift,
-    float* dgh_first, float* dhbuf, float* dgh_tmp, int B, int T, int H, int reverse, float* ws, size_t ws_bytes);
+    float* dgh_first, float* dhbuf, float* dgh_tmp, int B, int T, int H, int reverse, float* ws, size_t ws_bytes,
+    float* ranges_out, int* ranges_valid);
 int a2s_staff_emb_bwd_impl(hipStream_t st, const float* note_emb, const float* const* w, float* const* grads_dev, float* note_emb_grad,
     const long long* ids64, const int* ids32, long id_bstride, const long long* lengths, long len_stride,
     const float* dout, long lddo, int col0, const float* hsave, int R, int maxlen, int E, int S);
@@ -230,7 +238,7 @@
 bool a2s_gru_seq_bwd_persist_ok(int B, int T, int H, float* ws, size_t ws_bytes, size_t ws_used);
 int a2s_gru_seq_bwd_persist_impl(hipStream_t st, const float* dout, long do_bstride, long do_tstride, const float* out, long out_bstride, long out_tstride,
     const float* gates, const float* w_hh_t, const float* dhn, float* dgi_all, float* dgh_shift, float* dgh_first, int B, int T,
-    int H, int reverse, float* ws, size_t ws_off, size_t ws_bytes);
+    int H, int reverse, float* ws, size_t ws_off, size_t ws_bytes, float* ranges_out);
 
 int a2s_dec_persist_launches(void);
 bool a2s_note_decoder_fwd_persist_ok(const a2s_note_dec_args& a);
diff --git a/piano_a2s_amd/csrc/a2s_linear.hip b/piano_a2s_amd/csrc/a2s_linear.hip
--- a/piano_a2s_amd/csrc/a2s_linear.hip
+++ b/piano_a2s_amd/csrc/a2s_linear.hip
@@ -368,6 +368,8 @@
     const float* a_scale; const float* a_shift;
     const float* a_absmax; const float* d_absmax;
     int M, K, period, nblk, blk_per_split;
+    long plane_stride; int np;
+    float* bias_partial;
 };
 
 __global__ __launch_bounds__(256) void lin_pack_dz_planes(const float* __restrict__ dz, long ld, int M, int nsteps, const float* __restrict__ absmax,
@@ -375,6 +377,8 @@
     const long id = (long)blockIdx.x * 256 + threadIdx.x;
     const int n = (int)(id & 255), lk = (int)((id >> 8) & 3), s = (int)(id >> 10);
     if (s >= nsteps) return;
+    dz += blockIdx.y * 256;
+    out += (size_t)blockIdx.y * nsteps * (16 * 2 * 1024);
     float ps = ldexpf(1.f, pow2_scale_exp(*absmax, 12));
     if ((s >> 3) & 1) ps = -ps;
     float x[8];
@@ -391,6 +395,7 @@
     *reinterpret_cast<lu32x4*>(o + 64 * 16) = lo;
 }
 
+template <bool BIAS>
 __global__ __launch_bounds__(LIN_NTH) void lin_wgrad_roles(LinWgradArgs a) {
     __shared__ __attribute__((aligned(16))) unsigned char lds[LF_NS * LF_STAGE];
     const int tid = threadIdx.x, lane = tid & 63, lr = lane & 15, lk = lane >> 4;
@@ -411,6 +416,7 @@
         }
         const float floor_ = affine ? 0.f : -INFINITY;
         f32x4 ar[2][8];
+        f32x4 bs[2] = {(f32x4){0.f, 0.f, 0.f, 0.f}, (f32x4){0.f, 0.f, 0.f, 0.f}};
         auto issue_a = [&](int blk, f32x4 (&r)[8]) {
 #pragma unroll
             for (int u = 0; u < 2; ++u)
@@ -424,6 +430,14 @@
         auto commit_a = [&](int blk, const f32x4 (&r)[8]) {
             if (blk >= b_hi) return;
             unsigned char* st = lds + (blk % LF_NS) * LF_STAGE;
+            if (BIAS) {
+#pragma unroll
+                for (int u = 0; u < 2; ++u)
+#pragma unroll
+                    for (int j = 0; j < 4; ++j)
+#pragma unroll
+                        for (int c = 0; c < 4; ++c) bs[u][c] += r[4 * u + j][c];
+            }
 #pragma unroll
             for (int u = 0; u < 2; ++u)
 #pragma unroll
@@ -452,16 +466,27 @@
                 commit_a(b + 2, ar[0]); issue_a(b + 4, ar[0]);
             }
         }
+        if (BIAS && blockIdx.z == 0) {
+#pragma unroll
+            for (int u = 0; u < 2; ++u) {
+#pragma unroll
+                for (int c = 0; c < 4; ++c)
+#pragma unroll
+                    for (int o = 1; o < 16; o <<= 1) bs[u][c] += __shfl_xor(bs[u][c], o, 64);
+                if (rq == 0) *reinterpret_cast<f32x4*>(a.bias_partial + (long)blockIdx.y * a.K + k0 + 4 * (cq0 + 16 * u)) = bs[u];
+            }
+        }
         return;
     }
     lu32x4 df[2][4][2];
+    const unsigned char* planes = a.planes + blockIdx.z * a.plane_stride;
     auto load_d = [&](int step, lu32x4 (&dst)[4][2]) {
         if (step >= 2 * b_hi) return;
 #pragma unroll
         for (int nt = 0; nt < 4; ++nt)
 #pragma unroll
             for (int sp = 0; sp < 2; ++sp)
-                dst[nt][sp] = *reinterpret_cast<const lu32x4*>(a.planes + ((((long)step) * 16 + wave * 4 + nt) * 2 + sp) * 1024 + (unsigned)lane * 16u);
+                dst[nt][sp] = *reinterpret_cast<const lu32x4*>(planes + ((((long)step) * 16 + wave * 4 + nt) * 2 + sp) * 1024 + (unsigned)lane * 16u);
     };
     f32x4 acc[8][4];
 #pragma unroll
@@ -522,7 +547,7 @@
         __builtin_amdgcn_sched_barrier(0);
     }
     if (neg) flip();
-    float* slab = a.partial + (long)blockIdx.y * 256 * a.K;
+    float* slab = a.partial + ((long)blockIdx.y * a.np + blockIdx.z * 256) * a.K;
 #pragma unroll
     for (int kt = 0; kt < 8; ++kt)
 #pragma unroll
@@ -534,14 +559,34 @@
         }
 }
 
-__global__ __launch_bounds__(256) void lin_wgrad_reduce(const float* __restrict__ partial, int splits, long n, float* __restrict__ G, long ldg, int K) {
+template <bool TR>
+__global__ __launch_bounds__(256) void lin_wgrad_reduce(const float* __restrict__ partial, int splits, long n, float* __restrict__ G, long ldg, int K,
+                                                        const float* __restrict__ bias_partial, float* __restrict__ bias) {
     const long i = ((long)blockIdx.x * 256 + threadIdx.x) * 4;
-    if (i >= n) return;
+    if (i >= n) {
+        const long k = i - n;
+        if (!bias_partial || k >= K) return;
+        f32x4 s = *reinterpret_cast<const f32x4*>(bias_partial + k);
+        for (int p = 1; p < splits; ++p) {
+            const f32x4 v = *reinterpret_cast<const f32x4*>(bias_partial + (long)p * K + k);
+#pragma unroll
+            for (int r = 0; r < 4; ++r) s[r] += v[r];
+        }
+#pragma unroll
+        for (int r = 0; r < 4; ++r) bias[k + r] += s[r];
+        return;
+    }
     f32x4 s = *reinterpret_cast<const f32x4*>(partial + i);
     for (int p = 1; p < splits; ++p) {
         const f32x4 v = *reinterpret_cast<const f32x4*>(partial + (long)p * n + i);
 #pragma unroll
         for (int r = 0; r < 4; ++r) s[r] += v[r];
+    }
+    if (TR) {
+        float* g = G + (i % K) * ldg + (i / K);
+#pragma unroll
+        for (int r = 0; r < 4; ++r) g[r * ldg] += s[r];
+        return;
     }
     float* g = G + (i / K) * ldg + (i % K);
     const f32x4 o = *reinterpret_cast<const f32x4*>(g);
@@ -577,11 +622,65 @@
     float* partial = reinterpret_cast<float*>(planes + (size_t)nsteps * 16 * 2 * 1024);
     hipLaunchKernelGGL(lin_pack_dz_planes, dim3((unsigned)(((long)nsteps * 1024 + 255) / 256)), dim3(256), 0, st, dz, ldz, M, nsteps, dz_absmax, planes);
     A2S_CHECK_LAUNCH("lin_pack_dz_planes");
-    LinWgradArgs a{A, lda, planes, partial, a_scale, a_shift, a_absmax, dz_absmax, M, K, a_scale ? period : K, nblk, (nblk + splits - 1) / splits};
-    hipLaunchKernelGGL(lin_wgrad_roles, dim3(K / LIN_BM, splits), dim3(LIN_NTH), 0, st, a);
+    LinWgradArgs a{A, lda, planes, partial, a_scale, a_shift, a_absmax, dz_absmax, M, K, a_scale ? period : K, nblk, (nblk + splits - 1) / splits, 0, 256, nullptr};
+    hipLaunchKernelGGL(lin_wgrad_roles<false>, dim3(K / LIN_BM, splits), dim3(LIN_NTH), 0, st, a);
     A2S_CHECK_LAUNCH("lin_wgrad");
     const long n = 256L * K;
-    hipLaunchKernelGGL(lin_wgrad_reduce, dim3((unsigned)((n / 4 + 255) / 256)), dim3(256), 0, st, partial, splits, n, G, ldg, K);
+    hipLaunchKernelGGL(lin_wgrad_reduce<false>, dim3((unsigned)((n / 4 + 255) / 256)), dim3(256), 0, st, partial, splits, n, G, ldg, K, nullptr, nullptr);
     A2S_CHECK_LAUNCH("lin_wgrad_reduce");
     return A2S_OK;
 }
+
+#define TALLK_SLAB_BYTES (64u << 20)
+int a2s_tallk_wgrad_on = 1;
+int a2s_tallk_wgrad_max_splits = 0;
+static long long g_tallk_launches = 0;
+long a2s_tallk_wgrad_launches(void) { return (long)__atomic_load_n(&g_tallk_launches, __ATOMIC_RELAXED); }
+
+static int tallk_splits(int M, int Np, int K) {
+    const int tiles = (K / LIN_BM) * (Np / 256), nblk = (M + 63) / 64;
+    int cus = a2s_device_geometry().cus;
+    if (cus < 1) cus = 256;
+    int s = cus / tiles;
+    const size_t slab = (size_t)Np * K * sizeof(float);
+    if ((size_t)s * slab > TALLK_SLAB_BYTES) s = (int)(TALLK_SLAB_BYTES / slab);
+    if (s > nblk) s = nblk;
+    if (a2s_tallk_wgrad_max_splits > 0 && s > a2s_tallk_wgrad_max_splits) s = a2s_tallk_wgrad_max_splits;
+    return s < 1 ? 1 : s;
+}
+bool a2s_tallk_wgrad_ok(int M, int Np, int K, long ldp, long lda, long ldg, int transposed, const void* P, const void* A, const void* G, const void* bias) {
+    return a2s_tallk_wgrad_on && M >= 64 && Np >= 256 && Np % 256 == 0 && Np <= 2048 && K >= LIN_BM && K % LIN_BM == 0 && K <= 4096 && ldp >= Np && lda >= K &&
+           lda % 4 == 0 && ldg % 4 == 0 && ldg >= (transposed ? Np : K) && (((uintptr_t)P | (uintptr_t)A | (uintptr_t)G | (uintptr_t)bias) % 16 == 0);
+}
+size_t a2s_tallk_wgrad_ws_bytes_impl(int M, int Np, int K) {
+    if (M < 1 || Np < 256 || Np % 256 || K < LIN_BM || K % LIN_BM) return 0;
+    const size_t nsteps = 2 * (size_t)((M + 63) / 64), splits = (size_t)tallk_splits(M, Np, K);
+    return (size_t)(Np / 256) * nsteps * 16 * 2 * 1024 + splits * Np * K * sizeof(float) + splits * K * sizeof(float);
+}
+int a2s_tallk_wgrad_impl(hipStream_t st, int M, int Np, int K, const float* P, long ldp, const float* A, long lda, float* G, long ldg, int transposed,
+                         float* bias, const float* p_absmax, const float* a_absmax, float* ws, size_t ws_bytes) {
+    A2S_REQUIRE(P && A && G && p_absmax && a_absmax && ws, "tallk_wgrad: null argument");
+    A2S_REQUIRE(a2s_tallk_wgrad_ok(M, Np, K, ldp, lda, ldg, transposed, P, A, G, bias),
+                "tallk_wgrad: needs M >= 64, Np %% 256 == 0, K %% 128 == 0, 16-byte aligned bases and rows (or the switch \"tallk_wgrad\" is off)");
+    A2S_REQUIRE(((uintptr_t)ws % 16 == 0) && ws_bytes >= a2s_tallk_wgrad_ws_bytes_impl(M, Np, K), "tallk_wgrad: workspace too small (%zu bytes needed)",
+                a2s_tallk_wgrad_ws_bytes_impl(M, Np, K));
+    const int nblk = (M + 63) / 64, nsteps = 2 * nblk, splits = tallk_splits(M, Np, K), npb = Np / 256;
+    const size_t plane_stride = (size_t)nsteps * 16 * 2 * 1024;
+    unsigned char* planes = reinterpret_cast<unsigned char*>(ws);
+    float* partial = reinterpret_cast<float*>(planes + npb * plane_stride);
+    float* bias_partial = partial + (size_t)splits * Np * K;
+    hipLaunchKernelGGL(lin_pack_dz_planes, dim3((unsigned)(((long)nsteps * 1024 + 255) / 256), npb), dim3(256), 0, st, P, ldp, M, nsteps, p_absmax, planes);
+    A2S_CHECK_LAUNCH("lin_pack_dz_planes");
+    LinWgradArgs a{A, lda, planes, partial, nullptr, nullptr, a_absmax, p_absmax, M, K, K, nblk, (nblk + splits - 1) / splits, (long)plane_stride, Np,
+                   bias ? bias_partial : nullptr};
+    if (bias) hipLaunchKernelGGL(lin_wgrad_roles<true>, dim3(K / LIN_BM, splits, npb), dim3(LIN_NTH), 0, st, a);
+    else hipLaunchKernelGGL(lin_wgrad_roles<false>, dim3(K / LIN_BM, splits, npb), dim3(LIN_NTH), 0, st, a);
+    A2S_CHECK_LAUNCH("lin_wgrad (tall-K)");
+    const long n = (long)Np * K, nthreads = (n + (bias ? K : 0)) / 4;
+    const dim3 rgrid((unsigned)((nthreads + 255) / 256));
+    if (transposed) hipLaunchKernelGGL(lin_wgrad_reduce<true>, rgrid, dim3(256), 0, st, partial, splits, n, G, ldg, K, bias ? bias_partial : nullptr, bias);
+    else hipLaunchKernelGGL(lin_wgrad_reduce<false>, rgrid, dim3(256), 0, st, partial, splits, n, G, ldg, K, bias ? bias_partial : nullptr, bias);
+    A2S_CHECK_LAUNCH("lin_wgrad_reduce");
+    __atomic_fetch_add(&g_tallk_launches, 1LL, __ATOMIC_RELAXED);
+    return A2S_OK;
+}
diff --git a/piano_a2s_amd/csrc/a2s_persist.hip b/piano_a2s_amd/csrc/a2s_persist.hip
--- a/piano_a2s_amd/csrc/a2s_persist.hip
+++ b/piano_a2s_amd/csrc/a2s_persist.hip
@@ -230,6 +230,7 @@
 #pragma unroll
     for (int r = 0; r < 4; ++r) carry[r] = (wave == 0 && a.dhn) ? a.dhn[(long)min(row0 + lk * 4 + r, R - 1) * H + j] : 0.f;
     bool dead = false;
+    float mgi = 0.f, mgh = 0.f;
     for (int s = T - 1; s >= 0; --s) {
         const int t = a.reverse ? T - 1 - s : s;
         const int tp = a.reverse ? t + 1 : t - 1;
@@ -299,11 +300,19 @@
                 if (row < R) {
                     float* gi = a.dgi_all + ((long)row * T + t) * 3 * H;
                     gi[j] = dr; gi[H + j] = dz; gi[2 * H + j] = dn;
+                    const float mrz = fmaxf(fabsf(dr), fabsf(dz));
+                    mgi = fmaxf(mgi, fmaxf(mrz, fabsf(dn)));
+                    if (s > 0) mgh = fmaxf(mgh, fmaxf(mrz, fabsf(dnr)));
                     if (s > 0) { float* g2 = a.dgh_shift + ((long)row * T + tp) * 3 * H; g2[j] = dr; g2[H + j] = dz; g2[2 * H + j] = dnr; }
                     else { float* g1 = a.dgh_first + (long)row * 3 * H; g1[j] = dr; g1[H + j] = dz; g1[2 * H + j] = dnr; }
                 }
             }
         }
+    }
+    if (wave == 0) {
+        const float m1 = wave_max(mgi), m2 = wave_max(mgh);
+        if (lane == 0 && m1 > 0.f) atomicMax(a.abort_flag + 2, __float_as_uint(m1));
+        if (lane == 0 && m2 > 0.f) atomicMax(a.abort_flag + 3, __float_as_uint(m2));
     }
     if (wave == 0 && (dead || aborted(a.abort_flag))) {
 #pragma unroll
@@ -378,7 +387,7 @@
 }
 int a2s_gru_seq_bwd_persist_impl(hipStream_t st, const float* dout, long do_bstride, long do_tstride, const float* out, long out_bstride, long out_tstride,
                                  const float* gates, const float* w_hh_t, const float* dhn, float* dgi_all, float* dgh_shift, float* dgh_first, int B, int T,
-                                 int H, int reverse, float* ws, size_t ws_off, size_t ws_bytes) {
+                                 int H, int reverse, float* ws, size_t ws_off, size_t ws_bytes, float* ranges_out) {
     const size_t need = a2s_gru_persist_ws_bytes(B, H, 1);
     A2S_REQUIRE(need && ws_bytes >= ws_off + need, "gru_seq_bwd_persist: workspace too small");
     char* base = reinterpret_cast<char*>(ws) + ws_off;
@@ -391,5 +400,9 @@
                     g_abort_latch, a2s_persist_dbg()};
     hipLaunchKernelGGL(gru_seq_bwd_persist<256>, dim3((H / 16) * nrb), dim3(256), 0, st, a);
     A2S_CHECK_LAUNCH("gru_seq_bwd_persist");
+    if (ranges_out) {
+        e = hipMemcpyAsync(ranges_out, base + 2 * sizeof(unsigned), 2 * sizeof(float), hipMemcpyDeviceToDevice, st);
+        if (e != hipSuccess) A2S_FAIL(A2S_ERR_HIP, "gru_seq_bwd_persist range words: %s", hipGetErrorString(e));
+    }
     return A2S_OK;
 }
diff --git a/piano_a2s_amd/engine_bwd.py b/piano_a2s_amd/engine_bwd.py
--- a/piano_a2s_amd/engine_bwd.py
+++ b/piano_a2s_amd/engine_bwd.py
@@ -450,10 +450,11 @@
         enc_amax = hip.absmax(enc) if self.two_term else None
         for p, dKp in dK.items():
             Wn = p + ".attn.attn.weight"
-            sk = L.a2s_gemm_pick_splitk(H, H2, B * T, 1)
             dk_amax = hip.absmax(dKp) if self.two_term else None
-            hip.gemm(dKp, 1, H, enc2d, H2, 1, G[Wn], 4 * H, H, H2, B * T, beta=1.0, splitk=sk, c_off=H2,
-                     two_term=(dk_amax, enc_amax) if self.two_term else None)
+            if not hip.tallk_wgrad(dKp, 0, H, enc2d, 0, H2, G[Wn], H2, 4 * H, B * T, H, H2, dk_amax, enc_amax):
+                sk = L.a2s_gemm_pick_splitk(H, H2, B * T, 1)
+                hip.gemm(dKp, 1, H, enc2d, H2, 1, G[Wn], 4 * H, H, H2, B * T, beta=1.0, splitk=sk, c_off=H2,
+                         two_term=(dk_amax, enc_amax) if self.two_term else None)
             hip.gemm(dKp, H, 1, S[Wn], 4 * H, 1, dEnc, H2, B * T, H2, H, beta=1.0, b_off=H2,
                      two_term=(dk_amax, hip.absmax(S[Wn])) if self.two_term else None)
         if late_join is not None:
@@ -562,18 +563,26 @@
             dgi = torch.empty((B, T, 3 * H), device=dev)
             dghs = torch.empty((B, T, 3 * H), device=dev)
             dgh_first, dhbuf, dgh_tmp = torch.empty((B, 3 * H), device=dev), torch.empty((2, B, H), device=dev), torch.empty((B, 3 * H), device=dev)
-            hip.check(L.a2s_gru_seq_bwd(hip.stream(), _ptr(dout, d * H), C.c_long(T * 2 * H), C.c_long(2 * H), _ptr(out, d * H), C.c_long(T * 2 * H),
-                                        C.c_long(2 * H), hip._p(ls["dirs"][d]["gates"]), hip._p(S[f"encoder.gru.weight_hh_{sfx}"]), hip._p(dhn[2 * layer + d]),
-                                        hip._p(dgi), hip._p(dghs), hip._p(dgh_first), hip._p(dhbuf), hip._p(dgh_tmp), B, T, H, d, hip._p(gws[d]),
-                                        C.c_size_t(gws[d].numel() * 4)), "a2s_gru_seq_bwd")
-            return (dgi, dghs, dgh_first, dhbuf, dgh_tmp)
+            ranges, valid = torch.empty(2, device=dev), C.c_int(0)
+            if two_term and L.a2s_debug_get(b"tallk_wgrad") > 0:
+                hip.check(L.a2s_gru_seq_bwd_ranged(hip.stream(), _ptr(dout, d * H), C.c_long(T * 2 * H), C.c_long(2 * H), _ptr(out, d * H), C.c_long(T * 2 * H),
+                                                   C.c_long(2 * H), hip._p(ls["dirs"][d]["gates"]), hip._p(S[f"encoder.gru.weight_hh_{sfx}"]),
+                                                   hip._p(dhn[2 * layer + d]), hip._p(dgi), hip._p(dghs), hip._p(dgh_first), hip._p(dhbuf), hip._p(dgh_tmp), B, T, H, d,
+                                                   hip._p(gws[d]), C.c_size_t(gws[d].numel() * 4), hip._p(ranges), C.byref(valid)), "a2s_gru_seq_bwd_ranged")
+            else:
+                hip.check(L.a2s_gru_seq_bwd(hip.stream(), _ptr(dout, d * H), C.c_long(T * 2 * H), C.c_long(2 * H), _ptr(out, d * H), C.c_long(T * 2 * H),
+                                            C.c_long(2 * H), hip._p(ls["dirs"][d]["gates"]), hip._p(S[f"encoder.gru.weight_hh_{sfx}"]), hip._p(dhn[2 * layer + d]),
+                                            hip._p(dgi), hip._p(dghs), hip._p(dgh_first), hip._p(dhbuf), hip._p(dgh_tmp), B, T, H, d, hip._p(gws[d]),
+                                            C.c_size_t(gws[d].numel() * 4)), "a2s_gru_seq_bwd")
+            return (dgi, dghs, dgh_first, dhbuf, dgh_tmp, ranges if valid.value else None)
 
         res = fork_on_streams(dev, streams, [lambda d=d, sfx=sfx: direction(d, sfx) for d, sfx in enumerate((f"l{layer}", f"l{layer}_reverse"))])()
         dgi_amax = []
         for d, sfx in enumerate((f"l{layer}", f"l{layer}_reverse")):
             dgi2 = res[d][0].view(B * T, 3 * H)
             Wih = S[f"encoder.gru.weight_ih_{sfx}"]
-            tt = (hip.absmax(dgi2), hip.absmax(Wih)) if two_term else None
+            ranges = res[d][5]
+            tt = (ranges[0:1] if ranges is not None else hip.absmax(dgi2), hip.absmax(Wih)) if two_term else None
             dgi_amax.append(tt[0] if tt else None)
             if L.a2s_debug_get(b"gemm_bf16x3") > 0:
                 hip.gemm(dgi2, 3 * H, 1, Wih.t().contiguous(), 1, 3 * H, dX, I, B * T, I, 3 * H, beta=0.0 if d == 0 else 1.0, two_term=tt)
@@ -584,18 +593,24 @@
         ev.record()
         wg.wait_event(ev)
         for d, sfx in enumerate((f"l{layer}", f"l{layer}_reverse")):
-            dgi, dghs, dgh_first = res[d][:3]
-            for t in (dgi, dghs, dgh_first, dgi_amax[d], in_amax):
+            dgi, dghs, dgh_first, ranges = res[d][0], res[d][1], res[d][2], res[d][5]
+            for t in (dgi, dghs, dgh_first, dgi_amax[d], in_amax, ranges):
                 if t is not None:
                     t.record_stream(wg)
             with torch.cuda.stream(wg):
                 dgi2, dghs2 = dgi.view(B * T, 3 * H), dghs.view(B * T, 3 * H)
-                _linear_bwd(inp, S[f"encoder.gru.weight_ih_{sfx}"], dgi2, G, f"encoder.gru.weight_ih_{sfx}", f"encoder.gru.bias_ih_{sfx}",
-                            dy_amax=dgi_amax[d], x_bound=(in_amax if layer == 0 else hip.one(dev)) if two_term else None)
-                sk = L.a2s_gemm_pick_splitk(3 * H, H, B * T, 1)
-                hip.gemm(dghs2, 1, 3 * H, out, 2 * H, 1, G[f"encoder.gru.weight_hh_{sfx}"], H, 3 * H, H, B * T, beta=1.0, splitk=sk, b_off=d * H,
-                         two_term=(hip.absmax(dghs2), hip.one(dev)) if two_term else None)
-                _colsum(dghs2, 3 * H, G[f"encoder.gru.bias_hh_{sfx}"], B * T, 3 * H)
+                x_bound = ((in_amax if layer == 0 else hip.one(dev)) if two_term else None)
+                if not hip.tallk_wgrad(inp, 0, I, dgi2, 0, 3 * H, G[f"encoder.gru.weight_ih_{sfx}"], 0, I, B * T, I, 3 * H, x_bound, dgi_amax[d],
+                                       transposed=True, bias=G[f"encoder.gru.bias_ih_{sfx}"]):
+                    _linear_bwd(inp, S[f"encoder.gru.weight_ih_{sfx}"], dgi2, G, f"encoder.gru.weight_ih_{sfx}", f"encoder.gru.bias_ih_{sfx}",
+                                dy_amax=dgi_amax[d], x_bound=x_bound)
+                dghs_amax = (ranges[1:2] if ranges is not None else hip.absmax(dghs2)) if two_term else None
+                if not hip.tallk_wgrad(out, d * H, 2 * H, dghs2, 0, 3 * H, G[f"encoder.gru.weight_hh_{sfx}"], 0, H, B * T, H, 3 * H,
+                                       hip.one(dev) if two_term else None, dghs_amax, transposed=True, bias=G[f"encoder.gru.bias_hh_{sfx}"]):
+                    sk = L.a2s_gemm_pick_splitk(3 * H, H, B * T, 1)
+                    hip.gemm(dghs2, 1, 3 * H, out, 2 * H, 1, G[f"encoder.gru.weight_hh_{sfx}"], H, 3 * H, H, B * T, beta=1.0, splitk=sk, b_off=d * H,
+                             two_term=(dghs_amax, hip.one(dev)) if two_term else None)
+                    _colsum(dghs2, 3 * H, G[f"encoder.gru.bias_hh_{sfx}"], B * T, 3 * H)
                 _colsum(dgh_first, 3 * H, G[f"encoder.gru.bias_hh_{sfx}"], B, 3 * H)
         dout = dX.view(B, T, I)
     if wait_weight_grads:
diff --git a/piano_a2s_amd/hip.py b/piano_a2s_amd/hip.py
--- a/piano_a2s_amd/hip.py
+++ b/piano_a2s_amd/hip.py
@@ -1,5 +1,6 @@
 import ctypes as C
 import os
+import threading
 
 import torch
 
@@ -66,7 +67,7 @@
         L = C.CDLL(LIB)
         L.a2s_last_error.restype = C.c_char_p
         L.a2s_launch_count.restype = C.c_longlong
-        for fn in ("a2s_note_step_workspace_floats", "a2s_note_decoder_persist_ws_bytes", "a2s_note_decoder_bwd_persist_ws_bytes", "a2s_linear_dgrad_ws_bytes", "a2s_linear_wgrad_ws_bytes", "a2s_gemm_workspace_bytes", "a2s_bn_bwd_partial_floats", "a2s_conv3x3_wgrad_workspace_bytes", "a2s_attn_workspace_floats", "a2s_attn_workspace_floats_fused",
+        for fn in ("a2s_note_step_workspace_floats", "a2s_note_decoder_persist_ws_bytes", "a2s_note_decoder_bwd_persist_ws_bytes", "a2s_linear_dgrad_ws_bytes", "a2s_linear_wgrad_ws_bytes", "a2s_tallk_wgrad_ws_bytes", "a2s_gemm_workspace_bytes", "a2s_bn_bwd_partial_floats", "a2s_conv3x3_wgrad_workspace_bytes", "a2s_attn_workspace_floats", "a2s_attn_workspace_floats_fused",
                    "a2s_conv3x3_workspace_floats"):
             getattr(L, fn).restype = C.c_size_t
         if hasattr(L, "a2s_env_check") and L.a2s_env_check() != 0:
@@ -75,6 +76,8 @@
             L.a2s_edit_distance.argtypes = [C.c_void_p] * 6 + [C.c_int] * 3 + [C.c_void_p]
         if hasattr(L, "a2s_attn_denc_accum"):
             L.a2s_attn_denc_accum.argtypes = [C.c_void_p] * 4 + [C.c_int] * 4 + [C.c_void_p, C.c_int]
+        if hasattr(L, "a2s_tallk_wgrad_eligible"):
+            L.a2s_tallk_wgrad_eligible.argtypes = [C.c_int] * 3 + [C.c_long] * 3 + [C.c_int]
         if arith != "f16x2":
             for key in (b"conv_f16x2", b"wgrad_f16x2", b"gemm_f16x2"):
                 L.a2s_debug_set(key, 0)
@@ -446,6 +449,27 @@
     return True
 
 
+_TALLK_WS = {}
+
+
+def tallk_wgrad(P, p_off, ldp, A, a_off, lda, G, g_off, ldg, M, Np, K, p_absmax, a_absmax, transposed=False, bias=None):
+    L = lib()
+    if not hasattr(L, "a2s_tallk_wgrad_eligible"):
+        return False
+    pp, pa, pg = P.data_ptr() + 4 * p_off, A.data_ptr() + 4 * a_off, G.data_ptr() + 4 * g_off
+    if (p_absmax is None or a_absmax is None or (pp | pa | pg | (bias.data_ptr() if bias is not None else 0)) % 16
+            or not L.a2s_tallk_wgrad_eligible(M, Np, K, ldp, lda, ldg, int(transposed))):
+        return False
+    nb = L.a2s_tallk_wgrad_ws_bytes(M, Np, K)
+    key = (A.device, torch.cuda.current_stream().cuda_stream, threading.get_ident())
+    ws = _TALLK_WS.get(key)
+    if ws is None or ws.numel() * 4 < nb:
+        ws = _TALLK_WS[key] = torch.empty((nb + 3) // 4, dtype=torch.float32, device=A.device)
+    check(L.a2s_tallk_wgrad(stream(), M, Np, K, C.c_void_p(pp), C.c_long(ldp), C.c_void_p(pa), C.c_long(lda), C.c_void_p(pg), C.c_long(ldg), int(transposed),
+                            _p(bias), _p(p_absmax), _p(a_absmax), _p(ws), C.c_size_t(ws.numel() * 4)), "a2s_tallk_wgrad")
+    return True
+
+
 def linear_forward_for_test(x, w, aff):
     period = aff[2]
     xmax = x.view(x.shape[0], -1, period).abs().amax(dim=(0, 2)).contiguous()
```

Result: faster. 639.8, median of 6 (+2.1%).
